# Mine268/CS-ViT

Measured on NVIDIA B200. Metric: images/sec Swin-B spatial fwd @224^2 bs256, higher is better.
Workload: dtype fp16

## Files before the change

cs-vit_b200/cs_vit/_lib.py:

```python
from __future__ import annotations

import ctypes
import os
from ctypes import c_char_p, c_float, c_int, c_longlong, c_void_p

_HERE = os.path.dirname(os.path.abspath(__file__))
LIB_PATH = os.environ.get("CSVIT_LIB", os.path.join(_HERE, "..", "lib", "libcsvit_sm100.so"))

SIGNATURES = {
    "csvit_abi_version": [],
    "csvit_window_index_map": [c_int, c_int, c_int, c_int, c_void_p, c_void_p],
    "csvit_shift_mask": [c_int, c_int, c_int, c_int, c_void_p, c_void_p],
    "csvit_rel_pos_index": [c_int, c_void_p, c_void_p],
    "csvit_merge_index_map": [c_int, c_int, c_void_p, c_void_p],
    "csvit_host_window_index_map": [c_int, c_int, c_int, c_int, c_void_p],
    "csvit_host_shift_mask": [c_int, c_int, c_int, c_int, c_void_p],
    "csvit_host_rel_pos_index": [c_int, c_void_p],
    "csvit_host_merge_index_map": [c_int, c_int, c_void_p],
    "csvit_expand_rel_bias": [c_void_p, c_void_p, c_int, c_int, c_void_p],
    "csvit_layernorm": [c_void_p, c_void_p, c_void_p, c_float, c_void_p, c_int, c_longlong, c_int, c_int, c_int,
                        c_int, c_int, c_int, c_int, c_void_p],
    "csvit_affine_rows": [c_void_p, c_void_p, c_void_p, c_void_p, c_int, c_longlong, c_int, c_void_p],
    "csvit_patch_im2col": [c_void_p, c_void_p, c_int, c_int, c_int, ctypes.POINTER(c_float), ctypes.POINTER(c_float),
                           c_void_p],
    "csvit_linear": [c_void_p, c_longlong, c_void_p, c_longlong, c_int, c_int, c_int, c_int, c_void_p, c_int, c_void_p,
                     c_longlong, c_void_p, c_longlong, c_int, c_int, c_int, c_int, c_int, c_int, c_void_p],
    "csvit_mlp_fused": [c_void_p, c_longlong, c_void_p, c_longlong, c_void_p, c_void_p, c_longlong, c_void_p, c_void_p,
                        c_longlong, c_int, c_int, c_int, c_void_p],
    "csvit_swin_attn_fused": [c_void_p, c_float, c_void_p, c_void_p, c_void_p, c_void_p, c_int, c_int, c_int, c_int,
                              c_int, c_int, c_int, c_int, c_void_p],
    "csvit_swin_attn_core": [c_void_p, c_longlong, c_void_p, c_void_p, c_int, c_int, c_int, c_int, c_int, c_int, c_int, c_int,
                             c_int, c_int, c_void_p],
    "csvit_crop_resize": [c_void_p, c_int, c_int, c_int, c_int, c_void_p, c_float, c_void_p, c_void_p, c_int, c_void_p],
    "csvit_rot6d_to_axis_angle": [c_void_p, c_void_p, c_longlong, c_void_p],
    "csvit_mano_fk": [c_void_p] * 10 + [c_void_p, c_void_p, c_int, c_void_p, c_void_p, c_void_p, c_int, c_void_p],
    "csvit_allreduce_f32": [c_void_p, c_void_p, c_void_p, c_longlong, c_int, c_int, c_float, c_int, c_void_p],
    "csvit_last_gemm_kernel": [],
    "csvit_set_gemm_tuning": [c_int, c_int, c_int, c_int],
    "csvit_window_attention": [c_void_p, c_void_p, c_void_p, c_int, c_int, c_int, c_int, c_int, c_int, c_int, c_int, c_void_p],
    "csvit_attention": [c_void_p, c_void_p, c_void_p, c_void_p, c_int, c_longlong, c_longlong, c_longlong, c_longlong,
                        c_int, c_int, c_int, c_int, c_float, c_void_p],
    "csvit_swinv2_window_attention": [c_void_p, c_void_p, c_void_p, c_void_p, c_int, c_int, c_int, c_int, c_int, c_int, c_int, c_int,
                                      c_int, c_int, c_void_p],
    "csvit_swinv2_qkv": [c_void_p, c_longlong, c_void_p, c_longlong, c_int, c_int, c_int, c_int, c_void_p, c_void_p, c_void_p, c_longlong,
                         c_void_p],
    "csvit_swinv2_attn_tc": [c_void_p, c_longlong, c_void_p, c_void_p, c_int, c_int, c_int, c_int, c_int, c_int, c_int, c_int, c_int,
                             c_void_p],
    "csvit_layernorm_post": [c_void_p, c_longlong, c_void_p, c_void_p, c_void_p, c_float, c_void_p, c_void_p, c_int, c_longlong,
                             c_int, c_int, c_int, c_int, c_int, c_int, c_int, c_void_p],
    "csvit_gemm_ex": [c_void_p, c_longlong, c_int, c_void_p, c_longlong, c_int, c_int, c_int, c_int, c_int, c_void_p, c_longlong,
                      c_int, c_int, c_int, c_int, c_void_p],
    "csvit_col_reduce": [c_void_p, c_int, c_longlong, c_void_p, c_longlong, c_void_p, c_int, c_int, c_int, c_int, c_int, c_int,
                         c_int, c_int, c_void_p, c_int, c_longlong, c_void_p, c_void_p, c_void_p],
    "csvit_transpose_f32": [c_void_p, c_longlong, c_void_p, c_longlong, c_int, c_int, c_void_p],
    "csvit_row_scale_add": [c_void_p, c_void_p, c_void_p, c_void_p, c_longlong, c_int, c_int, c_void_p],
    "csvit_eltwise": [c_int, c_void_p, c_void_p, c_void_p, c_int, c_longlong, c_void_p],
    "csvit_affine2_rows": [c_void_p, c_void_p, c_void_p, c_void_p, c_void_p, c_void_p, c_void_p, c_longlong, c_int, c_void_p],
    "csvit_layernorm_bwd": [c_void_p, c_void_p, c_int, c_longlong, c_void_p, c_float, c_int, c_int, c_int, c_int, c_int, c_int,
                            c_int, c_void_p, c_void_p, c_void_p, c_void_p, c_void_p],
    "csvit_attention_bwd": [c_void_p, c_void_p, c_void_p, c_void_p, c_void_p, c_void_p, c_void_p, c_int, c_longlong, c_longlong,
                            c_longlong, c_longlong, c_longlong, c_longlong, c_longlong, c_int, c_int, c_int, c_int, c_float,
                            c_void_p, c_void_p, c_int, c_int, c_int, c_int, c_void_p],
}

_lib = None


class CsvitError(RuntimeError):
    pass


def load() -> ctypes.CDLL:
    global _lib
    if _lib is not None:
        return _lib
    path = os.path.abspath(LIB_PATH)
    if not os.path.exists(path):
        raise ImportError(
            f"{path} not found. cs_vit has no CPU/PyTorch fallback: build the sm_100a kernels first with "
            f"`python -c 'import __graft_entry__ as g; g.build()'` or `make -C cs-vit_b200/csrc`.")
    lib = ctypes.CDLL(path)
    for name, argtypes in SIGNATURES.items():
        fn = getattr(lib, name)
        fn.argtypes = argtypes
        fn.restype = c_int
    lib.csvit_last_error.argtypes = []
    lib.csvit_last_error.restype = c_char_p
    _lib = lib
    return lib


def check(code: int) -> None:
    if code != 0:
        raise CsvitError(load().csvit_last_error().decode("utf-8", "replace"))
```

cs-vit_b200/cs_vit/net/swin_b200.py:

```python
from __future__ import annotations

import json
import os
from types import SimpleNamespace
from typing import Dict, List, Optional

import torch
import torch.nn as nn

from .. import ops
from ._pack import PackCache


PRECISIONS = {"bf16": torch.bfloat16, "fp16": torch.float16, "fp32": torch.float32}


class SwinConfigLite(SimpleNamespace):

    @classmethod
    def from_dict(cls, d: Dict) -> "SwinConfigLite":
        model_type = d.get("model_type", "swin")
        if model_type != "swin":
            raise NotImplementedError(
                f"backbone model_type '{model_type}' is not built: only Swin v1 (window 7) has sm_100a kernels "
                f"(SwinV2 is the next row of SURVEY.md §8f); there is no fallback path")
        embed_dim = d.get("embed_dim", 96)
        depths = list(d.get("depths", [2, 2, 6, 2]))
        cfg = cls(
            model_type=model_type,
            image_size=d.get("image_size", 224),
            patch_size=d.get("patch_size", 4),
            num_channels=d.get("num_channels", 3),
            embed_dim=embed_dim,
            depths=depths,
            num_heads=list(d.get("num_heads", [3, 6, 12, 24])),
            window_size=d.get("window_size", 7),
            mlp_ratio=d.get("mlp_ratio", 4.0),
            qkv_bias=d.get("qkv_bias", True),
            layer_norm_eps=d.get("layer_norm_eps", 1e-5),
            use_absolute_embeddings=d.get("use_absolute_embeddings", False),
            hidden_act=d.get("hidden_act", "gelu"),
            drop_path_rate=d.get("drop_path_rate", 0.1),
            hidden_size=int(embed_dim * 2 ** (len(depths) - 1)),
        )
        if cfg.patch_size != 4 or cfg.num_channels != 3 or cfg.mlp_ratio != 4.0 or not cfg.qkv_bias:
            raise NotImplementedError("only patch 4 / RGB / mlp_ratio 4 / qkv_bias Swin configurations are built")
        if cfg.use_absolute_embeddings or cfg.hidden_act != "gelu":
            raise NotImplementedError("absolute position embeddings / non-GELU activations are not built")
        if any(cfg.embed_dim * 2 ** s != 32 * h for s, h in enumerate(cfg.num_heads)):
            raise NotImplementedError("the attention kernels require head_dim == 32 at every stage")
        return cfg


def _holder(**children) -> nn.Module:
    m = nn.Module()
    for k, v in children.items():
        setattr(m, k, v)
    return m


class _SelfAttnParams(nn.Module):
    def __init__(self, dim: int, heads: int, ws: int):
        super().__init__()
        self.query = nn.Linear(dim, dim)
        self.key = nn.Linear(dim, dim)
        self.value = nn.Linear(dim, dim)
        self.relative_position_bias_table = nn.Parameter(torch.zeros((2 * ws - 1) ** 2, heads))
        ys, xs = torch.meshgrid(torch.arange(ws), torch.arange(ws), indexing="ij")
        dy = ys.reshape(-1, 1) - ys.reshape(1, -1) + ws - 1
        dx = xs.reshape(-1, 1) - xs.reshape(1, -1) + ws - 1
        self.register_buffer("relative_position_index", (dy * (2 * ws - 1) + dx).to(torch.int64))


class _BlockParams(nn.Module):

    def __init__(self, dim: int, heads: int, ws: int, eps: float):
        super().__init__()
        self.layernorm_before = nn.LayerNorm(dim, eps=eps)
        self.attention = _holder(self=_SelfAttnParams(dim, heads, ws), output=_holder(dense=nn.Linear(dim, dim)))
        self.layernorm_after = nn.LayerNorm(dim, eps=eps)
        self.intermediate = _holder(dense=nn.Linear(dim, 4 * dim))
        self.output = _holder(dense=nn.Linear(4 * dim, dim))


class SwinBackboneB200(nn.Module):
    def __init__(self, config: SwinConfigLite, precision: str = "bf16"):
        super().__init__()
        self.config = config
        self.precision = precision
        self.fuse_attn = True
        self.fuse_attn_widths = ops.ATTN_FUSED_WIDTHS
        self._drop_path_rand: List[torch.Tensor] = []
        self.fuse_mlp = True
        self.micro_batch = 0
        c0, eps, ws = config.embed_dim, config.layer_norm_eps, config.window_size
        self.embeddings = _holder(
            patch_embeddings=_holder(projection=nn.Conv2d(3, c0, kernel_size=4, stride=4)),
            norm=nn.LayerNorm(c0, eps=eps))
        stages: List[nn.Module] = []
        for s, (depth, heads) in enumerate(zip(config.depths, config.num_heads)):
            dim = c0 * 2 ** s
            stage = nn.Module()
            stage.blocks = nn.ModuleList([_BlockParams(dim, heads, ws, eps) for _ in range(depth)])
            if s < len(config.depths) - 1:
                stage.downsample = _holder(reduction=nn.Linear(4 * dim, 2 * dim, bias=False), norm=nn.LayerNorm(4 * dim, eps=eps))
            stages.append(stage)
        self.encoder = _holder(layers=nn.ModuleList(stages))
        self.layernorm = nn.LayerNorm(config.hidden_size, eps=eps)
        self._pack = PackCache()

    @classmethod
    def from_pretrained(cls, path: str, precision: str = "bf16") -> "SwinBackboneB200":
        with open(os.path.join(path, "config.json")) as f:
            cfg = SwinConfigLite.from_dict(json.load(f))
        model = cls(cfg, precision)
        st = os.path.join(path, "model.safetensors")
        if os.path.exists(st):
            from safetensors.torch import load_file
            sd = load_file(st)
        else:
            sd = torch.load(os.path.join(path, "pytorch_model.bin"), map_location="cpu")
        sd = {(k[len("swin."):] if k.startswith("swin.") else k): v for k, v in sd.items()}
        missing, unexpected = model.load_state_dict(sd, strict=False)
        missing = [k for k in missing if not k.endswith("relative_position_index")]
        unexpected = [k for k in unexpected if not k.startswith("pooler")]
        if missing or unexpected:
            raise RuntimeError(f"backbone checkpoint mismatch: missing {missing[:5]} unexpected {unexpected[:5]}")
        model.eval()
        return model

    @property
    def _fp32(self) -> bool:
        if self.precision not in PRECISIONS:
            raise ValueError(f"precision must be one of {sorted(PRECISIONS)}, got {self.precision!r}")
        return self.precision == "fp32"

    @property
    def _act_dtype(self) -> torch.dtype:
        _ = self._fp32
        return PRECISIONS[self.precision]

    def _w(self, key: str, tensors, build):
        return self._pack.get(f"{self.precision}/{key}", tensors, build)

    def _weight(self, key: str, lin_weight: torch.Tensor) -> torch.Tensor:
        dt = self._act_dtype
        return self._w(key, [lin_weight], lambda: lin_weight.detach().reshape(lin_weight.shape[0], -1).to(dt).contiguous())

    def _f32(self, key: str, t: torch.Tensor) -> torch.Tensor:
        return self._w(key, [t], lambda: t.detach().float().contiguous())

    def _block(self, x: torch.Tensor, blk: _BlockParams, key: str, B: int, H: int, W: int, heads: int, shift: int) -> None:
        cfg = self.config
        ws = cfg.window_size
        if min(H, W) <= ws:
            ws, shift = min(H, W), 0
        C = x.shape[1]
        act = self._act_dtype
        impl = ops.GEMM_SIMT if self._fp32 else ops.GEMM_TC
        sa = blk.attention.self
        qkv_src = [sa.query.weight, sa.key.weight, sa.value.weight]
        bqkv_src = [sa.query.bias, sa.key.bias, sa.value.bias]
        eps = cfg.layer_norm_eps
        ln1 = blk.layernorm_before
        proj = blk.attention.output.dense
        wproj, bproj = self._weight(key + "wproj", proj.weight), self._f32(key + "bproj", proj.bias)
        if self._fp32:
            wqkv = self._w(key + "wqkv", qkv_src, lambda: torch.cat([w.detach() for w in qkv_src], 0).to(act).contiguous())
            bqkv = self._w(key + "bqkv", bqkv_src, lambda: torch.cat([b.detach() for b in bqkv_src], 0).float().contiguous())
            bias = self._w(key + "relbias", [sa.relative_position_bias_table],
                           lambda: ops.expand_rel_bias(sa.relative_position_bias_table.detach(), ws))
            xn = ops.layernorm(x, self._f32(key + "ln1w", ln1.weight), self._f32(key + "ln1b", ln1.bias), eps, out_dtype=act,
                               mode=ops.LN_WINDOW, grid=(H, W), ws=ws, shift=shift)
            qkv = ops.linear(xn, wqkv, bqkv, out_dtype=act, impl=impl)
            ctx = ops.window_attention(qkv, bias, B, H, W, heads, ws, shift)
            ops.linear(ctx, wproj, bproj, resid=x, out=x, scatter=(H, W, ws, shift), impl=impl)
        else:
            if ws != 7 or C != 32 * heads:
                raise NotImplementedError(f"the tcgen05 window-attention kernels are built for 7x7 windows and head_dim 32 "
                                          f"(got window {ws}, C={C}, heads={heads}); use precision='fp32'")
            if self.fuse_attn and C in self.fuse_attn_widths:
                src = qkv_src + bqkv_src + [sa.relative_position_bias_table, ln1.weight, ln1.bias]
                wqkv_h, bqkv_h, bias_op = self._w(key + "attn_fused", src, lambda: ops.pack_attn_fused(
                    sa.query.weight, sa.key.weight, sa.value.weight, sa.query.bias, sa.key.bias, sa.value.bias,
                    sa.relative_position_bias_table, sa.relative_position_index, act, ln1.weight, ln1.bias))
                ctx = ops.swin_attn_fused(x, eps, wqkv_h, bqkv_h, bias_op, B, H, W, heads, ws, shift)
                ops.linear(ctx, wproj, bproj, resid=x, out=x, impl=impl)
            else:
                wqs, bqs = self._w(key + "wqkv_qs", qkv_src + bqkv_src, lambda: ops.pack_qkv_prescaled(
                    sa.query.weight, sa.key.weight, sa.value.weight, sa.query.bias, sa.key.bias, sa.value.bias, act))
                bias_l2 = self._w(key + "relbias_l2", [sa.relative_position_bias_table],
                                  lambda: ops.pack_rel_bias_log2(sa.relative_position_bias_table, sa.relative_position_index))
                xn = ops.layernorm(x, self._f32(key + "ln1w", ln1.weight), self._f32(key + "ln1b", ln1.bias), eps, out_dtype=act,
                                   mode=ops.LN_WINDOW, grid=(H, W), ws=ws, shift=shift)
                qkv = ops.linear(xn, wqs, bqs, out_dtype=act, impl=impl)
                tok = C >= 256
                ctx = ops.swin_attn_core(qkv, bias_l2, B, H, W, heads, ws, shift, token_order=tok, q_prescaled=True)
                ops.linear(ctx, wproj, bproj, resid=x, out=x, impl=impl, **({} if tok else {"scatter": (H, W, ws, shift)}))
        ln2 = blk.layernorm_after
        fc1, fc2 = blk.intermediate.dense, blk.output.dense
        xn = ops.layernorm(x, self._f32(key + "ln2w", ln2.weight), self._f32(key + "ln2b", ln2.bias), eps, out_dtype=act)
        if self.fuse_mlp and not self._fp32 and C in ops.MLP_FUSED_WIDTHS:
            ops.mlp_fused(xn, self._weight(key + "w1", fc1.weight), self._f32(key + "b1", fc1.bias),
                          self._weight(key + "w2", fc2.weight), self._f32(key + "b2", fc2.bias), x)
            return
        hid = ops.linear(xn, self._weight(key + "w1", fc1.weight), self._f32(key + "b1", fc1.bias), act=ops.ACT_GELU,
                         out_dtype=act, impl=impl)
        ops.linear(hid, self._weight(key + "w2", fc2.weight), self._f32(key + "b2", fc2.bias), resid=x, out=x, impl=impl)

    def forward_features(self, images: torch.Tensor, normalize: bool, return_stages: bool = False):
        cfg = self.config
        if not images.is_cuda:
            raise RuntimeError("SwinBackboneB200 runs on CUDA tensors only (there is no CPU fallback)")
        n, _, S, S2 = images.shape
        if S != S2 or S % (32 * cfg.window_size) != 0:
            raise ValueError(f"image side {S} must be a multiple of {32 * cfg.window_size} (no padding path, SURVEY.md §8b)")
        wants_grad = torch.is_grad_enabled() and any(p.requires_grad for p in self.parameters())
        if not return_stages and (wants_grad or (self.training and cfg.drop_path_rate > 0)):
            return self._forward_train(images, normalize)
        with torch.no_grad():
            return self._forward_infer(images, normalize, return_stages)

    def _block_pack(self, blk: _BlockParams, key: str, ws: int) -> Dict:
        act = self._act_dtype
        sa = blk.attention.self
        qkv_src = [sa.query.weight, sa.key.weight, sa.value.weight]
        bqkv_src = [sa.query.bias, sa.key.bias, sa.value.bias]
        tab = sa.relative_position_bias_table
        return {
            "wqkv": self._w(key + "wqkv", qkv_src, lambda: torch.cat([w.detach() for w in qkv_src], 0).to(act).contiguous()),
            "bqkv": self._w(key + "bqkv", bqkv_src, lambda: torch.cat([b.detach() for b in bqkv_src], 0).float().contiguous()),
            "bias": self._w(key + "relbias", [tab], lambda: ops.expand_rel_bias(tab.detach(), ws)),
            "bias_log2": None if self._fp32 else self._w(key + "relbias_l2", [tab], lambda: ops.pack_rel_bias_log2(tab, sa.relative_position_index)),
            "wo": self._weight(key + "wproj", blk.attention.output.dense.weight),
            "w1": self._weight(key + "w1", blk.intermediate.dense.weight),
            "w2": self._weight(key + "w2", blk.output.dense.weight),
            "rel_index": self._w(key + "relidx", [sa.relative_position_index], lambda: sa.relative_position_index.reshape(-1).long()),
            "table_rows": tab.shape[0],
        }

    def _forward_train(self, images: torch.Tensor, normalize: bool) -> torch.Tensor:
        from .. import autograd as ag
        cfg = self.config
        n, _, S, _ = images.shape
        act = self._act_dtype
        impl = ops.GEMM_SIMT if self._fp32 else ops.GEMM_TC
        eps = cfg.layer_norm_eps
        H = W = S // 4
        pe = self.embeddings.patch_embeddings.projection
        x = ag.PatchEmbedFn.apply(images.float().contiguous(), pe.weight, pe.bias, self.embeddings.norm.weight, self.embeddings.norm.bias,
                                  self._weight("pe_w", pe.weight), (normalize, eps, act, impl))
        total_blocks = sum(cfg.depths)
        rates = torch.linspace(0, cfg.drop_path_rate, total_blocks).tolist() if self.training and cfg.drop_path_rate > 0 else [0.0] * total_blocks
        k = -1
        for s, stage in enumerate(self.encoder.layers):
            heads = cfg.num_heads[s]
            for i, blk in enumerate(stage.blocks):
                k += 1
                ws, shift = cfg.window_size, (0 if i % 2 == 0 else cfg.window_size // 2)
                if min(H, W) <= ws:
                    ws, shift = min(H, W), 0
                sa = blk.attention.self
                pk = dict(self._block_pack(blk, f"s{s}b{i}/", ws))
                if rates[k] > 0.0:
                    keep = 1.0 - rates[k]
                    u = self._drop_path_rand.pop(0).to(x.device, torch.float32) if self._drop_path_rand else torch.rand(n, device=x.device)
                    pk["keep_scale"] = (torch.floor(keep + u) / keep).contiguous()
                x = ag.SwinBlockFn.apply(
                    x, blk.layernorm_before.weight, blk.layernorm_before.bias, sa.query.weight, sa.query.bias, sa.key.weight,
                    sa.key.bias, sa.value.weight, sa.value.bias, sa.relative_position_bias_table, blk.attention.output.dense.weight,
                    blk.attention.output.dense.bias, blk.layernorm_after.weight, blk.layernorm_after.bias, blk.intermediate.dense.weight,
                    blk.intermediate.dense.bias, blk.output.dense.weight, blk.output.dense.bias, pk,
                    (n, H, W, heads, ws, shift, eps, act, impl))
            if hasattr(stage, "downsample"):
                ds = stage.downsample
                x = ag.PatchMergeFn.apply(x, ds.norm.weight, ds.norm.bias, ds.reduction.weight,
                                          self._weight(f"s{s}/dsr", ds.reduction.weight), (H, W, eps, act, impl))
                H, W = H // 2, W // 2
        out = ag.LayerNormFn.apply(x, self.layernorm.weight, self.layernorm.bias, eps)
        return out.view(n, H * W, cfg.hidden_size)

    def _forward_infer(self, images: torch.Tensor, normalize: bool, return_stages: bool = False, out: Optional[torch.Tensor] = None):
        cfg = self.config
        n, _, S, _ = images.shape
        mb = self.micro_batch
        if mb and n > mb and not return_stages:
            images = images.float().contiguous()
            full = torch.empty(n, (S // 32) ** 2, cfg.hidden_size, dtype=torch.float32, device=images.device)
            for lo in range(0, n, mb):
                self._forward_infer(images[lo:lo + mb], normalize, out=full[lo:lo + mb])
            return full
        act = self._act_dtype
        impl = ops.GEMM_SIMT if self._fp32 else ops.GEMM_TC
        eps = cfg.layer_norm_eps
        H = W = S // 4
        cols = ops.patch_im2col(images.float().contiguous(), out_dtype=act, normalize=normalize)
        pe = self.embeddings.patch_embeddings.projection
        y = ops.linear(cols, self._weight("pe_w", pe.weight), self._f32("pe_b", pe.bias), out_dtype=torch.float32, impl=impl)
        x = ops.layernorm(y, self._f32("pe_lnw", self.embeddings.norm.weight), self._f32("pe_lnb", self.embeddings.norm.bias), eps)
        stages = []
        for s, stage in enumerate(self.encoder.layers):
            heads = cfg.num_heads[s]
            for i, blk in enumerate(stage.blocks):
                self._block(x, blk, f"s{s}b{i}/", n, H, W, heads, 0 if i % 2 == 0 else cfg.window_size // 2)
            if return_stages:
                stages.append(x.view(n, H * W, -1).clone())
            if hasattr(stage, "downsample"):
                ds = stage.downsample
                xm = ops.layernorm(x, self._f32(f"s{s}/dsw", ds.norm.weight), self._f32(f"s{s}/dsb", ds.norm.bias), eps,
                                   out_dtype=act, mode=ops.LN_MERGE2X2, grid=(H, W))
                x = ops.linear(xm, self._weight(f"s{s}/dsr", ds.reduction.weight), None, out_dtype=torch.float32, impl=impl)
                H, W = H // 2, W // 2
        out = ops.layernorm(x, self._f32("final_w", self.layernorm.weight), self._f32("final_b", self.layernorm.bias), eps,
                            out=None if out is None else out.view(n * H * W, cfg.hidden_size))
        out = out.view(n, H * W, cfg.hidden_size)
        return (out, stages) if return_stages else out

    def forward(self, pixel_values: torch.Tensor, **_unused) -> SimpleNamespace:
        return SimpleNamespace(last_hidden_state=self.forward_features(pixel_values, normalize=False), pooler_output=None)
```

cs-vit_b200/cs_vit/ops.py:

```python
from __future__ import annotations

import ctypes
from typing import Optional, Tuple

import torch

from . import _lib

F32, BF16, F16 = 0, 1, 2
ACT_NONE, ACT_GELU, ACT_RELU = 0, 1, 2
LN_IDENTITY, LN_WINDOW, LN_MERGE2X2 = 0, 1, 2
GEMM_TC, GEMM_SIMT = 0, 1

_DT = {torch.float32: F32, torch.bfloat16: BF16, torch.float16: F16}

launch_count = 0


def _code(dtype: torch.dtype) -> int:
    try:
        return _DT[dtype]
    except KeyError:
        raise TypeError(f"cs_vit kernels take float32, bfloat16 or float16 tensors, got {dtype}") from None

# ... 30 lines not shown
    for kind in sorted({e[4] for e in ev if e[4]}):
        sel = [e for e in ev if e[4] == kind]
        out[f"kind{kind}"] = {"launches": len(sel), "ms": sum(e[0].elapsed_time(e[1]) for e in sel), "flops": float(sum(e[2] for e in sel))}
    return out


def _call(name: str, *args, flops: float = 0.0, nbytes: float = 0.0) -> None:
    global launch_count
    launch_count += 1
    if _profile is not None and _profile["name"] == name:
        e0, e1 = torch.cuda.Event(enable_timing=True), torch.cuda.Event(enable_timing=True)
        e0.record()
        _lib.check(getattr(_lib.load(), name)(*args))
        e1.record()
        kind = _lib.load().csvit_last_gemm_kernel() if name == "csvit_linear" else 0
        _profile["events"].append((e0, e1, flops, nbytes, kind))
        return
    _lib.check(getattr(_lib.load(), name)(*args))


def _rows2d(t: torch.Tensor) -> Tuple[int, int, int]:
    if t.dim() != 2 or t.stride(1) != 1:
        raise ValueError(f"expected a 2-D tensor with contiguous rows, got shape {tuple(t.shape)} strides {t.stride()}")
    return t.shape[0], t.shape[1], t.stride(0)


def window_index_map(H: int, W: int, ws: int, shift: int, device="cuda") -> torch.Tensor:
    out = torch.empty(H * W, dtype=torch.int32, device=device)
    _call("csvit_window_index_map", H, W, ws, shift, out.data_ptr(), _stream())
    return out


def shift_mask(H: int, W: int, ws: int, shift: int, device="cuda") -> torch.Tensor:
    nW, L = (H // ws) * (W // ws), ws * ws
    out = torch.empty(nW, L, L, dtype=torch.float32, device=device)
    _call("csvit_shift_mask", H, W, ws, shift, out.data_ptr(), _stream())
    return out


def rel_pos_index(ws: int, device="cuda") -> torch.Tensor:
    out = torch.empty(ws * ws, ws * ws, dtype=torch.int32, device=device)
    _call("csvit_rel_pos_index", ws, out.data_ptr(), _stream())
    return out


def merge_index_map(H: int, W: int, device="cuda") -> torch.Tensor:
    out = torch.empty((H // 2) * (W // 2), 4, dtype=torch.int32, device=device)
    _call("csvit_merge_index_map", H, W, out.data_ptr(), _stream())
    return out


def expand_rel_bias(table: torch.Tensor, ws: int) -> torch.Tensor:
    _dev(table)
    table = table.contiguous().float()
    heads = table.shape[1]
    out = torch.empty(heads, ws * ws, ws * ws, dtype=torch.float32, device=table.device)
    _call("csvit_expand_rel_bias", table.data_ptr(), out.data_ptr(), heads, ws, _stream())
    return out


def layernorm(x: torch.Tensor, gamma: torch.Tensor, beta: torch.Tensor, eps: float, *, out_dtype=torch.float32,
              mode: int = LN_IDENTITY, grid: Tuple[int, int] = (0, 0), ws: int = 0, shift: int = 0,
              out: Optional[torch.Tensor] = None) -> torch.Tensor:
    _dev(x, gamma, beta, out)
    if x.dtype != torch.float32 or not x.is_contiguous():
        raise ValueError("layernorm input must be contiguous float32")
    rows_in, C = x.shape
    H, W = grid
    if mode == LN_MERGE2X2:
        rows, width = rows_in // 4, 4 * C
    else:
        rows, width = rows_in, C
    if gamma.numel() != width or beta.numel() != width:
        raise ValueError(f"layernorm affine width {gamma.numel()} != {width}")
    if out is None:
        out = torch.empty(rows, width, dtype=out_dtype, device=x.device)
    _call("csvit_layernorm", x.data_ptr(), gamma.data_ptr(), beta.data_ptr(), float(eps), out.data_ptr(), _code(out.dtype),
          out.stride(0), rows, C, mode, H, W, ws, shift, _stream(),
          nbytes=float(rows * width * (4 + out.element_size())))
    return out


def affine_rows(x: torch.Tensor, scale: torch.Tensor, shift: torch.Tensor, *, out_dtype=torch.float32) -> torch.Tensor:
    _dev(x, scale, shift)
    if x.dtype != torch.float32 or not x.is_contiguous():
        raise ValueError("affine_rows input must be contiguous float32")
    C = x.shape[-1]
    out = torch.empty(x.shape, dtype=out_dtype, device=x.device)
    _call("csvit_affine_rows", x.data_ptr(), scale.data_ptr(), shift.data_ptr(), out.data_ptr(), _code(out_dtype),
          x.numel() // C, C, _stream())
    return out


_MEAN = (ctypes.c_float * 3)(0.485, 0.456, 0.406)
_STD = (ctypes.c_float * 3)(0.229, 0.224, 0.225)


def patch_im2col(img: torch.Tensor, *, out_dtype=torch.bfloat16, normalize: bool = True) -> torch.Tensor:
    _dev(img)
    if img.dtype != torch.float32 or not img.is_contiguous() or img.dim() != 4 or img.shape[1] != 3:
        raise ValueError("patch_im2col takes contiguous float32 [B,3,S,S]")
    B, _, S, S2 = img.shape
    if S != S2:
        raise ValueError("square images only")
    out = torch.empty(B * (S // 4) ** 2, 48, dtype=out_dtype, device=img.device)
    mean = _MEAN if normalize else (ctypes.c_float * 3)(0, 0, 0)
    std = _STD if normalize else (ctypes.c_float * 3)(1, 1, 1)
    _call("csvit_patch_im2col", img.data_ptr(), out.data_ptr(), _code(out_dtype), B, S, mean, std, _stream())
    return out


def linear(a: torch.Tensor, w: torch.Tensor, bias: Optional[torch.Tensor] = None, *, act: int = ACT_NONE,
           resid: Optional[torch.Tensor] = None, out: Optional[torch.Tensor] = None, out_dtype: Optional[torch.dtype] = None,
           scatter: Optional[Tuple[int, int, int, int]] = None, impl: int = GEMM_TC) -> torch.Tensor:
    _dev(a, w, bias, resid, out)
    M, K, lda = _rows2d(a)
    N, K2, ldw = _rows2d(w)
    if K != K2 or a.dtype != w.dtype:
        raise ValueError(f"linear: A {tuple(a.shape)}/{a.dtype} vs W {tuple(w.shape)}/{w.dtype}")
    if out is None:
        out = torch.empty(M, N, dtype=out_dtype or a.dtype, device=a.device)
    _, No, ldo = _rows2d(out)
    if No != N:
        raise ValueError("linear: output width mismatch")
    ldr = 0
    if resid is not None:
        if resid.dtype != torch.float32:
            raise ValueError("linear: residual must be float32")
        ldr = _rows2d(resid)[2]
    if bias is not None and (bias.dtype != torch.float32 or bias.numel() != N):
        raise ValueError("linear: bias must be float32 [N]")
    sH, sW, sws, ssh = scatter if scatter is not None else (0, 0, 0, 0)
    _call("csvit_linear", a.data_ptr(), lda, w.data_ptr(), ldw, _code(a.dtype), M, N, K, _p(bias), act, _p(resid), ldr,
          out.data_ptr(), ldo, _code(out.dtype), sH, sW, sws, ssh, impl, _stream(), flops=2.0 * M * N * K)
    return out


MLP_FUSED_WIDTHS = (128, 256)


def mlp_fused(xn: torch.Tensor, w1: torch.Tensor, b1: torch.Tensor, w2: torch.Tensor, b2: torch.Tensor, x: torch.Tensor) -> torch.Tensor:
    _dev(xn, w1, b1, w2, b2, x)
    M, C, ldxn = _rows2d(xn)
    if w1.shape != (4 * C, C) or w2.shape != (C, 4 * C) or x.shape != (M, C) or x.dtype != torch.float32:
        raise ValueError("mlp_fused: shape mismatch")
    if not (xn.dtype == w1.dtype == w2.dtype) or xn.dtype not in (torch.bfloat16, torch.float16):
        raise ValueError("mlp_fused: xn / w1 / w2 must share a 16-bit dtype")
    _call("csvit_mlp_fused", xn.data_ptr(), ldxn, w1.data_ptr(), w1.stride(0), b1.data_ptr(), w2.data_ptr(), w2.stride(0),
          b2.data_ptr(), x.data_ptr(), x.stride(0), _code(xn.dtype), M, C, _stream(), flops=16.0 * M * C * C)
    return x


ATTN_FUSED_WIDTHS = (128, 256)
_LOG2E = 1.4426950408889634


def pack_attn_fused(wq: torch.Tensor, wk: torch.Tensor, wv: torch.Tensor, bq: torch.Tensor, bk: torch.Tensor, bv: torch.Tensor,
                    table: torch.Tensor, rel_index: torch.Tensor, dtype: torch.dtype, gamma: torch.Tensor, beta: torch.Tensor):
    C = wq.shape[0]
    heads = C // 32
    g64, be64 = gamma.detach().double(), beta.detach().double()
    fold_w = lambda w_: (w_.detach().double() * g64[None, :]).float()
    fold_b = lambda w_, b_: (b_.detach().double() + w_.detach().double() @ be64).float()
    w = torch.stack([fold_w(wq).view(heads, 32, C), fold_w(wk).view(heads, 32, C), fold_w(wv).view(heads, 32, C)], 1)
    qs = _LOG2E / 32.0 ** 0.5
    b = torch.stack([fold_b(wq, bq).view(heads, 32) * qs, fold_b(wk, bk).view(heads, 32), fold_b(wv, bv).view(heads, 32)], 1)
    return w.reshape(3 * C, C).to(dtype).contiguous(), b.reshape(3 * C).contiguous(), pack_rel_bias_log2(table, rel_index)


def pack_rel_bias_log2(table: torch.Tensor, rel_index: torch.Tensor) -> torch.Tensor:
    heads = table.shape[1]
    L = rel_index.shape[0]
    if L != 49:
        raise ValueError("pack_rel_bias_log2: 7x7 windows only")
    bias = table.detach().float()[rel_index.reshape(-1).long()].view(L, L, heads).permute(2, 0, 1)
    op = torch.zeros(heads, L, 56, dtype=torch.float32, device=table.device)
    op[:, :, :L] = bias * _LOG2E
    return op.to(torch.float16).reshape(heads * L, 56).contiguous()


def pack_qkv_prescaled(wq, wk, wv, bq, bk, bv, dtype: torch.dtype):
    qs = _LOG2E / 32.0 ** 0.5
    w = torch.cat([wq.detach().float() * qs, wk.detach().float(), wv.detach().float()], 0)
    b = torch.cat([bq.detach().float() * qs, bk.detach().float(), bv.detach().float()], 0)
    return w.to(dtype).contiguous(), b.contiguous()


def swin_attn_core(qkv: torch.Tensor, bias_log2: torch.Tensor, B: int, H: int, W: int, heads: int, ws: int, shift: int,
                   token_order: bool = False, q_prescaled: bool = False, out: Optional[torch.Tensor] = None) -> torch.Tensor:
    _dev(qkv, bias_log2, out)
    rows, C3, ld = _rows2d(qkv)
    C = C3 // 3
    if qkv.dtype not in (torch.bfloat16, torch.float16) or rows != B * H * W or C != heads * 32 or ws != 7:
        raise ValueError(f"swin_attn_core: needs 16-bit qkv [B*H*W, 3C] with head_dim 32 and 7x7 windows (rows={rows} C={C} heads={heads} ws={ws})")
    if bias_log2.dtype != torch.float16 or tuple(bias_log2.shape) != (heads * 49, 56) or not bias_log2.is_contiguous():
        raise ValueError("swin_attn_core: bias_log2 must be contiguous float16 [heads*49, 56] (pack_rel_bias_log2)")
    if out is None:
        out = torch.empty(rows, C, dtype=qkv.dtype, device=qkv.device)
    L = ws * ws
    _call("csvit_swin_attn_core", qkv.data_ptr(), ld, bias_log2.data_ptr(), out.data_ptr(), _code(qkv.dtype), B, H, W, C, heads, ws,
          shift, 1 if token_order else 0, 1 if q_prescaled else 0, _stream(),
          flops=float(rows) * 4.0 * L * C, nbytes=float(rows) * C * 8.0)
    return out


def swin_attn_fused(x: torch.Tensor, eps: float, wqkv_h: torch.Tensor, bqkv_h: torch.Tensor,
                    bias_op: torch.Tensor, B: int, H: int, W: int, heads: int, ws: int, shift: int,
                    out: Optional[torch.Tensor] = None) -> torch.Tensor:
    _dev(x, wqkv_h, bqkv_h, bias_op, out)
    if x.dtype != torch.float32 or not x.is_contiguous() or x.dim() != 2:
        raise ValueError("swin_attn_fused input must be contiguous float32 [B*H*W, C]")
    rows, C = x.shape
    if rows != B * H * W or C != heads * 32 or C not in ATTN_FUSED_WIDTHS:
        raise ValueError(f"swin_attn_fused: rows={rows} C={C} heads={heads} not supported (C in {ATTN_FUSED_WIDTHS}, head_dim 32)")
    if wqkv_h.dtype not in (torch.bfloat16, torch.float16) or tuple(wqkv_h.shape) != (3 * C, C) or not wqkv_h.is_contiguous():
        raise ValueError("swin_attn_fused: wqkv_h must be contiguous 16-bit [3C, C]")
    if bqkv_h.dtype != torch.float32 or bqkv_h.numel() != 3 * C or bias_op.dtype != torch.float16 or tuple(bias_op.shape) != (heads * 49, 56) or not bias_op.is_contiguous():
        raise ValueError("swin_attn_fused: bqkv_h must be float32 [3C] and bias_op contiguous float16 [heads*49, 56]")
    if out is None:
        out = torch.empty(rows, C, dtype=wqkv_h.dtype, device=x.device)
    L = ws * ws
    _call("csvit_swin_attn_fused", x.data_ptr(), float(eps), wqkv_h.data_ptr(), bqkv_h.data_ptr(),
          bias_op.data_ptr(), out.data_ptr(), _code(wqkv_h.dtype), B, H, W, C, heads, ws, shift, _stream(),
          flops=float(rows) * (6.0 * C * C + 4.0 * L * C), nbytes=float(rows) * C * 6.0)
    return out


def window_attention(qkv: torch.Tensor, bias_exp: Optional[torch.Tensor], B: int, H: int, W: int, heads: int, ws: int,
                     shift: int, bias_log2: Optional[torch.Tensor] = None, token_order: bool = False) -> torch.Tensor:
    if qkv.dtype != torch.float32:
        if bias_log2 is None:
            raise ValueError("window_attention: 16-bit qkv needs bias_log2 (ops.pack_rel_bias_log2)")
        return swin_attn_core(qkv, bias_log2, B, H, W, heads, ws, shift, token_order=token_order)
    if token_order:
        raise ValueError("window_attention: token-ordered output is built for the 16-bit kernels only")
    _dev(qkv, bias_exp)
    rows, C3, ld = _rows2d(qkv)
    C = C3 // 3
    if ld != C3 or rows != B * H * W:
        raise ValueError("window_attention: qkv must be dense [B*H*W, 3C]")
    out = torch.empty(rows, C, dtype=qkv.dtype, device=qkv.device)
    _call("csvit_window_attention", qkv.data_ptr(), _p(bias_exp), out.data_ptr(), _code(qkv.dtype), B, H, W, C,
          heads, ws, shift, _stream(), nbytes=float(qkv.numel() + out.numel()) * qkv.element_size())
    return out


def attention(q: torch.Tensor, k: torch.Tensor, v: torch.Tensor, n_seq: int, Lq: int, S: int, heads: int,
              scale: float) -> torch.Tensor:
    _dev(q, k, v)
    rq, D, ldq = _rows2d(q)
    rk, _, ldk = _rows2d(k)
    _, _, ldv = _rows2d(v)
    if rq != n_seq * Lq or rk != n_seq * S or D != heads * 32:
        raise ValueError("attention: shape mismatch (head_dim must be 32)")
    out = torch.empty(rq, D, dtype=q.dtype, device=q.device)
    _call("csvit_attention", q.data_ptr(), k.data_ptr(), v.data_ptr(), out.data_ptr(), _code(q.dtype), ldq, ldk, ldv, D,
          n_seq, Lq, S, heads, float(scale), _stream())
    return out


COPY_NONE, COPY_IDENTITY, COPY_WINDOW, COPY_MERGE2X2 = 0, 1, 2, 3


def swinv2_window_attention(qkv: torch.Tensor, bias_tab: torch.Tensor, logit_scale: torch.Tensor, B: int, H: int, W: int, heads: int,
                            ws: int, shift: int, mask_repeat: int = 2, token_order: bool = False) -> torch.Tensor:
    _dev(qkv, bias_tab, logit_scale)
    rows, C3, ld = _rows2d(qkv)
    C = C3 // 3
    if ld != C3 or rows != B * H * W:
        raise ValueError("swinv2_window_attention: qkv must be dense [B*H*W, 3C]")
    if bias_tab.dtype != torch.float32 or tuple(bias_tab.shape) != (heads, (2 * ws - 1) ** 2) or not bias_tab.is_contiguous():
        raise ValueError(f"swinv2_window_attention: bias table must be contiguous float32 [{heads}, {(2 * ws - 1) ** 2}]")
    if logit_scale.dtype != torch.float32 or logit_scale.numel() != heads or not logit_scale.is_contiguous():
        raise ValueError("swinv2_window_attention: logit_scale must be contiguous float32 [heads]")
    out = torch.empty(rows, C, dtype=qkv.dtype, device=qkv.device)
    L = ws * ws
    _call("csvit_swinv2_window_attention", qkv.data_ptr(), bias_tab.data_ptr(), logit_scale.data_ptr(), out.data_ptr(),
          _code(qkv.dtype), B, H, W, C, heads, ws, shift, mask_repeat, 1 if token_order else 0, _stream(),
          flops=4.0 * rows * L * C, nbytes=float(qkv.numel() + out.numel()) * qkv.element_size())
    return out


def swinv2_qkv(a: torch.Tensor, w: torch.Tensor, bias: Optional[torch.Tensor], qscale_log2: torch.Tensor) -> torch.Tensor:
    _dev(a, w, qscale_log2)
    M, K, lda = _rows2d(a)
    N, K2, ldw = _rows2d(w)
    C = N // 3
    if K2 != K or N != 3 * C or a.dtype != w.dtype or a.dtype not in (torch.float16, torch.bfloat16):
        raise ValueError("swinv2_qkv: a [M, K] and w [3C, K] must share one 16-bit dtype")
    if qscale_log2.dtype != torch.float32 or qscale_log2.numel() != C // 32 or not qscale_log2.is_contiguous():
        raise ValueError("swinv2_qkv: qscale_log2 must be contiguous float32 [C / 32]")
    if bias is not None and (bias.dtype != torch.float32 or bias.numel() != N or not bias.is_contiguous()):
        raise ValueError("swinv2_qkv: bias must be contiguous float32 [3C]")
    out = torch.empty(M, N, dtype=a.dtype, device=a.device)
    _call("csvit_swinv2_qkv", a.data_ptr(), lda, w.data_ptr(), ldw, _code(a.dtype), M, C, K, bias.data_ptr() if bias is not None else None,
          qscale_log2.data_ptr(), out.data_ptr(), N, _stream(), flops=2.0 * M * N * K,
          nbytes=float(a.numel() + w.numel() + out.numel()) * a.element_size())
    return out


def swinv2_bias_log2(bias_tab: torch.Tensor) -> torch.Tensor:
    heads = bias_tab.shape[0]
    out = torch.zeros(heads, 31, 48, dtype=torch.float32, device=bias_tab.device)
    out[:, :, :31] = bias_tab.float().view(heads, 31, 31) * 1.4426950408889634
    return out.contiguous()


def swinv2_attn_tc(qkv: torch.Tensor, bias_log2: torch.Tensor, B: int, H: int, W: int, heads: int, shift: int, mask_repeat: int = 2,
                   token_order: bool = False) -> torch.Tensor:
    _dev(qkv, bias_log2)
    rows, C3, ld = _rows2d(qkv)
    C = C3 // 3
    if rows != B * H * W or qkv.dtype not in (torch.float16, torch.bfloat16):
        raise ValueError("swinv2_attn_tc: qkv must be 16-bit [B*H*W, 3C]")
    if bias_log2.dtype != torch.float32 or tuple(bias_log2.shape) != (heads, 31, 48) or not bias_log2.is_contiguous():
        raise ValueError(f"swinv2_attn_tc: bias table must be contiguous float32 [{heads}, 31, 48]")
    out = torch.empty(rows, C, dtype=qkv.dtype, device=qkv.device)
    _call("csvit_swinv2_attn_tc", qkv.data_ptr(), ld, bias_log2.data_ptr(), out.data_ptr(), _code(qkv.dtype), B, H, W, C, heads, shift,
          mask_repeat, 1 if token_order else 0, _stream(), flops=4.0 * rows * 256 * C,
          nbytes=float(qkv.numel() + out.numel()) * qkv.element_size())
    return out


def layernorm_post(y: torch.Tensor, resid: Optional[torch.Tensor], gamma: torch.Tensor, beta: torch.Tensor, eps: float, *,
                   out: Optional[torch.Tensor] = None, copy_mode: int = COPY_NONE, copy_dtype: torch.dtype = torch.bfloat16,
                   geom: Tuple[int, int, int, int] = (0, 0, 0, 0)) -> Tuple[torch.Tensor, Optional[torch.Tensor]]:
    _dev(y, resid, gamma, beta, out)
    rows, C, ldy = _rows2d(y)
    if y.dtype != torch.float32:
        raise ValueError("layernorm_post input must be float32")
    if resid is not None and (resid.dtype != torch.float32 or tuple(resid.shape) != (rows, C) or not resid.is_contiguous()):
        raise ValueError("layernorm_post: residual must be contiguous float32 [rows, C]")
    if gamma.numel() != C or beta.numel() != C:
        raise ValueError(f"layernorm_post affine width {gamma.numel()} != {C}")
    if out is None:
        out = torch.empty(rows, C, dtype=torch.float32, device=y.device)
    elif out.dtype != torch.float32 or tuple(out.shape) != (rows, C) or not out.is_contiguous():
        raise ValueError("layernorm_post: out must be contiguous float32 [rows, C]")
    H, W, ws, shift = geom
    copy = None
    if copy_mode == COPY_MERGE2X2:
        copy = torch.empty(rows // 4, 4 * C, dtype=copy_dtype, device=y.device)
    elif copy_mode != COPY_NONE:
        copy = torch.empty(rows, C, dtype=copy_dtype, device=y.device)
    _call("csvit_layernorm_post", y.data_ptr(), ldy, _p(resid), gamma.data_ptr(), beta.data_ptr(), float(eps), out.data_ptr(), _p(copy),
          _code(copy_dtype), 0 if copy is None else copy.stride(0), copy_mode, rows, C, H, W, ws, shift, _stream(),
          nbytes=float(rows * C * (8 + (4 if resid is not None else 0) + (0 if copy is None else copy.element_size()))))
    return out, copy


CR_SUM, CR_CENTERED, CR_DOT = 0, 1, 2
EW_GELU_FWD, EW_GELU_BWD, EW_RELU_BWD = 0, 1, 2


def gemm_ex(a: torch.Tensor, a_mn: bool, b: torch.Tensor, b_mn: bool, *, out: Optional[torch.Tensor] = None,
            out_dtype: Optional[torch.dtype] = None, accumulate: bool = False, impl: int = GEMM_TC, split_k: int = 0) -> torch.Tensor:
    _dev(a, b, out)
    if a.dtype == torch.float32 and impl == GEMM_TC:
        if a_mn:
            a, a_mn = transpose(a), False
        if b_mn:
            b, b_mn = transpose(b), False
    r0, c0, lda = _rows2d(a)
    r1, c1, ldb = _rows2d(b)
    M, K = (c0, r0) if a_mn else (r0, c0)
    N, K2 = (c1, r1) if b_mn else (r1, c1)
    if K != K2 or a.dtype != b.dtype:
        raise ValueError(f"gemm_ex: A {tuple(a.shape)}/{a.dtype} (mn={a_mn}) vs B {tuple(b.shape)}/{b.dtype} (mn={b_mn})")
    if out is None:
        if accumulate:
            raise ValueError("gemm_ex: accumulate needs an output tensor")
        out = torch.empty(M, N, dtype=out_dtype or a.dtype, device=a.device)
    Mo, No, ldo = _rows2d(out)
    if (Mo, No) != (M, N):
        raise ValueError("gemm_ex: output shape mismatch")
    _call("csvit_gemm_ex", a.data_ptr(), lda, int(a_mn), b.data_ptr(), ldb, int(b_mn), _code(a.dtype), M, N, K, out.data_ptr(), ldo,
# ... 208 lines not shown
```

cs-vit_b200/csrc/api.cu:

```cuda
#include <cstdarg>
#include <cstdio>
#include <cstdlib>

#include "../../include/csvit.h"
#include "errors.h"
#include "gemm.cuh"
#include "rowops.cuh"

namespace csvit {

static thread_local char g_err[1024] = "";

int set_error(const char* fmt, ...) {
  va_list ap;
  va_start(ap, fmt);
  vsnprintf(g_err, sizeof(g_err), fmt, ap);
  va_end(ap);
  return 1;
}
const char* last_error() { return g_err; }

bool pdl_enabled() {
  static const bool on = [] { const char* e = getenv("CSVIT_PDL"); return e && e[0] == '1'; }();
  return on;
}

}

using namespace csvit;

static_assert(int(CSVIT_F32) == int(DT_F32) && int(CSVIT_BF16) == int(DT_BF16) && int(CSVIT_F16) == int(DT_F16), "dtype codes");
static inline bool ok_dtype(int d) { return d == DT_F32 || d == DT_BF16 || d == DT_F16; }
static_assert(int(CSVIT_ACT_GELU) == int(ACT_GELU) && int(CSVIT_ACT_RELU) == int(ACT_RELU), "activation codes");
static_assert(int(CSVIT_LN_WINDOW) == int(LN_WINDOW) && int(CSVIT_LN_MERGE2X2) == int(LN_MERGE2X2), "layernorm modes");
static_assert(int(CSVIT_GEMM_SIMT_FP32) == int(GEMM_SIMT), "gemm impl codes");

static inline cudaStream_t S(void* s) { return static_cast<cudaStream_t>(s); }
static GemmTuning g_tune = {0, 0, -1, -1};

extern "C" {

int csvit_abi_version(void) { return CSVIT_ABI_VERSION; }
const char* csvit_last_error(void) { return last_error(); }

int csvit_window_index_map(int H, int W, int ws, int shift, int32_t* out, void* stream) {
  CSVIT_REQUIRE(ws > 0 && H % ws == 0 && W % ws == 0, "window_index_map: %dx%d not divisible by window %d", H, W, ws);
  CSVIT_REQUIRE(shift >= 0 && shift < ws, "window_index_map: shift %d outside [0,%d)", shift, ws);
  return launch_window_index_map(H, W, ws, shift, out, S(stream));
}
int csvit_shift_mask(int H, int W, int ws, int shift, float* out, void* stream) {
  CSVIT_REQUIRE(ws > 0 && H % ws == 0 && W % ws == 0, "shift_mask: %dx%d not divisible by window %d", H, W, ws);
  CSVIT_REQUIRE(shift >= 0 && shift < ws, "shift_mask: shift %d outside [0,%d)", shift, ws);
  return launch_shift_mask(H, W, ws, shift, out, S(stream));
}
int csvit_rel_pos_index(int ws, int32_t* out, void* stream) {
  CSVIT_REQUIRE(ws > 0, "rel_pos_index: window %d", ws);
  return launch_rel_index(ws, out, S(stream));
}
int csvit_merge_index_map(int H, int W, int32_t* out, void* stream) {
  CSVIT_REQUIRE(H % 2 == 0 && W % 2 == 0, "merge_index_map: %dx%d must be even", H, W);
  return launch_merge_index_map(H, W, out, S(stream));
}
int csvit_host_window_index_map(int H, int W, int ws, int shift, int32_t* out) {
  CSVIT_REQUIRE(ws > 0 && H % ws == 0 && W % ws == 0, "window_index_map: %dx%d not divisible by window %d", H, W, ws);
  CSVIT_REQUIRE(shift >= 0 && shift < ws, "window_index_map: shift %d outside [0,%d)", shift, ws);
  WinGeom g = make_geom(H, W, ws, shift);
  for (int r = 0; r < g.N; ++r) out[r] = win_row_to_token(g, r);
  return 0;
}
int csvit_host_shift_mask(int H, int W, int ws, int shift, float* out) {
  CSVIT_REQUIRE(ws > 0 && H % ws == 0 && W % ws == 0, "shift_mask: %dx%d not divisible by window %d", H, W, ws);
  CSVIT_REQUIRE(shift >= 0 && shift < ws, "shift_mask: shift %d outside [0,%d)", shift, ws);
  WinGeom g = make_geom(H, W, ws, shift);
  const int nW = (H / ws) * (W / ws);
  for (int w = 0; w < nW; ++w)
    for (int i = 0; i < g.L; ++i)
      for (int j = 0; j < g.L; ++j)
        out[(w * g.L + i) * g.L + j] = (shift > 0 && win_region(g, w, i) != win_region(g, w, j)) ? -100.0f : 0.0f;
  return 0;
}
int csvit_host_rel_pos_index(int ws, int32_t* out) {
  CSVIT_REQUIRE(ws > 0, "rel_pos_index: window %d", ws);
  const int L = ws * ws;
  for (int i = 0; i < L; ++i)
    for (int j = 0; j < L; ++j) out[i * L + j] = rel_pos_index(ws, i, j);
  return 0;
}
int csvit_host_merge_index_map(int H, int W, int32_t* out) {
  CSVIT_REQUIRE(H % 2 == 0 && W % 2 == 0, "merge_index_map: %dx%d must be even", H, W);
  for (int t = 0; t < (H / 2) * (W / 2); ++t)
    for (int q = 0; q < 4; ++q) out[t * 4 + q] = merge_src_token(W, t / (W / 2), t % (W / 2), q);
  return 0;
}

int csvit_expand_rel_bias(const float* table, float* out, int heads, int ws, void* stream) {
  CSVIT_REQUIRE(heads > 0 && ws > 0, "expand_rel_bias: heads=%d ws=%d", heads, ws);
  return launch_expand_rel_bias(table, out, heads, ws, S(stream));
}

int csvit_layernorm(const float* x, const float* gamma, const float* beta, float eps, void* out, int out_dtype,
                    long long ldo, int rows, int C, int mode, int H, int W, int ws, int shift, void* stream) {
  CSVIT_REQUIRE(ok_dtype(out_dtype), "layernorm: bad out_dtype %d", out_dtype);
  WinGeom g = make_geom(H > 0 ? H : 1, W > 0 ? W : 1, ws > 0 ? ws : 1, shift);
  if (mode == LN_WINDOW) {
    CSVIT_REQUIRE(ws > 0 && H % ws == 0 && W % ws == 0, "layernorm(window): %dx%d not divisible by window %d", H, W, ws);
    CSVIT_REQUIRE(shift >= 0 && shift < ws, "layernorm(window): shift %d outside [0,%d)", shift, ws);
    CSVIT_REQUIRE(rows % (H * W) == 0, "layernorm(window): rows %d not a multiple of %d tokens", rows, H * W);
  } else if (mode == LN_MERGE2X2) {
    CSVIT_REQUIRE(H % 2 == 0 && W % 2 == 0, "layernorm(merge): %dx%d must be even", H, W);
    CSVIT_REQUIRE(rows % ((H / 2) * (W / 2)) == 0, "layernorm(merge): rows %d not a multiple of %d", rows, (H / 2) * (W / 2));
  } else {
    CSVIT_REQUIRE(mode == LN_IDENTITY, "layernorm: unknown mode %d", mode);
  }
  return launch_layernorm(x, gamma, beta, eps, out, out_dtype, ldo, rows, C, mode, g, S(stream));
}

int csvit_affine_rows(const float* x, const float* scale, const float* shift, void* out, int out_dtype, long long rows,
                      int C, void* stream) {
  CSVIT_REQUIRE(ok_dtype(out_dtype), "affine_rows: bad out_dtype %d", out_dtype);
  return launch_affine_rows(x, scale, shift, out, out_dtype, rows, C, S(stream));
}

int csvit_patch_im2col(const float* img, void* out, int out_dtype, int B, int S_, const float* mean3, const float* std3,
                       void* stream) {
  CSVIT_REQUIRE(ok_dtype(out_dtype), "patch_im2col: bad out_dtype %d", out_dtype);
  return launch_patch_im2col(img, out, out_dtype, B, S_, mean3, std3, S(stream));
}

int csvit_linear(const void* A, long long lda, const void* W, long long ldw, int in_dtype, int M, int N, int K,
                 const float* bias, int act, const float* resid, long long ldr, void* out, long long ldo, int out_dtype,
                 int scatter_H, int scatter_W, int scatter_ws, int scatter_shift, int impl, void* stream) {
  CSVIT_REQUIRE(ok_dtype(in_dtype), "linear: bad in_dtype %d", in_dtype);
  CSVIT_REQUIRE(ok_dtype(out_dtype), "linear: bad out_dtype %d", out_dtype);
  CSVIT_REQUIRE(act >= ACT_NONE && act <= ACT_RELU, "linear: bad activation %d", act);
  CSVIT_REQUIRE(lda >= K && ldw >= K && ldo >= N, "linear: pitches smaller than the logical widths");
  EpiParams ep{};
  ep.bias = bias; ep.resid = resid; ep.out = out; ep.ldo = ldo; ep.ldr = ldr;
  ep.out_dtype = out_dtype; ep.act = act;
  ep.map_mode = ROWMAP_IDENTITY;
  ep.geom = make_geom(1, 1, 1, 0);
  if (scatter_ws > 0) {
    CSVIT_REQUIRE(scatter_H % scatter_ws == 0 && scatter_W % scatter_ws == 0, "linear: scatter grid %dx%d vs window %d",
                  scatter_H, scatter_W, scatter_ws);
    CSVIT_REQUIRE(M % (scatter_H * scatter_W) == 0, "linear: M=%d not a multiple of %d tokens", M, scatter_H * scatter_W);
    ep.map_mode = ROWMAP_WINDOW;
    ep.geom = make_geom(scatter_H, scatter_W, scatter_ws, scatter_shift);
  }
  return launch_gemm(A, lda, W, ldw, in_dtype, M, N, K, ep, impl, g_tune, S(stream));
}

int csvit_mlp_fused(const void* xn, long long ldxn, const void* W1, long long ldw1, const float* b1, const void* W2,
                    long long ldw2, const float* b2, float* x, long long ldx, int dtype, int M, int C, void* stream) {
  CSVIT_REQUIRE(ldxn >= C && ldw1 >= C && ldw2 >= 4 * C && ldx >= C, "mlp_fused: pitches smaller than the logical widths");
  return launch_mlp_fused(xn, ldxn, W1, ldw1, b1, W2, ldw2, b2, x, ldx, dtype, M, C, S(stream));
}

int csvit_last_gemm_kernel(void) { return last_gemm_kernel(); }

int csvit_set_gemm_tuning(int cluster, int tma_store, int max_ctas, int pair) {
  g_tune.pair = pair;
  CSVIT_REQUIRE(cluster == 0 || cluster == 1 || cluster == 2 || cluster == 4, "gemm tuning: cluster %d not in {0,1,2,4}", cluster);
  g_tune.cluster = cluster; g_tune.tma_store = tma_store; g_tune.max_ctas = max_ctas;
  return 0;
}

int csvit_swin_attn_fused(const float* x, float eps, const void* wqkv_h, const float* bqkv_h,
                          const void* bias_op, void* ctx, int dtype, int B, int H, int W, int C, int heads, int ws, int shift,
                          void* stream) {
  CSVIT_REQUIRE(x && wqkv_h && bqkv_h && bias_op && ctx, "swin_attn_fused: null operand");
  return launch_swin_attn_fused(x, eps, wqkv_h, bqkv_h, bias_op, ctx, dtype, B, H, W, C, heads, ws, shift, S(stream));
}

int csvit_swin_attn_core(const void* qkv, long long ldq, const void* bias_log2, void* ctx, int dtype, int B, int H, int W, int C,
                         int heads, int ws, int shift, int token_order, int q_prescaled, void* stream) {
  CSVIT_REQUIRE(qkv && bias_log2 && ctx, "swin_attn_core: null operand");
  return launch_swin_attn_core(qkv, ldq, bias_log2, ctx, dtype, B, H, W, C, heads, ws, shift, token_order, q_prescaled, S(stream));
}

int csvit_window_attention(const void* qkv, const float* bias, void* out, int dtype, int B, int H, int W, int C, int heads, int ws,
                           int shift, void* stream) {
  CSVIT_REQUIRE(dtype == DT_F32, "window_attention: the exact fp32 kernel only (16-bit operands: csvit_swin_attn_core), dtype %d", dtype);
  CSVIT_REQUIRE(bias != nullptr, "window_attention: needs the csvit_expand_rel_bias table");
  CSVIT_REQUIRE(C == heads * 32, "window_attention: head_dim must be 32 (C=%d heads=%d)", C, heads);
  CSVIT_REQUIRE(H % ws == 0 && W % ws == 0, "window_attention: %dx%d not divisible by window %d", H, W, ws);
  const int L = ws * ws, nW = (H / ws) * (W / ws);
  const float* q = static_cast<const float*>(qkv);
  return launch_attention_simt(q, q + C, q + 2 * C, out, DT_F32, 3ll * C, 3ll * C, 3ll * C, C, B * nW, L, L, heads,
                               0.17677669529663687f, bias, H, W, ws, shift, S(stream));
}

int csvit_crop_resize(const void* frames, int frames_u8, int N, int H, int W, const float* boxes, float expansion_ratio,
                      float* square_boxes_out, float* out, int size, void* stream) {
  CSVIT_REQUIRE(frames && boxes && out, "crop_resize: null operand");
  return launch_crop_resize(frames, frames_u8, N, H, W, boxes, expansion_ratio, square_boxes_out, out, size, S(stream));
}

int csvit_rot6d_to_axis_angle(const float* d6, float* axis_angle, long long n, void* stream) {
  CSVIT_REQUIRE(d6 && axis_angle, "rot6d_to_axis_angle: null operand");
  return launch_rot6d_to_axis_angle(d6, axis_angle, n, S(stream));
}

int csvit_mano_fk(const float* pose, const float* betas, const float* root_norm, const float* v_template, const float* shapedirs,
                  const float* posedirs, const float* pose_mean, const float* j_regressor, const float* lbs_weights,
                  const float* j_regressor_out, const int* parents16, const int* edges40, int rodrigues_mode, float* joint_cam,
                  float* verts_cam, float* root_transl, int n, void* stream) {
  CSVIT_REQUIRE(pose && betas && root_norm && v_template && shapedirs && j_regressor && lbs_weights && j_regressor_out && parents16 &&
                    edges40 && joint_cam && verts_cam && root_transl, "mano_fk: null operand");
  CSVIT_REQUIRE(rodrigues_mode == 0 || rodrigues_mode == 1, "mano_fk: rodrigues_mode %d", rodrigues_mode);
  return launch_mano_fk(pose, betas, root_norm, v_template, shapedirs, posedirs, pose_mean, j_regressor, lbs_weights, j_regressor_out,
                        parents16, edges40, rodrigues_mode, joint_cam, verts_cam, root_transl, n, S(stream));
}

int csvit_allreduce_f32(const void* const* bufs, const void* const* flags, void* multicast, long long n, int rank, int world, float scale,
                        int ctas, void* stream) {
  CSVIT_REQUIRE(bufs && flags, "allreduce_f32: null pointer tables");
  return launch_allreduce_f32(const_cast<void* const*>(bufs), const_cast<void* const*>(flags), multicast, n, rank, world, scale, ctas,
                              S(stream));
}

int csvit_attention(const void* q, const void* k, const void* v, void* out, int dtype, long long ldq, long long ldk,
                    long long ldv, long long ldo, int n_seq, int Lq, int S_, int heads, float scale, void* stream) {
  CSVIT_REQUIRE(ok_dtype(dtype), "attention: bad dtype %d", dtype);
  return launch_attention_simt(q, k, v, out, dtype, ldq, ldk, ldv, ldo, n_seq, Lq, S_, heads, scale, nullptr, 0, 0, 0, 0,
                               S(stream));
}

int csvit_swinv2_window_attention(const void* qkv, const float* bias_tab, const float* logit_scale, void* out, int dtype, int B, int H,
                                  int W, int C, int heads, int ws, int shift, int mask_repeat, int out_token_order, void* stream) {
  CSVIT_REQUIRE(ok_dtype(dtype), "swinv2_window_attention: bad dtype %d", dtype);
  CSVIT_REQUIRE(bias_tab != nullptr && logit_scale != nullptr, "swinv2_window_attention: bias table and logit scale are required");
  CSVIT_REQUIRE(mask_repeat >= 0 && mask_repeat <= 2, "swinv2_window_attention: mask_repeat %d outside [0,2]", mask_repeat);
  return launch_swinv2_window_attention(qkv, bias_tab, logit_scale, out, dtype, B, H, W, C, heads, ws, shift, mask_repeat,
                                        out_token_order ? 1 : 0, S(stream));
}

int csvit_swinv2_qkv(const void* A, long long lda, const void* W, long long ldw, int dtype, int M, int C, int K, const float* bias,
                     const float* qscale_log2, void* out, long long ldo, void* stream) {
  CSVIT_REQUIRE(dtype == DT_BF16 || dtype == DT_F16, "swinv2_qkv: 16-bit operands only (the fp32 mode normalises inside its attention kernel)");
  CSVIT_REQUIRE(A && W && out && qscale_log2, "swinv2_qkv: null operand");
  CSVIT_REQUIRE(C > 0 && C % 32 == 0 && lda >= K && ldw >= K && ldo >= 3ll * C, "swinv2_qkv: C=%d must be a multiple of 32, pitches >= widths", C);
  CSVIT_REQUIRE(ldo % 8 == 0 && (reinterpret_cast<uintptr_t>(out) & 15) == 0 && (!bias || (reinterpret_cast<uintptr_t>(bias) & 15) == 0),
                "swinv2_qkv: output rows and bias must be 16-byte aligned");
  EpiParams ep{};
  ep.bias = bias; ep.out = out; ep.ldo = ldo; ep.out_dtype = dtype; ep.act = ACT_NONE;
  ep.map_mode = ROWMAP_IDENTITY;
  ep.geom = make_geom(1, 1, 1, 0);
  ep.cos_scale = qscale_log2; ep.cos_C = C;
  return launch_gemm(A, lda, W, ldw, dtype, M, 3 * C, K, ep, GEMM_TC, g_tune, S(stream));
}

int csvit_swinv2_attn_tc(const void* qkv, long long ldq, const float* bias_log2, void* ctx, int dtype, int B, int H, int W, int C,
                         int heads, int shift, int mask_repeat, int token_order, void* stream) {
  CSVIT_REQUIRE(qkv && bias_log2 && ctx, "swinv2_attn_tc: null operand");
  CSVIT_REQUIRE(mask_repeat >= 0 && mask_repeat <= 2, "swinv2_attn_tc: mask_repeat %d outside [0,2]", mask_repeat);
  return launch_swinv2_attn_tc(qkv, ldq, bias_log2, ctx, dtype, B, H, W, C, heads, shift, mask_repeat, token_order, S(stream));
}

int csvit_layernorm_post(const float* y, long long ldy, const float* resid, const float* gamma, const float* beta, float eps, float* out,
                         void* copy, int copy_dtype, long long ldc, int copy_mode, int rows, int C, int H, int W, int ws, int shift,
                         void* stream) {
  CSVIT_REQUIRE(ok_dtype(copy_dtype), "layernorm_post: bad copy dtype %d", copy_dtype);
  CSVIT_REQUIRE(ldy >= C, "layernorm_post: pitch smaller than the row width");
  WinGeom g = make_geom(H > 0 ? H : 1, W > 0 ? W : 1, ws > 0 ? ws : 1, shift);
  if (copy_mode == CSVIT_COPY_WINDOW) {
    CSVIT_REQUIRE(ws > 0 && H % ws == 0 && W % ws == 0, "layernorm_post(window): %dx%d not divisible by window %d", H, W, ws);
    CSVIT_REQUIRE(shift >= 0 && shift < ws, "layernorm_post(window): shift %d outside [0,%d)", shift, ws);
    CSVIT_REQUIRE(rows % (H * W) == 0, "layernorm_post(window): rows %d not a multiple of %d tokens", rows, H * W);
    CSVIT_REQUIRE(ldc >= C, "layernorm_post(window): copy pitch smaller than the row width");
  } else if (copy_mode == CSVIT_COPY_MERGE2X2) {
    CSVIT_REQUIRE(H > 0 && W > 0 && H % 2 == 0 && W % 2 == 0, "layernorm_post(merge): %dx%d must be even", H, W);
    CSVIT_REQUIRE(rows % (H * W) == 0, "layernorm_post(merge): rows %d not a multiple of %d tokens", rows, H * W);
    CSVIT_REQUIRE(ldc >= 4 * C, "layernorm_post(merge): copy pitch smaller than 4C");
  }
  return launch_layernorm_post(y, ldy, resid, gamma, beta, eps, out, copy, copy_dtype, ldc, copy_mode, rows, C, g, S(stream));
}

int csvit_gemm_ex(const void* A, long long lda, int a_mn, const void* B, long long ldb, int b_mn, int in_dtype, int M, int N, int K,
                  void* out, long long ldo, int out_dtype, int accumulate, int impl, int split_k, void* stream) {
  CSVIT_REQUIRE(ok_dtype(in_dtype) && ok_dtype(out_dtype), "gemm_ex: bad dtype (%d, %d)", in_dtype, out_dtype);
  CSVIT_REQUIRE(lda >= (a_mn ? M : K) && ldb >= (b_mn ? N : K) && ldo >= N, "gemm_ex: pitches smaller than the logical widths");
  return launch_gemm_ex(A, lda, a_mn ? 1 : 0, B, ldb, b_mn ? 1 : 0, in_dtype, M, N, K, out, ldo, out_dtype, accumulate ? 1 : 0, impl,
                        split_k, S(stream));
}

int csvit_col_reduce(const void* a, int a_dtype, long long lda, const float* b, long long ldb, const float* center, int mode,
                     int rows, int C, int row_mode, int H, int W, int ws, int shift, void* copy, int copy_dtype, long long ldc,
                     float* s1, float* s2, void* stream) {
  CSVIT_REQUIRE(ok_dtype(a_dtype) && ok_dtype(copy_dtype), "col_reduce: bad dtype (%d, %d)", a_dtype, copy_dtype);
  WinGeom g = make_geom(H > 0 ? H : 1, W > 0 ? W : 1, ws > 0 ? ws : 1, shift);
  if (row_mode == LN_WINDOW) {
    CSVIT_REQUIRE(ws > 0 && H % ws == 0 && W % ws == 0, "col_reduce(window): %dx%d not divisible by window %d", H, W, ws);
    CSVIT_REQUIRE(shift >= 0 && shift < ws, "col_reduce(window): shift %d outside [0,%d)", shift, ws);
    CSVIT_REQUIRE(rows % (H * W) == 0, "col_reduce(window): rows %d not a multiple of %d tokens", rows, H * W);
  }
  return launch_col_reduce(a, a_dtype, lda, b, ldb, center, mode, rows, C, row_mode, g, copy, copy_dtype, ldc, s1, s2, S(stream));
}

int csvit_transpose_f32(const float* src, long long lds, float* dst, long long ldd, int rows, int cols, void* stream) {
  CSVIT_REQUIRE(lds >= cols && ldd >= rows, "transpose: pitches smaller than the logical widths");
  return launch_transpose_f32(src, lds, dst, ldd, rows, cols, S(stream));
}

int csvit_row_scale_add(const float* x, const float* y, const float* s, float* out, long long rows, int C, int group_rows, void* stream) {
  CSVIT_REQUIRE(y && s && out, "row_scale_add: null operand");
  return launch_row_scale_add(x, y, s, out, rows, C, group_rows, S(stream));
}

int csvit_eltwise(int op, const void* a, const void* b, void* out, int dtype, long long n, void* stream) {
  CSVIT_REQUIRE(ok_dtype(dtype), "eltwise: bad dtype %d", dtype);
  return launch_eltwise(op, a, b, out, dtype, n, S(stream));
}

int csvit_affine2_rows(const float* dy, const float* x, const float* a, const float* b, const float* c0, const float* resid,
                       float* out, long long rows, int C, void* stream) {
  return launch_affine2_rows(dy, x, a, b, c0, resid, out, rows, C, S(stream));
}

int csvit_layernorm_bwd(const float* x, const void* dy, int dy_dtype, long long ldy, const float* gamma, float eps, int rows, int C,
                        int mode, int H, int W, int ws, int shift, const float* dres, float* dx, float* dgamma, float* dbeta,
                        void* stream) {
  CSVIT_REQUIRE(ok_dtype(dy_dtype), "layernorm_bwd: bad dy dtype %d", dy_dtype);
  WinGeom g = make_geom(H > 0 ? H : 1, W > 0 ? W : 1, ws > 0 ? ws : 1, shift);
  if (mode == LN_WINDOW) {
// ... 37 lines not shown
```

cs-vit_b200/csrc/attn_common.cuh:

```cuda
#pragma once
#include "common.cuh"

namespace csvit {

constexpr int FA_L = 49;
constexpr uint32_t FA_BIAS_BYTES = 49 * 56 * 2;
constexpr uint32_t FA_BIAS_STAGE = 5632;
constexpr float FA_MASK_LOG2 = -100.0f * 1.4426950408889634f;

__device__ __forceinline__ void tmem_ld_32x16(uint32_t taddr, uint32_t (&r)[16]) {
  asm volatile(
      "tcgen05.ld.sync.aligned.32x32b.x16.b32 "
      "{%0, %1, %2, %3, %4, %5, %6, %7, %8, %9, %10, %11, %12, %13, %14, %15}, [%16];"
      : "=r"(r[0]), "=r"(r[1]), "=r"(r[2]), "=r"(r[3]), "=r"(r[4]), "=r"(r[5]), "=r"(r[6]), "=r"(r[7]),
        "=r"(r[8]), "=r"(r[9]), "=r"(r[10]), "=r"(r[11]), "=r"(r[12]), "=r"(r[13]), "=r"(r[14]), "=r"(r[15])
      : "r"(taddr)
      : "memory");
}
__device__ __forceinline__ void tmem_ld_32x8(uint32_t taddr, uint32_t (&r)[8]) {
  asm volatile("tcgen05.ld.sync.aligned.32x32b.x8.b32 {%0, %1, %2, %3, %4, %5, %6, %7}, [%8];"
               : "=r"(r[0]), "=r"(r[1]), "=r"(r[2]), "=r"(r[3]), "=r"(r[4]), "=r"(r[5]), "=r"(r[6]), "=r"(r[7])
               : "r"(taddr)
               : "memory");
}
__device__ __forceinline__ uint64_t fa_mnmajor_desc(uint32_t smem_addr) {
  uint64_t d = 0;
  d |= static_cast<uint64_t>((smem_addr & 0x3FFFFu) >> 4);
  d |= static_cast<uint64_t>(8192 >> 4) << 16;
  d |= static_cast<uint64_t>(1024 >> 4) << 32;
  d |= static_cast<uint64_t>(1) << 46;
  d |= static_cast<uint64_t>(2) << 61;
  return d;
}
__device__ __forceinline__ float fa_exp2(float x) {
  float y;
  asm("ex2.approx.ftz.f32 %0, %1;" : "=f"(y) : "f"(x));
  return y;
}

__device__ __forceinline__ void tmem_ld_32x1(uint32_t taddr, uint32_t& r) {
  asm volatile("tcgen05.ld.sync.aligned.32x32b.x1.b32 {%0}, [%1];" : "=r"(r) : "r"(taddr) : "memory");
}
__device__ __forceinline__ void fa_add_h2(float& a, float& b, uint32_t h2) {
  asm("{\n\t.reg .f16 lo, hi;\n\tmov.b32 {lo, hi}, %2;\n\tadd.rn.f32.f16 %0, lo, %0;\n\tadd.rn.f32.f16 %1, hi, %1;\n\t}" : "+f"(a), "+f"(b) : "r"(h2));
}
__device__ __forceinline__ void fa_bulk_load(void* smem_dst, const void* gsrc, uint32_t bytes, uint64_t* bar) {
  asm volatile("cp.async.bulk.shared::cluster.global.mbarrier::complete_tx::bytes [%0], [%1], %2, [%3];"
               ::"r"(smem_u32(smem_dst)), "l"(gsrc), "r"(bytes), "r"(smem_u32(bar)) : "memory");
}
__device__ __forceinline__ float fa_max3(float a, float b, float c) {
  float d;
  asm("max.f32 %0, %1, %2, %3;" : "=f"(d) : "f"(a), "f"(b), "f"(c));
  return d;
}


__device__ __forceinline__ unsigned long long fa_row_mask(const WinGeom& g, int w, int j) {
  if (g.shift <= 0) return 0ull;
  const int nWy = g.H / g.ws;
  const int wy = w / g.nWx, wx = w - wy * g.nWx;
  const int iy = j / 7, ix = j - iy * 7, th = g.ws - g.shift;
  unsigned long long dm = 0;
  if (wy == nWy - 1) {
    const unsigned long long rows_lo = (1ull << (7 * th)) - 1ull;
    dm |= (iy < th) ? ~rows_lo : rows_lo;
  }
  if (wx == g.nWx - 1) {
    const unsigned long long cols_lo = ((1ull << th) - 1ull) * 0x40810204081ull;
    dm |= (ix < th) ? ~cols_lo : cols_lo;
  }
  return dm & ((1ull << FA_L) - 1ull);
}

__device__ __forceinline__ void fa_add_mask(float (&sv)[50], uint32_t dm_lo, uint32_t dm_hi, bool th4) {
  if ((dm_lo | dm_hi) == 0u) return;
  if (th4) {
    const float m[2][2] = {{(dm_lo & 1u) ? FA_MASK_LOG2 : 0.0f, (dm_lo & (1u << 4)) ? FA_MASK_LOG2 : 0.0f},
                           {(dm_lo & (1u << 28)) ? FA_MASK_LOG2 : 0.0f, (dm_hi & 1u) ? FA_MASK_LOG2 : 0.0f}};
#pragma unroll
    for (int c = 0; c < FA_L; ++c) sv[c] += m[(c / 7) >= 4][(c % 7) >= 4];
  } else {
#pragma unroll
    for (int c = 0; c < FA_L; ++c) {
      const uint32_t bit = c < 32 ? (dm_lo >> c) & 1u : (dm_hi >> (c - 32)) & 1u;
      sv[c] += bit ? FA_MASK_LOG2 : 0.0f;
    }
  }
}

}
```

cs-vit_b200/csrc/attn_fused.cu:

```cuda
#include <type_traits>

#include "errors.h"
#include "gemm.cuh"
#include "rowops.cuh"
#include "attn_common.cuh"

namespace csvit {

constexpr int FA_THREADS = 768;
constexpr int FA_SM_WARP0 = 4, FA_LN_WARP0 = 16, FA_LN_WARPS = 8;
constexpr int FA_NSLOT = 3;
constexpr int FA_ROWS = 2 * FA_L;
constexpr uint32_t FA_SLAB = 128 * 128;
constexpr uint32_t FA_STAGE = 96 * 128;
constexpr int FA_NBS = 2;
constexpr int FA_NST = 4;
constexpr uint32_t FA_QP = 0, FA_K = 16384, FA_V = 24576, FA_HB = 32768;
constexpr uint32_t FA_TM_SLOT = 160, FA_TM_S = 96;
constexpr uint32_t FA_TAB = FA_K + 49 * 128;

template <int C>
struct FaCfg {
  static constexpr int KB = C / 64;
  static constexpr int HEADS = C / 32;
  static constexpr int XNB = C <= 128 ? 2 : 1;
  static constexpr uint32_t XN_TILE = KB * FA_SLAB;
  static constexpr uint32_t XN_OFF = 0;
  static constexpr uint32_t RING_OFF = XNB * XN_TILE;
  static constexpr uint32_t HB_OFF = RING_OFF + FA_NST * FA_STAGE;
  static constexpr uint32_t BIAS_OFF = HB_OFF + FA_NSLOT * FA_HB;
  static constexpr uint32_t BAR_OFF = BIAS_OFF + FA_NBS * FA_BIAS_STAGE;
  static constexpr size_t SMEM = 1024 + size_t(BAR_OFF) + 512;
};

struct FaParams {
  const float* x;
  float eps;
  const float* bqkv;
  const void* bias;
  void* ctx;
  int num_windows;
  int nW;
  float qscale;
  WinGeom g;
};

#ifdef CSVIT_FA_TRACE
__device__ long long fa_trace_buf[16][256];
#define FA_TR(kind, idx) do { if (blockIdx.x == 0 && (idx) < 256) fa_trace_buf[kind][idx] = clock64(); } while (0)
#else
#define FA_TR(kind, idx) do { } while (0)
#endif

template <int FMT, int C>
__global__ void __launch_bounds__(FA_THREADS, 1)
swin_attn_fused_kernel(const __grid_constant__ CUtensorMap tmW, FaParams p) {
  using Cfg = FaCfg<C>;
  using T16 = typename std::conditional<FMT == 1, __nv_bfloat16, __half>::type;
  constexpr int KB = Cfg::KB, HEADS = Cfg::HEADS, XNB = Cfg::XNB;
  extern __shared__ uint8_t smem_raw[];
  const uint32_t base = (smem_u32(smem_raw) + 1023u) & ~1023u;
  uint8_t* smem = smem_raw + (base - smem_u32(smem_raw));
  uint64_t* bars = reinterpret_cast<uint64_t*>(smem + Cfg::BAR_OFF);
  uint64_t* w_full = bars;
  uint64_t* w_empty = bars + FA_NST;
  uint64_t* xn_full = bars + 2 * FA_NST;
  uint64_t* xn_empty = xn_full + 2;
  uint64_t* acc_full = xn_full + 4;
  uint64_t* acc_empty = acc_full + FA_NSLOT;
  uint64_t* qkv_full = acc_empty + FA_NSLOT;
  uint64_t* s_full = qkv_full + FA_NSLOT;
  uint64_t* p_full = s_full + FA_NSLOT;
  uint64_t* o_full = p_full + FA_NSLOT;
  uint64_t* b_full = o_full + FA_NSLOT;
  uint64_t* b_empty = b_full + FA_NBS;
  uint32_t* tmem_slot = reinterpret_cast<uint32_t*>(b_empty + FA_NBS);
  volatile int* ln_done = reinterpret_cast<volatile int*>(tmem_slot + 1);
  float* bq_tab = reinterpret_cast<float*>(smem + Cfg::HB_OFF + FA_TAB);
  float* bv_tab = reinterpret_cast<float*>(smem + Cfg::HB_OFF + FA_HB + FA_TAB);
  static_assert(C * 4 <= 15 * 128, "bias table does not fit the padding key rows");

  const int warp = threadIdx.x >> 5, lane = threadIdx.x & 31;
  const int num_tiles = (p.num_windows + 1) >> 1;
  const int my_tiles = (num_tiles - int(blockIdx.x) + int(gridDim.x) - 1) / int(gridDim.x);
  const int total = my_tiles * HEADS;

  for (uint32_t i = threadIdx.x; i < Cfg::RING_OFF / 16; i += FA_THREADS) reinterpret_cast<uint4*>(smem)[i] = make_uint4(0u, 0u, 0u, 0u);
  for (uint32_t i = threadIdx.x; i < (FA_NSLOT * FA_HB) / 16; i += FA_THREADS)
    reinterpret_cast<uint4*>(smem + Cfg::HB_OFF)[i] = make_uint4(0u, 0u, 0u, 0u);
  if (threadIdx.x == 0) {
    prefetch_tmap(&tmW);
    for (int s = 0; s < FA_NST; ++s) { mbar_init(&w_full[s], 1); mbar_init(&w_empty[s], 1); }
    for (int b = 0; b < 2; ++b) { mbar_init(&xn_full[b], FA_LN_WARPS); mbar_init(&xn_empty[b], 1); }
    for (int b = 0; b < FA_NBS; ++b) { mbar_init(&b_full[b], 1); mbar_init(&b_empty[b], 4); }
    for (int b = 0; b < FA_NSLOT; ++b) {
      mbar_init(&acc_full[b], 1); mbar_init(&acc_empty[b], 4);
      mbar_init(&qkv_full[b], 4); mbar_init(&s_full[b], 1);
      mbar_init(&p_full[b], 4); mbar_init(&o_full[b], 1);
    }
    *ln_done = 0;
    fence_mbar_init();
  }
  if (warp == 1) tmem_alloc(tmem_slot, 512);
  __syncthreads();
  for (int c = threadIdx.x; c < C; c += FA_THREADS) {
    bq_tab[c] = p.bqkv[(c >> 5) * 96 + (c & 31)];
    bv_tab[c] = p.bqkv[(c >> 5) * 96 + 64 + (c & 31)];
  }
  fence_proxy_async_smem();
  tc_fence_before();
  __syncthreads();
  tc_fence_after();
  const uint32_t tmem_base = *tmem_slot;
  griddep_launch();
  griddep_wait();

  if (warp < FA_SM_WARP0) {
  asm volatile("setmaxnreg.dec.sync.aligned.u32 40;");
  if (warp == 0) {
    if (lane == 0) {
      int s = 0; uint32_t ph = 0;
      int wq = 0, bq = 0;
      while (wq < total * KB || bq < total) {
        bool moved = false;
        if (wq < total * KB && mbar_test_wait(&w_empty[s], ph ^ 1u)) {
          const int h = (wq / KB) % HEADS, kb = wq % KB;
          mbar_arrive_expect_tx(&w_full[s], 96 * 128);
          tma_load_2d(smem + Cfg::RING_OFF + size_t(s) * FA_STAGE, &tmW, &w_full[s], kb * 64, h * 96);
          if (wq < 128) FA_TR(15, 128 + wq);
          if (++s == FA_NST) { s = 0; ph ^= 1u; }
          ++wq; moved = true;
        }
        if (bq < total) {
          const int bs = bq % FA_NBS;
          if (mbar_test_wait(&b_empty[bs], ((uint32_t(bq) / FA_NBS) & 1u) ^ 1u)) {
            mbar_arrive_expect_tx(&b_full[bs], FA_BIAS_BYTES);
            fa_bulk_load(smem + Cfg::BIAS_OFF + uint32_t(bs) * FA_BIAS_STAGE, static_cast<const char*>(p.bias) + size_t(bq % HEADS) * FA_BIAS_BYTES,
                         FA_BIAS_BYTES, &b_full[bs]);
            ++bq; moved = true;
          }
        }
        if (!moved) __nanosleep(256);
      }
    }
  } else if (warp == 1) {
    {
      constexpr uint32_t idesc_g = make_idesc(uint32_t(FMT), 128, 96);
      int s = 0; uint32_t ph = 0;
      uint32_t xn_addr = 0;
      auto issue_g = [&](int gh) {
        const int h = gh % HEADS, ti = gh / HEADS, sl = gh % FA_NSLOT;
        const uint32_t n = uint32_t(gh / FA_NSLOT);
        const int xb = XNB == 2 ? (ti & 1) : 0;
        if (h == 0) {
          mbar_wait(&xn_full[xb], XNB == 2 ? ((ti >> 1) & 1) : (ti & 1));
          xn_addr = base + Cfg::XN_OFF + uint32_t(xb) * Cfg::XN_TILE;
        }
        mbar_wait(&acc_empty[sl], (n & 1u) ^ 1u);
        tc_fence_after();
        if (lane == 0) FA_TR(0, gh);
        const uint32_t d_tmem = tmem_base + uint32_t(sl) * FA_TM_SLOT;
#pragma unroll 1
        for (int kb = 0; kb < KB; ++kb) {
          mbar_wait(&w_full[s], ph);
          tc_fence_after();
          if (lane == 0 && kb < 2 && gh < 64) FA_TR(15, 2 * gh + kb);
          if (fa_elect_one()) {
            const uint64_t adesc = make_sw128_kmajor_desc(xn_addr + uint32_t(kb) * FA_SLAB);
            const uint64_t bdesc = make_sw128_kmajor_desc(base + Cfg::RING_OFF + uint32_t(s) * FA_STAGE);
#pragma unroll
            for (int k = 0; k < 4; ++k) umma_ss<false>(d_tmem, adesc + uint64_t(2 * k), bdesc + uint64_t(2 * k), idesc_g, (kb | k) ? 1u : 0u);
            umma_commit(&w_empty[s]);
            if (kb == KB - 1) {
              umma_commit(&acc_full[sl]);
              if (h == HEADS - 1) umma_commit(&xn_empty[xb]);
            }
          }
          __syncwarp();
          if (++s == FA_NST) { s = 0; ph ^= 1u; }
        }
        if (lane == 0) FA_TR(1, gh);
      };
      for (int gh = 0; gh < total; ++gh) issue_g(gh);
    }
  } else if (warp == 2) {
    {
      constexpr uint32_t idesc_s = make_idesc(uint32_t(FMT), 128, 64);
      constexpr uint32_t idesc_o = make_idesc(uint32_t(FMT), 128, 64) | (1u << 16);
      for (int gs = 0; gs < total + 2; ++gs) {
        if (gs >= 2) {
          const int gh = gs - 2, sl = gh % FA_NSLOT;
          mbar_wait(&p_full[sl], uint32_t(gh / FA_NSLOT) & 1u);
          tc_fence_after();
          if (lane == 0) FA_TR(2, gh);
          if (fa_elect_one()) {
            const uint32_t hb = base + Cfg::HB_OFF + uint32_t(sl) * FA_HB;
            const uint32_t d_tmem = tmem_base + uint32_t(sl) * FA_TM_SLOT + FA_TM_S;
            const uint64_t pdesc = make_sw128_kmajor_desc(hb + FA_QP);
            const uint64_t vdesc = fa_mnmajor_desc(hb + FA_V);
#pragma unroll
            for (int k = 0; k < 4; ++k) umma_ss<false>(d_tmem, pdesc + uint64_t(2 * k), vdesc + uint64_t(128 * k), idesc_o, k ? 1u : 0u);
            umma_commit(&o_full[sl]);
          }
          __syncwarp();
        }
        if (gs < total) {
          const int sl = gs % FA_NSLOT;
          mbar_wait(&qkv_full[sl], uint32_t(gs / FA_NSLOT) & 1u);
          tc_fence_after();
          if (lane == 0) FA_TR(3, gs);
          if (fa_elect_one()) {
            const uint32_t hb = base + Cfg::HB_OFF + uint32_t(sl) * FA_HB;
            const uint32_t d_tmem = tmem_base + uint32_t(sl) * FA_TM_SLOT + FA_TM_S;
            const uint64_t qdesc = make_sw128_kmajor_desc(hb + FA_QP), kdesc = make_sw128_kmajor_desc(hb + FA_K);
#pragma unroll
            for (int k = 0; k < 4; ++k) umma_ss<false>(d_tmem, qdesc + uint64_t(2 * k), kdesc + uint64_t(2 * k), idesc_s, k ? 1u : 0u);
            umma_commit(&s_full[sl]);
          }
          __syncwarp();
          if (lane == 0) FA_TR(4, gs);
        }
      }
    }
  } else {
    const int pl = lane;
    for (int ti = 1; ti < my_tiles; ++ti) {
      while (*ln_done + 3 < ti) __nanosleep(2000);
      const int t = int(blockIdx.x) + ti * int(gridDim.x);
      for (int q = pl; q < FA_ROWS; q += 32) {
        const int wg = 2 * t + q / FA_L, i = q % FA_L;
        if (wg >= p.num_windows) continue;
        const int b = wg / p.nW, w = wg - b * p.nW;
        const char* src = reinterpret_cast<const char*>(p.x + (static_cast<long long>(b) * p.g.N + win_row_to_token(p.g, w * FA_L + i)) * C);
#pragma unroll
        for (int o = 0; o < C * 4; o += 128) asm volatile("prefetch.global.L2 [%0];" ::"l"(src + o));
      }
    }
  }
  } else if (warp < FA_LN_WARP0) {
    asm volatile("setmaxnreg.inc.sync.aligned.u32 104;");
    const int g = (warp - FA_SM_WARP0) >> 2;
    const int quad = warp & 3;
    const int r = quad * 32 + lane;
    const int wdx = r >> 6, j = r & 63;
    const bool bf = FMT == 1;
    uint8_t* hb = smem + Cfg::HB_OFF + uint32_t(g) * FA_HB;
    const uint32_t lane_bits = uint32_t(quad * 32) << 16;
    const uint32_t ta = tmem_base + lane_bits + uint32_t(g) * FA_TM_SLOT;
    const uint32_t ts = ta + FA_TM_S;
    T16* ctx = static_cast<T16*>(p.ctx);
    long long tok_off = -1;
    uint32_t dm_lo = 0, dm_hi = 0;
    int cur_ti = -1;
    uint32_t n = 0;
    const int slot_iy = (j < FA_L ? j : 0) / 7, slot_ix = (j < FA_L ? j : 0) % 7;
    const int th = p.g.ws - p.g.shift, nWy = p.g.H / p.g.ws;
    const unsigned long long rows_lo = (1ull << (7 * th)) - 1ull;
    const unsigned long long cols_lo = ((1ull << th) - 1ull) * 0x40810204081ull;
    for (int gh = g; gh < total; gh += FA_NSLOT, ++n) {
      const int ti = gh / HEADS, h = gh - ti * HEADS;
      const uint32_t ph = n & 1u;
      if (ti != cur_ti) {
        cur_ti = ti;
        const int t = int(blockIdx.x) + ti * int(gridDim.x);
        const int wg = 2 * t + wdx;
        tok_off = -1; dm_lo = dm_hi = 0;
        if (j < FA_L && wg < p.num_windows) {
          const int b = wg / p.nW, w = wg - b * p.nW;
          const int wy = w / p.g.nWx, wx = w - wy * p.g.nWx;
          int y = wy * 7 + slot_iy + p.g.shift; if (y >= p.g.H) y -= p.g.H;
          int x = wx * 7 + slot_ix + p.g.shift; if (x >= p.g.W) x -= p.g.W;
          tok_off = (static_cast<long long>(b) * p.g.N + y * p.g.W + x) * C;
          if (p.g.shift > 0) {
            unsigned long long dm = 0;
            if (wy == nWy - 1) dm |= (slot_iy < th) ? ~rows_lo : rows_lo;
            if (wx == p.g.nWx - 1) dm |= (slot_ix < th) ? ~cols_lo : cols_lo;
            dm &= (1ull << FA_L) - 1ull;
            dm_lo = uint32_t(dm); dm_hi = uint32_t(dm >> 32);
          }
        }
      }
      {
        if (quad == 0 && lane == 0) FA_TR(5, gh);
        mbar_wait(&acc_full[g], ph);
        tc_fence_after();
        if (quad == 0 && lane == 0) FA_TR(6, gh);
        uint8_t* qrow = hb + FA_QP + r * 128;
        uint8_t* krow = hb + FA_K + j * 128;
        uint8_t* vrow = hb + FA_V + j * 128;
        uint32_t rq[32], rk[32];
        tmem_ld_32x32(ta, rq);
        tmem_ld_wait();
        tmem_ld_32x32(ta + 32u, rk);
        {
          const float4* bq4 = reinterpret_cast<const float4*>(bq_tab + h * 32);
          const float2 qs2 = make_float2(p.qscale, p.qscale);
#pragma unroll
          for (int c = 0; c < 4; ++c) {
            const float4 b0 = bq4[2 * c], b1 = bq4[2 * c + 1];
            const float2 q0 = __ffma2_rn(make_float2(__uint_as_float(rq[8 * c]), __uint_as_float(rq[8 * c + 1])), qs2, make_float2(b0.x, b0.y));
            const float2 q1 = __ffma2_rn(make_float2(__uint_as_float(rq[8 * c + 2]), __uint_as_float(rq[8 * c + 3])), qs2, make_float2(b0.z, b0.w));
            const float2 q2 = __ffma2_rn(make_float2(__uint_as_float(rq[8 * c + 4]), __uint_as_float(rq[8 * c + 5])), qs2, make_float2(b1.x, b1.y));
            const float2 q3 = __ffma2_rn(make_float2(__uint_as_float(rq[8 * c + 6]), __uint_as_float(rq[8 * c + 7])), qs2, make_float2(b1.z, b1.w));
            const uint32_t own = uint32_t(((wdx * 4 + c) ^ (r & 7)) << 4), other = uint32_t((((1 - wdx) * 4 + c) ^ (r & 7)) << 4);
            *reinterpret_cast<uint4*>(qrow + own) = make_uint4(pack16(bf, q0.x, q0.y), pack16(bf, q1.x, q1.y), pack16(bf, q2.x, q2.y), pack16(bf, q3.x, q3.y));
            *reinterpret_cast<uint4*>(qrow + other) = make_uint4(0u, 0u, 0u, 0u);
          }
        }
        auto store_kv = [&](uint8_t* row, const uint32_t (&rr)[32]) {
          if (j < FA_L) {
#pragma unroll
            for (int c = 0; c < 4; ++c)
              *reinterpret_cast<uint4*>(row + (((wdx * 4 + c) ^ (r & 7)) << 4)) =
                  make_uint4(pack16(bf, __uint_as_float(rr[8 * c]), __uint_as_float(rr[8 * c + 1])), pack16(bf, __uint_as_float(rr[8 * c + 2]), __uint_as_float(rr[8 * c + 3])),
                             pack16(bf, __uint_as_float(rr[8 * c + 4]), __uint_as_float(rr[8 * c + 5])), pack16(bf, __uint_as_float(rr[8 * c + 6]), __uint_as_float(rr[8 * c + 7])));
          }
        };
        tmem_ld_wait();
        tmem_ld_32x32(ta + 64u, rq);
        store_kv(krow, rk);
        tmem_ld_wait();
        tc_fence_before();
        __syncwarp();
        if (lane == 0) mbar_arrive(&acc_empty[g]);
        store_kv(vrow, rq);
        fence_proxy_async_smem();
        __syncwarp();
        if (lane == 0) mbar_arrive(&qkv_full[g]);
        if (quad == 0 && lane == 0) FA_TR(7, gh);
      }
      float rsum;
      {
        mbar_wait(&s_full[g], ph);
        tc_fence_after();
        if (quad == 0 && lane == 0) FA_TR(8, gh);
        uint32_t s0[32], s1[16], s2;
        tmem_ld_32x32(ts, s0);
        tmem_ld_32x16(ts + 32u, s1);
        tmem_ld_32x1(ts + 48u, s2);
        tmem_ld_wait();
        tc_fence_before();
        float sv[50];
#pragma unroll
        for (int c = 0; c < 32; ++c) sv[c] = __uint_as_float(s0[c]);
#pragma unroll
        for (int c = 0; c < 16; ++c) sv[32 + c] = __uint_as_float(s1[c]);
        sv[48] = __uint_as_float(s2);
        sv[49] = 0.0f;
        {
          const int bs = gh % FA_NBS;
          mbar_wait(&b_full[bs], (uint32_t(gh) / FA_NBS) & 1u);
          const uint4* brow = reinterpret_cast<const uint4*>(smem + Cfg::BIAS_OFF + uint32_t(bs) * FA_BIAS_STAGE + (j < FA_L ? j : 0) * 112);
#pragma unroll
          for (int c = 0; c < 7; ++c) {
            const uint4 b4 = brow[c];
            fa_add_h2(sv[8 * c], sv[8 * c + 1], b4.x);
            if (c < 6) {
              fa_add_h2(sv[8 * c + 2], sv[8 * c + 3], b4.y);
              fa_add_h2(sv[8 * c + 4], sv[8 * c + 5], b4.z);
              fa_add_h2(sv[8 * c + 6], sv[8 * c + 7], b4.w);
            }
          }
          __syncwarp();
          if (lane == 0) mbar_arrive(&b_empty[bs]);
        }
        sv[49] = -INFINITY;
        fa_add_mask(sv, dm_lo, dm_hi, p.g.ws - p.g.shift == 4);
        float mx0 = fa_max3(sv[0], sv[1], sv[2]), mx1 = fa_max3(sv[3], sv[4], sv[5]);
#pragma unroll
        for (int c = 6; c < 48; c += 4) { mx0 = fa_max3(mx0, sv[c], sv[c + 1]); mx1 = fa_max3(mx1, sv[c + 2], sv[c + 3]); }
        const float mxx = fmaxf(mx0, mx1);
        const float2 nm = make_float2(-mxx, -mxx);
        float2 acc2 = make_float2(0.f, 0.f);
        uint32_t pp[25];
#pragma unroll
        for (int c = 0; c < 25; ++c) {
          const float2 d = __fadd2_rn(make_float2(sv[2 * c], sv[2 * c + 1]), nm);
          const float2 e = make_float2(fa_exp2(d.x), c == 24 ? 0.0f : fa_exp2(d.y));
          acc2 = __fadd2_rn(acc2, e);
          pp[c] = pack16(bf, e.x, e.y);
        }
        rsum = acc2.x + acc2.y;
        uint8_t* prow = hb + FA_QP + r * 128;
#pragma unroll
        for (int c = 0; c < 6; ++c)
          *reinterpret_cast<uint4*>(prow + ((c ^ (r & 7)) << 4)) = make_uint4(pp[4 * c], pp[4 * c + 1], pp[4 * c + 2], pp[4 * c + 3]);
        *reinterpret_cast<uint4*>(prow + ((6 ^ (r & 7)) << 4)) = make_uint4(pp[24], 0u, 0u, 0u);
        *reinterpret_cast<uint4*>(prow + ((7 ^ (r & 7)) << 4)) = make_uint4(0u, 0u, 0u, 0u);
        fence_proxy_async_smem();
        __syncwarp();
        if (lane == 0) mbar_arrive(&p_full[g]);
        if (quad == 0 && lane == 0) FA_TR(9, gh);
      }
      {
        mbar_wait(&o_full[g], ph);
        tc_fence_after();
        if (quad == 0 && lane == 0) FA_TR(10, gh);
        uint32_t o[32];
        tmem_ld_32x32(ts + uint32_t(wdx * 32), o);
        tmem_ld_wait();
        tc_fence_before();
        if (tok_off >= 0) {
          const float inv = 1.0f / rsum;
          const float2 inv2 = make_float2(inv, inv);
          const float4* bv4 = reinterpret_cast<const float4*>(bv_tab + h * 32);
          uint4* dst = reinterpret_cast<uint4*>(ctx + tok_off + h * 32);
#pragma unroll
          for (int q = 0; q < 4; ++q) {
            const float4 b0 = bv4[2 * q], b1 = bv4[2 * q + 1];
            const float2 c0 = __ffma2_rn(make_float2(__uint_as_float(o[8 * q]), __uint_as_float(o[8 * q + 1])), inv2, make_float2(b0.x, b0.y));
            const float2 c1 = __ffma2_rn(make_float2(__uint_as_float(o[8 * q + 2]), __uint_as_float(o[8 * q + 3])), inv2, make_float2(b0.z, b0.w));
            const float2 c2 = __ffma2_rn(make_float2(__uint_as_float(o[8 * q + 4]), __uint_as_float(o[8 * q + 5])), inv2, make_float2(b1.x, b1.y));
            const float2 c3 = __ffma2_rn(make_float2(__uint_as_float(o[8 * q + 6]), __uint_as_float(o[8 * q + 7])), inv2, make_float2(b1.z, b1.w));
            dst[q] = make_uint4(pack16(bf, c0.x, c0.y), pack16(bf, c1.x, c1.y), pack16(bf, c2.x, c2.y), pack16(bf, c3.x, c3.y));
          }
        }
      }
    }
  } else {
    asm volatile("setmaxnreg.dec.sync.aligned.u32 64;");
    constexpr int LPR = C / 16;
    constexpr int RPP = 32 / LPR;
    constexpr int CPL = 2;
    constexpr int NPASS = (FA_ROWS + FA_LN_WARPS * RPP - 1) / (FA_LN_WARPS * RPP);
    constexpr int GP = 2, GH = 2;
    constexpr int NB = (NPASS + GP - 1) / GP;
    const int ln = warp - FA_LN_WARP0;
    const int sub = lane / LPR, lr = lane % LPR;
    int* rowtab = reinterpret_cast<int*>(smem + Cfg::HB_OFF + 2 * FA_HB + FA_TAB);
    auto write_table = [&](int ti) {
      if (ln >= 4) return;
      const int q = ln * 32 + lane;
      int tok = -1;
      if (ti < my_tiles && q < FA_ROWS) {
        const int wg = 2 * (int(blockIdx.x) + ti * int(gridDim.x)) + q / FA_L, i = q % FA_L;
        if (wg < p.num_windows) {
          const int b = wg / p.nW, w = wg - b * p.nW;
          tok = b * p.g.N + win_row_to_token(p.g, w * FA_L + i);
        }
      }
      rowtab[(ti % 3) * 128 + q] = tok;
    };
    auto issue = [&](int ti, int pidx, float2 (&vv)[CPL][4], int& rr) {
      const int q = (pidx * FA_LN_WARPS + ln) * RPP + sub;
      int tok = -1;
      if (ti < my_tiles && pidx < NPASS && q < FA_ROWS) tok = rowtab[(ti % 3) * 128 + q];
      rr = tok >= 0 ? (q / FA_L) * 64 + q % FA_L : -1;
      const float* xr = p.x + static_cast<long long>(tok < 0 ? 0 : tok) * C;
#pragma unroll
      for (int tt = 0; tt < CPL; ++tt) {
        const int c = lr + LPR * tt;
        const float4 a0 = *reinterpret_cast<const float4*>(xr + c * 8), a1 = *reinterpret_cast<const float4*>(xr + c * 8 + 4);
        vv[tt][0] = make_float2(a0.x, a0.y); vv[tt][1] = make_float2(a0.z, a0.w);
        vv[tt][2] = make_float2(a1.x, a1.y); vv[tt][3] = make_float2(a1.z, a1.w);
      }
    };
    float2 v[GP][CPL][4];
    int rowq[GP];
    write_table(0);
    write_table(1);
    asm volatile("bar.sync 1, 256;" ::: "memory");
#pragma unroll
    for (int pp = 0; pp < GP; ++pp) issue(0, pp, v[pp], rowq[pp]);
    for (int ti = 0; ti < my_tiles; ++ti) {
      const int xb = XNB == 2 ? (ti & 1) : 0;
      uint8_t* xn = smem + Cfg::XN_OFF + uint32_t(xb) * Cfg::XN_TILE;
      if (ln == 0 && lane == 0) FA_TR(11, ti);
      if (ti > 0) {
        write_table(ti + 1);
        asm volatile("bar.sync 1, 256;" ::: "memory");
      }
      if (ln == 0 && lane == 0) FA_TR(12, ti);
      mbar_wait(&xn_empty[xb], (XNB == 2 ? ((ti >> 1) & 1) : (ti & 1)) ^ 1u);
      if (ln == 0 && lane == 0) FA_TR(13, ti);
#pragma unroll 1
      for (int bt = 0; bt < NB; ++bt) {
        const bool last = bt + 1 == NB;
        const int nti = last ? ti + 1 : ti, np0 = last ? 0 : (bt + 1) * GP;
#pragma unroll
        for (int g0 = 0; g0 < GP; g0 += GH) {
          if (bt * GP + g0 < NPASS) {
            float mean[GH], rstd[GH];
#pragma unroll
            for (int u = 0; u < GH; ++u) {
              float2 (&w)[CPL][4] = v[g0 + u];
              const float2 s2 = __fadd2_rn(__fadd2_rn(__fadd2_rn(w[0][0], w[0][1]), __fadd2_rn(w[0][2], w[0][3])),
                                           __fadd2_rn(__fadd2_rn(w[1][0], w[1][1]), __fadd2_rn(w[1][2], w[1][3])));
              mean[u] = s2.x + s2.y;
            }
#pragma unroll
            for (int o = LPR / 2; o > 0; o >>= 1)
#pragma unroll
              for (int u = 0; u < GH; ++u) mean[u] += __shfl_xor_sync(0xffffffffu, mean[u], o);
#pragma unroll
            for (int u = 0; u < GH; ++u) {
              float2 (&w)[CPL][4] = v[g0 + u];
              mean[u] *= 1.0f / float(C);
              const float2 nm = make_float2(-mean[u], -mean[u]);
              float2 qa = make_float2(0.f, 0.f), qb = make_float2(0.f, 0.f);
#pragma unroll
              for (int e = 0; e < 4; ++e) {
                w[0][e] = __fadd2_rn(w[0][e], nm); qa = __ffma2_rn(w[0][e], w[0][e], qa);
                w[1][e] = __fadd2_rn(w[1][e], nm); qb = __ffma2_rn(w[1][e], w[1][e], qb);
              }
              rstd[u] = (qa.x + qa.y) + (qb.x + qb.y);
            }
#pragma unroll
            for (int o = LPR / 2; o > 0; o >>= 1)
#pragma unroll
              for (int u = 0; u < GH; ++u) rstd[u] += __shfl_xor_sync(0xffffffffu, rstd[u], o);
#pragma unroll
            for (int u = 0; u < GH; ++u) {
              float2 (&w)[CPL][4] = v[g0 + u];
              const float rs = rsqrtf(rstd[u] * (1.0f / float(C)) + p.eps);
              const float2 rs2 = make_float2(rs, rs);
              const int rr = rowq[g0 + u];
              const int ra = rr < 0 ? 0 : rr;
#pragma unroll
              for (int tt = 0; tt < CPL; ++tt) {
                const int c = lr + LPR * tt;
                float2 y[4];
#pragma unroll
                for (int e = 0; e < 4; ++e) y[e] = __fmul2_rn(w[tt][e], rs2);
                uint4 pk;
                pk.x = Half16<T16>::pack(y[0].x, y[0].y); pk.y = Half16<T16>::pack(y[1].x, y[1].y);
                pk.z = Half16<T16>::pack(y[2].x, y[2].y); pk.w = Half16<T16>::pack(y[3].x, y[3].y);
                if (rr >= 0) *reinterpret_cast<uint4*>(xn + (c >> 3) * FA_SLAB + ra * 128 + (((c & 7) ^ (ra & 7)) << 4)) = pk;
              }
            }
          }
#pragma unroll
          for (int u = 0; u < GH; ++u) issue(nti, np0 + g0 + u, v[g0 + u], rowq[g0 + u]);
        }
      }
      fence_proxy_async_smem();
      __syncwarp();
      if (ln == 0 && lane == 0) FA_TR(14, ti);
      if (lane == 0) {
        mbar_arrive(&xn_full[xb]);
        if (ln == 0) *ln_done = ti + 1;
      }
    }
  }

  tc_fence_before();
  __syncthreads();
  if (warp == 1) tmem_dealloc(tmem_base, 512);
}

template <int FMT, int C>
static int launch_fa(const CUtensorMap& tmW, const FaParams& p, cudaStream_t stream) {
  using Cfg = FaCfg<C>;
  auto kern = swin_attn_fused_kernel<FMT, C>;
  CSVIT_CUDA(cudaFuncSetAttribute(kern, cudaFuncAttributeMaxDynamicSharedMemorySize, int(Cfg::SMEM)));
  const int tiles = (p.num_windows + 1) / 2;
  const int ctas = tiles < num_sms() ? tiles : num_sms();
  CSVIT_CUDA(launch_pdl(kern, dim3(ctas), dim3(FA_THREADS), Cfg::SMEM, stream, tmW, p));
  return 0;
}

int launch_swin_attn_fused(const float* x, float eps, const void* wqkv_h, const float* bqkv_h,
                           const void* bias_op, void* ctx, int dtype, int B, int H, int W, int C, int heads, int ws, int shift,
                           cudaStream_t stream) {
  CSVIT_REQUIRE(dtype == DT_BF16 || dtype == DT_F16, "swin_attn_fused: 16-bit operand formats only");
  CSVIT_REQUIRE(C == 128 || C == 256, "swin_attn_fused: C=%d not in {128, 256}", C);
  CSVIT_REQUIRE(ws == 7 && C == heads * 32, "swin_attn_fused: window 7 / head_dim 32 only (ws=%d C=%d heads=%d)", ws, C, heads);
  CSVIT_REQUIRE(H % ws == 0 && W % ws == 0 && shift >= 0 && shift < ws, "swin_attn_fused: bad geometry %dx%d shift %d", H, W, shift);
  CSVIT_REQUIRE((reinterpret_cast<uintptr_t>(x) & 15) == 0 && (reinterpret_cast<uintptr_t>(ctx) & 15) == 0 &&
                    (reinterpret_cast<uintptr_t>(bqkv_h) & 15) == 0,
                "swin_attn_fused: operands must be 16-byte aligned");
  const int nW = (H / ws) * (W / ws);
  const long long windows = static_cast<long long>(B) * nW;
  if (windows <= 0) return 0;
  CSVIT_REQUIRE(windows < (1ll << 30), "swin_attn_fused: too many windows");
  FaParams p{};
  p.x = x; p.eps = eps; p.bqkv = bqkv_h; p.bias = bias_op; p.ctx = ctx;
  p.num_windows = static_cast<int>(windows); p.nW = nW;
  p.qscale = 1.4426950408889634f * 0.17677669529663687f;
  p.g = make_geom(H, W, ws, shift);
  CUtensorMap tmW;
  if (int e = make_tmap(&tmW, wqkv_h, C, 3ll * C, C, dtype, 96, true)) return e;
  const bool bf = dtype == DT_BF16;
  if (C == 128) return bf ? launch_fa<1, 128>(tmW, p, stream) : launch_fa<0, 128>(tmW, p, stream);
  return bf ? launch_fa<1, 256>(tmW, p, stream) : launch_fa<0, 256>(tmW, p, stream);
}

}

#ifdef CSVIT_FA_TRACE
extern "C" __attribute__((visibility("default"))) int csvit_debug_fa_trace(long long* host_out) {
  return int(cudaMemcpyFromSymbol(host_out, csvit::fa_trace_buf, sizeof(long long) * 16 * 256));
}
#endif
```

cs-vit_b200/csrc/common.cuh:

```cuda
#pragma once
#include <cuda.h>
#include <cuda_bf16.h>
#include <cuda_fp16.h>
#include <cuda_runtime.h>
#include <stdint.h>
#include <stdio.h>

namespace csvit {

struct WinGeom {
  int H, W;
  int ws;
  int shift;
  int nWx;
  int L;
  int N;
};

__host__ __device__ inline WinGeom make_geom(int H, int W, int ws, int shift) {
  WinGeom g;
  g.H = H; g.W = W; g.ws = ws; g.shift = shift;
  g.nWx = W / ws; g.L = ws * ws; g.N = H * W;
  return g;
}

__host__ __device__ inline int win_row_to_token(const WinGeom& g, int r) {
  int w = r / g.L, i = r - w * g.L;
  int wy = w / g.nWx, wx = w - wy * g.nWx;
  int iy = i / g.ws, ix = i - iy * g.ws;
  int y = wy * g.ws + iy + g.shift; if (y >= g.H) y -= g.H;
  int x = wx * g.ws + ix + g.shift; if (x >= g.W) x -= g.W;
  return y * g.W + x;
}

__host__ __device__ inline int win_token_to_row(const WinGeom& g, int t) {
  int y = t / g.W, x = t - y * g.W;
  int ys = y - g.shift; if (ys < 0) ys += g.H;
  int xs = x - g.shift; if (xs < 0) xs += g.W;
  int wy = ys / g.ws, wx = xs / g.ws;
  return (wy * g.nWx + wx) * g.L + (ys - wy * g.ws) * g.ws + (xs - wx * g.ws);
}

__host__ __device__ inline int win_region(const WinGeom& g, int w, int i) {
  int wy = w / g.nWx, wx = w - wy * g.nWx;
  int iy = i / g.ws, ix = i - iy * g.ws;
  int p = wy * g.ws + iy, q = wx * g.ws + ix;
  int rp = p < g.H - g.ws ? 0 : (p < g.H - g.shift ? 1 : 2);
  int rq = q < g.W - g.ws ? 0 : (q < g.W - g.shift ? 1 : 2);
  return 3 * rp + rq;
}

__host__ __device__ inline int rel_pos_index(int ws, int i, int j) {
  int iy = i / ws, ix = i - iy * ws, jy = j / ws, jx = j - jy * ws;
  return (iy - jy + ws - 1) * (2 * ws - 1) + (ix - jx + ws - 1);
}

__host__ __device__ inline int merge_src_token(int W, int Y, int X, int q) {
  int dy = q & 1, dx = q >> 1;
  return (2 * Y + dy) * W + (2 * X + dx);
}

__device__ __forceinline__ float gelu_erf(float x) {
  return 0.5f * x * (1.0f + erff(x * 0.70710678118654752440f));
}

__device__ __forceinline__ uint32_t pack_bf16x2(float lo, float hi) {
  __nv_bfloat162 v = __floats2bfloat162_rn(lo, hi);
  return *reinterpret_cast<uint32_t*>(&v);
}

__device__ __forceinline__ uint32_t pack_f16x2(float lo, float hi) {
  __half2 v = __floats2half2_rn(lo, hi);
  return *reinterpret_cast<uint32_t*>(&v);
}
template <typename T> struct Half16;
template <> struct Half16<__nv_bfloat16> {
  static __device__ __forceinline__ uint32_t pack(float lo, float hi) { return pack_bf16x2(lo, hi); }
  static __device__ __forceinline__ __nv_bfloat16 from(float v) { return __float2bfloat16_rn(v); }
  static __device__ __forceinline__ float to(__nv_bfloat16 v) { return __bfloat162float(v); }
};
template <> struct Half16<__half> {
  static __device__ __forceinline__ uint32_t pack(float lo, float hi) { return pack_f16x2(lo, hi); }
  static __device__ __forceinline__ __half from(float v) { return __float2half_rn(v); }
  static __device__ __forceinline__ float to(__half v) { return __half2float(v); }
};

__device__ __forceinline__ float warp_sum(float v) {
#pragma unroll
  for (int o = 16; o > 0; o >>= 1) v += __shfl_xor_sync(0xffffffffu, v, o);
  return v;
}
__device__ __forceinline__ float warp_max(float v) {
#pragma unroll
  for (int o = 16; o > 0; o >>= 1) v = fmaxf(v, __shfl_xor_sync(0xffffffffu, v, o));
  return v;
}

__device__ __forceinline__ uint32_t smem_u32(const void* p) {
  return static_cast<uint32_t>(__cvta_generic_to_shared(p));
}

__device__ __forceinline__ void mbar_init(uint64_t* bar, uint32_t count) {
  asm volatile("mbarrier.init.shared::cta.b64 [%0], %1;" ::"r"(smem_u32(bar)), "r"(count) : "memory");
}
__device__ __forceinline__ void fence_mbar_init() {
  asm volatile("fence.mbarrier_init.release.cluster;" ::: "memory");
}
__device__ __forceinline__ void fence_proxy_async_smem() {
  asm volatile("fence.proxy.async.shared::cta;" ::: "memory");
}
__device__ __forceinline__ void mbar_arrive_expect_tx(uint64_t* bar, uint32_t bytes) {
  asm volatile("mbarrier.arrive.expect_tx.shared::cta.b64 _, [%0], %1;" ::"r"(smem_u32(bar)), "r"(bytes) : "memory");
}
__device__ __forceinline__ void mbar_arrive(uint64_t* bar) {
  asm volatile("mbarrier.arrive.shared::cta.b64 _, [%0];" ::"r"(smem_u32(bar)) : "memory");
}
__device__ __forceinline__ bool mbar_try_wait(uint64_t* bar, uint32_t parity) {
  uint32_t ok;
  asm volatile(
      "{\n\t.reg .pred p;\n\t"
      "mbarrier.try_wait.parity.shared::cta.b64 p, [%1], %2;\n\t"
      "selp.u32 %0, 1, 0, p;\n\t}"
      : "=r"(ok)
      : "r"(smem_u32(bar)), "r"(parity)
      : "memory");
  return ok != 0;
}
__device__ __forceinline__ uint64_t globaltimer_ns() {
  uint64_t t;
  asm volatile("mov.u64 %0, %%globaltimer;" : "=l"(t));
  return t;
}
__device__ __forceinline__ bool mbar_test_wait(uint64_t* bar, uint32_t parity) {
  uint32_t ok;
  asm volatile(
      "{\n\t.reg .pred p;\n\t"
      "mbarrier.test_wait.parity.shared::cta.b64 p, [%1], %2;\n\t"
      "selp.u32 %0, 1, 0, p;\n\t}"
      : "=r"(ok)
      : "r"(smem_u32(bar)), "r"(parity)
      : "memory");
  return ok != 0;
}
__device__ __forceinline__ void mbar_wait(uint64_t* bar, uint32_t parity) {
  if (mbar_try_wait(bar, parity)) return;
  uint32_t spins = 0;
  while (!mbar_try_wait(bar, parity)) {
    if (++spins > (1u << 26)) __trap();
  }
}

__device__ __forceinline__ void prefetch_tmap(const CUtensorMap* t) {
  asm volatile("prefetch.tensormap [%0];" ::"l"(reinterpret_cast<uint64_t>(t)) : "memory");
}
__device__ __forceinline__ void tma_load_2d(void* smem_dst, const CUtensorMap* tmap, uint64_t* bar, int x, int y) {
  asm volatile(
      "cp.async.bulk.tensor.2d.shared::cluster.global.mbarrier::complete_tx::bytes [%0], [%1, {%3, %4}], [%2];"
      ::"r"(smem_u32(smem_dst)), "l"(reinterpret_cast<uint64_t>(tmap)), "r"(smem_u32(bar)), "r"(x), "r"(y)
      : "memory");
}

__device__ __forceinline__ void tma_load_2d_mc(void* smem_dst, const CUtensorMap* tmap, uint64_t* bar, int x, int y, uint16_t cta_mask) {
  asm volatile(
      "cp.async.bulk.tensor.2d.shared::cluster.global.mbarrier::complete_tx::bytes.multicast::cluster [%0], [%1, {%3, %4}], [%2], %5;"
      ::"r"(smem_u32(smem_dst)), "l"(reinterpret_cast<uint64_t>(tmap)), "r"(smem_u32(bar)), "r"(x), "r"(y), "h"(cta_mask)
      : "memory");
}
__device__ __forceinline__ void tma_store_2d(const CUtensorMap* tmap, const void* smem_src, int x, int y) {
  asm volatile("cp.async.bulk.tensor.2d.global.shared::cta.bulk_group [%0, {%2, %3}], [%1];"
               ::"l"(reinterpret_cast<uint64_t>(tmap)), "r"(smem_u32(smem_src)), "r"(x), "r"(y) : "memory");
}
__device__ __forceinline__ void tma_reduce_add_2d(const CUtensorMap* tmap, const void* smem_src, int x, int y) {
  asm volatile("cp.reduce.async.bulk.tensor.2d.global.shared::cta.add.tile.bulk_group [%0, {%2, %3}], [%1];"
               ::"l"(reinterpret_cast<uint64_t>(tmap)), "r"(smem_u32(smem_src)), "r"(x), "r"(y) : "memory");
}
__device__ __forceinline__ void red_add_f32x4(float* p, float4 v) {
  asm volatile("red.global.add.v4.f32 [%0], {%1, %2, %3, %4};" ::"l"(p), "f"(v.x), "f"(v.y), "f"(v.z), "f"(v.w) : "memory");
}
__device__ __forceinline__ void tma_store_commit() { asm volatile("cp.async.bulk.commit_group;" ::: "memory"); }
__device__ __forceinline__ void tma_store_wait_read0() { asm volatile("cp.async.bulk.wait_group.read 0;" ::: "memory"); }
__device__ __forceinline__ void tma_store_wait_all() { asm volatile("cp.async.bulk.wait_group 0;" ::: "memory"); }

__device__ __forceinline__ uint32_t cluster_ctarank() {
  uint32_t r;
  asm volatile("mov.u32 %0, %%cluster_ctarank;" : "=r"(r));
  return r;
}
__device__ __forceinline__ void cluster_sync_all() {
  asm volatile("barrier.cluster.arrive.release.aligned;\n\tbarrier.cluster.wait.acquire.aligned;" ::: "memory");
}

#ifdef CSVIT_PDL_NO_TRIGGER
__device__ __forceinline__ void griddep_launch() {}
#else
__device__ __forceinline__ void griddep_launch() { asm volatile("griddepcontrol.launch_dependents;" ::: "memory"); }
#endif
__device__ __forceinline__ void griddep_wait() { asm volatile("griddepcontrol.wait;" ::: "memory"); }

__device__ __forceinline__ bool fa_elect_one() {
  uint32_t pred;
  asm volatile("{\n\t.reg .pred p;\n\telect.sync _|p, 0xffffffff;\n\tselp.u32 %0, 1, 0, p;\n\t}" : "=r"(pred));
  return pred != 0;
}

__device__ __forceinline__ void tc_fence_before() { asm volatile("tcgen05.fence::before_thread_sync;" ::: "memory"); }
__device__ __forceinline__ void tc_fence_after() { asm volatile("tcgen05.fence::after_thread_sync;" ::: "memory"); }

__device__ __forceinline__ void tmem_alloc(uint32_t* smem_dst, uint32_t ncols) {
  asm volatile("tcgen05.alloc.cta_group::1.sync.aligned.shared::cta.b32 [%0], %1;" ::"r"(smem_u32(smem_dst)), "r"(ncols) : "memory");
  asm volatile("tcgen05.relinquish_alloc_permit.cta_group::1.sync.aligned;" ::: "memory");
}
__device__ __forceinline__ void tmem_dealloc(uint32_t taddr, uint32_t ncols) {
  asm volatile("tcgen05.dealloc.cta_group::1.sync.aligned.b32 %0, %1;" ::"r"(taddr), "r"(ncols) : "memory");
}

template <bool kTF32>
__device__ __forceinline__ void umma_ss(uint32_t tmem_d, uint64_t adesc, uint64_t bdesc, uint32_t idesc, uint32_t accumulate) {
  if constexpr (kTF32) {
    asm volatile(
        "{\n\t.reg .pred p;\n\tsetp.ne.b32 p, %4, 0;\n\t"
        "tcgen05.mma.cta_group::1.kind::tf32 [%0], %1, %2, %3, p;\n\t}"
        ::"r"(tmem_d), "l"(adesc), "l"(bdesc), "r"(idesc), "r"(accumulate)
        : "memory");
  } else {
    asm volatile(
        "{\n\t.reg .pred p;\n\tsetp.ne.b32 p, %4, 0;\n\t"
        "tcgen05.mma.cta_group::1.kind::f16 [%0], %1, %2, %3, p;\n\t}"
        ::"r"(tmem_d), "l"(adesc), "l"(bdesc), "r"(idesc), "r"(accumulate)
        : "memory");
  }
}
__device__ __forceinline__ void umma_commit(uint64_t* bar) {
  asm volatile("tcgen05.commit.cta_group::1.mbarrier::arrive::one.shared::cluster.b64 [%0];" ::"r"(smem_u32(bar)) : "memory");
}

__device__ __forceinline__ void umma_commit_mc(uint64_t* bar, uint16_t cta_mask) {
  asm volatile("tcgen05.commit.cta_group::1.mbarrier::arrive::one.shared::cluster.multicast::cluster.b64 [%0], %1;"
               ::"r"(smem_u32(bar)), "h"(cta_mask) : "memory");
}

__device__ __forceinline__ uint32_t mapa_u32(uint32_t smem_addr, uint32_t rank) {
  uint32_t r;
  asm volatile("mapa.shared::cluster.u32 %0, %1, %2;" : "=r"(r) : "r"(smem_addr), "r"(rank));
  return r;
}
__device__ __forceinline__ void mbar_arrive_expect_tx_cluster(uint32_t cluster_bar_addr, uint32_t bytes) {
  asm volatile("mbarrier.arrive.expect_tx.shared::cluster.b64 _, [%0], %1;" ::"r"(cluster_bar_addr), "r"(bytes) : "memory");
}
__device__ __forceinline__ void mbar_arrive_cluster(uint32_t cluster_bar_addr) {
  asm volatile("mbarrier.arrive.shared::cluster.b64 _, [%0];" ::"r"(cluster_bar_addr) : "memory");
}
__device__ __forceinline__ void tma_load_2d_pair(void* smem_dst, const CUtensorMap* tmap, uint32_t cluster_bar_addr, int x, int y) {
  asm volatile(
      "cp.async.bulk.tensor.2d.cta_group::2.shared::cluster.global.mbarrier::complete_tx::bytes [%0], [%1, {%3, %4}], [%2];"
      ::"r"(smem_u32(smem_dst)), "l"(reinterpret_cast<uint64_t>(tmap)), "r"(cluster_bar_addr), "r"(x), "r"(y)
      : "memory");
}
__device__ __forceinline__ void tmem_alloc_pair(uint32_t* smem_dst, uint32_t ncols) {
  asm volatile("tcgen05.alloc.cta_group::2.sync.aligned.shared::cta.b32 [%0], %1;" ::"r"(smem_u32(smem_dst)), "r"(ncols) : "memory");
  asm volatile("tcgen05.relinquish_alloc_permit.cta_group::2.sync.aligned;" ::: "memory");
}
__device__ __forceinline__ void tmem_dealloc_pair(uint32_t taddr, uint32_t ncols) {
  asm volatile("tcgen05.dealloc.cta_group::2.sync.aligned.b32 %0, %1;" ::"r"(taddr), "r"(ncols) : "memory");
}
__device__ __forceinline__ void umma_ss_pair(uint32_t tmem_d, uint64_t adesc, uint64_t bdesc, uint32_t idesc, uint32_t accumulate) {
  asm volatile(
      "{\n\t.reg .pred p;\n\tsetp.ne.b32 p, %4, 0;\n\t"
      "tcgen05.mma.cta_group::2.kind::f16 [%0], %1, %2, %3, p;\n\t}"
      ::"r"(tmem_d), "l"(adesc), "l"(bdesc), "r"(idesc), "r"(accumulate)
      : "memory");
}
__device__ __forceinline__ void umma_commit_pair(uint64_t* bar, uint16_t cta_mask) {
  asm volatile("tcgen05.commit.cta_group::2.mbarrier::arrive::one.shared::cluster.multicast::cluster.b64 [%0], %1;"
               ::"r"(smem_u32(bar)), "h"(cta_mask) : "memory");
}

__device__ __forceinline__ void tmem_ld_32x32(uint32_t taddr, uint32_t (&r)[32]) {
  asm volatile(
      "tcgen05.ld.sync.aligned.32x32b.x32.b32 "
      "{%0, %1, %2, %3, %4, %5, %6, %7, %8, %9, %10, %11, %12, %13, %14, %15, "
      "%16, %17, %18, %19, %20, %21, %22, %23, %24, %25, %26, %27, %28, %29, %30, %31}, [%32];"
      : "=r"(r[0]), "=r"(r[1]), "=r"(r[2]), "=r"(r[3]), "=r"(r[4]), "=r"(r[5]), "=r"(r[6]), "=r"(r[7]),
        "=r"(r[8]), "=r"(r[9]), "=r"(r[10]), "=r"(r[11]), "=r"(r[12]), "=r"(r[13]), "=r"(r[14]), "=r"(r[15]),
        "=r"(r[16]), "=r"(r[17]), "=r"(r[18]), "=r"(r[19]), "=r"(r[20]), "=r"(r[21]), "=r"(r[22]), "=r"(r[23]),
        "=r"(r[24]), "=r"(r[25]), "=r"(r[26]), "=r"(r[27]), "=r"(r[28]), "=r"(r[29]), "=r"(r[30]), "=r"(r[31])
      : "r"(taddr)
      : "memory");
}
__device__ __forceinline__ void tmem_ld_wait() { asm volatile("tcgen05.wait::ld.sync.aligned;" ::: "memory"); }

__device__ __forceinline__ uint64_t make_sw128_kmajor_desc(uint32_t smem_addr) {
  uint64_t d = 0;
  d |= static_cast<uint64_t>((smem_addr & 0x3FFFFu) >> 4);
  d |= static_cast<uint64_t>(1) << 16;
  d |= static_cast<uint64_t>(1024 >> 4) << 32;
  d |= static_cast<uint64_t>(1) << 46;
  d |= static_cast<uint64_t>(2) << 61;
  return d;
}

__host__ __device__ constexpr uint32_t make_idesc(uint32_t fmt, int M, int N) {
  return (1u << 4)
         | (fmt << 7)
         | (fmt << 10)
         | (0u << 15) | (0u << 16)
         | (static_cast<uint32_t>(N >> 3) << 17) | (static_cast<uint32_t>(M >> 4) << 24);
}

}
```

cs-vit_b200/csrc/gemm.cu:

```cuda
#include <cudaTypedefs.h>

#include "errors.h"
#include <cstdlib>
#include "gemm.cuh"

namespace csvit {


template <int BN>
struct TcCfg {
  static constexpr int STAGES = BN == 256 ? 3 : 5;
  static constexpr uint32_t A_BYTES = kBM * 128;
  static constexpr uint32_t B_BYTES = BN * 128;
  static constexpr uint32_t STAGE_BYTES = A_BYTES + B_BYTES;
  static constexpr uint32_t TMEM_COLS = 2 * BN <= 256 ? 256 : 512;
  static constexpr uint32_t TILES_BYTES = STAGES * STAGE_BYTES;
  static constexpr uint32_t STG_BYTES = 2 * kEpiWarps * kStageBufBytes;
  static constexpr size_t SMEM = 1024 + size_t(TILES_BYTES) + STG_BYTES + 256;
};

template <int BN, int FMT, int CS>
__global__ void __launch_bounds__(kGemmThreads, 1)
gemm_tc_kernel(const __grid_constant__ CUtensorMap tmA, const __grid_constant__ CUtensorMap tmB,
               const __grid_constant__ CUtensorMap tmC, const __grid_constant__ CUtensorMap tmR, int K, EpiParams ep) {
// ... 46 lines not shown
  const uint32_t tmem_base = *tmem_slot;
  griddep_launch();
  griddep_wait();

  if (warp == 0) {
    if (lane == 0) {
      int s = 0; uint32_t ph = 0;
      for (int ct = cluster_id; ct < num_ctiles; ct += num_clusters) {
        const int mg = ct / num_n, n_blk = ct - mg * num_n;
        const int m_blk = mg * CS + rank;
        for (int kb = 0; kb < num_kb; ++kb) {
          mbar_wait(&empty[s], ph ^ 1u);
          mbar_arrive_expect_tx(&full[s], Cfg::STAGE_BYTES);
          uint8_t* sa = tiles + size_t(s) * Cfg::STAGE_BYTES;
          tma_load_2d(sa, &tmA, &full[s], kb * BK, m_blk * kBM);
          if constexpr (CS == 1) {
            tma_load_2d(sa + Cfg::A_BYTES, &tmB, &full[s], kb * BK, n_blk * BN);
          } else {
            tma_load_2d_mc(sa + Cfg::A_BYTES + rank * B_SLICE_ROWS * 128, &tmB, &full[s], kb * BK,
                           n_blk * BN + rank * B_SLICE_ROWS, kMask);
          }
          if (++s == STAGES) { s = 0; ph ^= 1u; }
        }
      }
    }
  } else if (warp == 1) {
    {
      constexpr uint32_t idesc = make_idesc(uint32_t(FMT), kBM, BN);
      int s = 0; uint32_t ph = 0;
      int as = 0; uint32_t aph = 0;
      for (int ct = cluster_id; ct < num_ctiles; ct += num_clusters) {
        mbar_wait(&tempty[as], aph ^ 1u);
        tc_fence_after();
        const uint32_t d_tmem = tmem_base + uint32_t(as * BN);
        for (int kb = 0; kb < num_kb; ++kb) {
          mbar_wait(&full[s], ph);
          tc_fence_after();
          if (fa_elect_one()) {
            const uint32_t sa = base + uint32_t(s) * Cfg::STAGE_BYTES;
            const uint64_t adesc = make_sw128_kmajor_desc(sa);
            const uint64_t bdesc = make_sw128_kmajor_desc(sa + Cfg::A_BYTES);
#pragma unroll
            for (int k = 0; k < 4; ++k)
              umma_ss<TF32>(d_tmem, adesc + uint64_t(2 * k), bdesc + uint64_t(2 * k), idesc, (kb | k) ? 1u : 0u);
            if constexpr (CS == 1) umma_commit(&empty[s]);
            else umma_commit_mc(&empty[s], kMask);
            if (kb == num_kb - 1) umma_commit(&tfull[as]);
          }
          __syncwarp();
          if (++s == STAGES) { s = 0; ph ^= 1u; }
        }
        if (++as == 2) { as = 0; aph ^= 1u; }
      }
    }
  } else {
    const int e = warp - 2;
    const int quad = warp & 3;
    const int half = e >> 2;
    uint8_t* stg = staging + e * 2 * kStageBufBytes;
    uint32_t stg_sel = 0, rph = 0;
    int as = 0; uint32_t aph = 0;
    for (int ct = cluster_id; ct < num_ctiles; ct += num_clusters) {
      const int mg = ct / num_n, n_blk = ct - mg * num_n;
      const int m_blk = mg * CS + rank;
      {
        const int nct = ct + num_clusters;
        if (ct == cluster_id) prefetch_resid_tile<BN>(ep, m_blk, n_blk, quad, half, lane);
        if (nct < num_ctiles) prefetch_resid_tile<BN>(ep, (nct / num_n) * CS + rank, nct % num_n, quad, half, lane);
      }
      epilogue_tile<BN>(ep, &tmC, stg, tmem_base + uint32_t(as * BN), &tfull[as], aph, m_blk, n_blk, quad, half, lane, 2, &stg_sel,
                        &tmR, rbar + 2 * e, &rph);
      tc_fence_before();
      __syncwarp();
      if (lane == 0) mbar_arrive(&tempty[as]);
      if (++as == 2) { as = 0; aph ^= 1u; }
    }
    if ((ep.tma_store || ep.tma_f32) && lane == 0) tma_store_wait_all();
  }

  tc_fence_before();
  __syncthreads();
  if constexpr (CS > 1) cluster_sync_all();
  if (warp == 1) tmem_dealloc(tmem_base, Cfg::TMEM_COLS);
}

__global__ void __launch_bounds__(256)
gemm_simt_f32_kernel(const float* __restrict__ A, long long lda, const float* __restrict__ W, long long ldw, int K, EpiParams ep) {
  __shared__ float As[16][64 + 4];
  __shared__ float Ws[16][64 + 4];
  const int tx = threadIdx.x & 15, ty = threadIdx.x >> 4;
  const int m0 = blockIdx.y * 64, n0 = blockIdx.x * 64;
  float acc[4][4] = {};
  for (int k0 = 0; k0 < K; k0 += 16) {
    for (int i = threadIdx.x; i < 64 * 16; i += 256) {
      int r = i >> 4, k = i & 15;
      int gm = m0 + r, gn = n0 + r, gk = k0 + k;
      As[k][r] = (gm < ep.M && gk < K) ? A[gm * lda + gk] : 0.0f;
      Ws[k][r] = (gn < ep.N && gk < K) ? W[gn * ldw + gk] : 0.0f;
    }
    __syncthreads();
#pragma unroll
    for (int k = 0; k < 16; ++k) {
      float a[4], b[4];
#pragma unroll
      for (int i = 0; i < 4; ++i) { a[i] = As[k][ty * 4 + i]; b[i] = Ws[k][tx * 4 + i]; }
#pragma unroll
      for (int i = 0; i < 4; ++i)
#pragma unroll
        for (int j = 0; j < 4; ++j) acc[i][j] = fmaf(a[i], b[j], acc[i][j]);
    }
    __syncthreads();
  }
#pragma unroll
  for (int i = 0; i < 4; ++i) {
    int row = m0 + ty * 4 + i;
    if (row >= ep.M) continue;
    long long orow = epi_out_row(ep, row);
#pragma unroll
    for (int j = 0; j < 4; ++j) {
      int col = n0 + tx * 4 + j;
      if (col < ep.N) epi_store_scalar(ep, orow, col, acc[i][j]);
    }
  }
}

static PFN_cuTensorMapEncodeTiled_v12000 get_tmap_encoder() {
  static PFN_cuTensorMapEncodeTiled_v12000 fn = nullptr;
  if (!fn) {
    void* p = nullptr;
    cudaDriverEntryPointQueryResult q;
    if (cudaGetDriverEntryPoint("cuTensorMapEncodeTiled", &p, cudaEnableDefault, &q) == cudaSuccess &&
        q == cudaDriverEntryPointSuccess)
      fn = reinterpret_cast<PFN_cuTensorMapEncodeTiled_v12000>(p);
  }
  return fn;
}

int make_tmap(CUtensorMap* tm, const void* ptr, long long ld, long long rows, long long cols, int dtype, int box_rows,
                     bool as_tf32) {
  auto enc = get_tmap_encoder();
  if (!enc) return set_error("cuTensorMapEncodeTiled entry point not available (driver too old?)");
  const size_t es = dtype_size(dtype);
  if ((reinterpret_cast<uintptr_t>(ptr) & 15) || ((ld * es) & 15))
    return set_error("GEMM operand must be 16-byte aligned with a 16-byte-multiple row pitch (ptr=%p ld=%lld)", ptr, ld);
  cuuint64_t gdim[2] = {cuuint64_t(cols), cuuint64_t(rows)};
  cuuint64_t gstr[1] = {cuuint64_t(ld * es)};
  cuuint32_t box[2] = {cuuint32_t(128 / es), cuuint32_t(box_rows)};
  cuuint32_t estr[2] = {1, 1};
  const CUtensorMapDataType tdt = dtype == DT_BF16 ? CU_TENSOR_MAP_DATA_TYPE_BFLOAT16
                                  : (dtype == DT_F16 ? CU_TENSOR_MAP_DATA_TYPE_FLOAT16
                                                     : (as_tf32 ? CU_TENSOR_MAP_DATA_TYPE_TFLOAT32 : CU_TENSOR_MAP_DATA_TYPE_FLOAT32));
  CUresult r = enc(tm, tdt, 2, const_cast<void*>(ptr), gdim, gstr, box, estr, CU_TENSOR_MAP_INTERLEAVE_NONE,
                   CU_TENSOR_MAP_SWIZZLE_128B, CU_TENSOR_MAP_L2_PROMOTION_L2_256B, CU_TENSOR_MAP_FLOAT_OOB_FILL_NONE);
  if (r != CUDA_SUCCESS)
    return set_error("cuTensorMapEncodeTiled failed with CUresult %d (rows=%lld cols=%lld ld=%lld)", int(r), rows, cols, ld);
  return 0;
}

int red_add_mode() {
  static const int m = [] { const char* e = getenv("CSVIT_RED_ADD"); return (e && e[0] >= '0' && e[0] <= '2') ? e[0] - '0' : 1; }();
  return m;
}
static const bool g_tma_f32 = [] { const char* e = getenv("CSVIT_TMA_F32"); return !(e && e[0] == '0'); }();
static int g_num_sms = 0;
int num_sms() {
  if (!g_num_sms) {
    int dev = 0;
    cudaGetDevice(&dev);
    cudaDeviceGetAttribute(&g_num_sms, cudaDevAttrMultiProcessorCount, dev);
    if (g_num_sms <= 0) g_num_sms = 148;
  }
  return g_num_sms;
}

template <int BN, int FMT, int CS>
static int launch_tc(const CUtensorMap& tmA, const CUtensorMap& tmB, const CUtensorMap& tmC, const CUtensorMap& tmR, int K,
                     const EpiParams& ep, int max_ctas, cudaStream_t stream) {
  using Cfg = TcCfg<BN>;
  static DeviceOnce once;
  auto kern = gemm_tc_kernel<BN, FMT, CS>;
  if (once.first()) {
    CSVIT_CUDA(cudaFuncSetAttribute(kern, cudaFuncAttributeMaxDynamicSharedMemorySize, int(Cfg::SMEM)));
  }
  const int num_m = (ep.M + kBM - 1) / kBM, num_n = (ep.N + BN - 1) / BN;
  const int ctiles = ((num_m + CS - 1) / CS) * num_n;
  int ctas = max_ctas > 0 ? max_ctas : num_sms();
  int clusters = ctas / CS;
  if (clusters > ctiles) clusters = ctiles;
  if (clusters < 1) clusters = 1;
  cudaLaunchConfig_t cfg{};
  cfg.gridDim = dim3(unsigned(clusters * CS));
  cfg.blockDim = dim3(kGemmThreads);
  cfg.dynamicSmemBytes = Cfg::SMEM;
  cfg.stream = stream;
  cudaLaunchAttribute attr[2];
  attr[0].id = cudaLaunchAttributeClusterDimension;
  attr[0].val.clusterDim.x = CS;
  attr[0].val.clusterDim.y = 1;
  attr[0].val.clusterDim.z = 1;
  attr[1].id = cudaLaunchAttributeProgrammaticStreamSerialization;
  attr[1].val.programmaticStreamSerializationAllowed = 1;
  cfg.attrs = attr;
  cfg.numAttrs = pdl_enabled() ? 2 : 1;
  CSVIT_CUDA(cudaLaunchKernelEx(&cfg, kern, tmA, tmB, tmC, tmR, K, ep));
  return 0;
}

template <int BN, int FMT>
static int launch_tc_cs(int cs, const CUtensorMap& a, const CUtensorMap& b, const CUtensorMap& c, const CUtensorMap& r, int K,
                        const EpiParams& ep, int max_ctas, cudaStream_t st) {
  if (cs == 4) return launch_tc<BN, FMT, 4>(a, b, c, r, K, ep, max_ctas, st);
  if (cs == 2) return launch_tc<BN, FMT, 2>(a, b, c, r, K, ep, max_ctas, st);
  return launch_tc<BN, FMT, 1>(a, b, c, r, K, ep, max_ctas, st);
}

static thread_local int g_last_gemm_kernel = 0;
int last_gemm_kernel() { return g_last_gemm_kernel; }

int launch_gemm(const void* A, long long lda, const void* W, long long ldw, int in_dtype, int M, int N, int K,
                const EpiParams& ep_in, int impl, const GemmTuning& tune, cudaStream_t stream) {
  g_last_gemm_kernel = 0;
  if (M <= 0 || N <= 0 || K <= 0) return 0;
  EpiParams ep = ep_in;
  ep.M = M; ep.N = N;
  const size_t oes = dtype_size(ep.out_dtype);
  ep.vec_ok = (N % 8 == 0) && ((ep.ldo * oes) % 16 == 0) && ((reinterpret_cast<uintptr_t>(ep.out) & 15) == 0) &&
              (!ep.resid || ((ep.ldr % 4 == 0) && (reinterpret_cast<uintptr_t>(ep.resid) & 15) == 0)) &&
              (!ep.bias || (reinterpret_cast<uintptr_t>(ep.bias) & 15) == 0);
  ep.tma_store = 0;
  if (impl == GEMM_SIMT) {
    if (in_dtype != DT_F32) return set_error("SIMT GEMM takes fp32 operands only");
    dim3 grid((N + 63) / 64, (M + 63) / 64);
    gemm_simt_f32_kernel<<<grid, 256, 0, stream>>>(static_cast<const float*>(A), lda, static_cast<const float*>(W), ldw, K, ep);
    CSVIT_CUDA(cudaGetLastError());
    g_last_gemm_kernel = 3;
    return 0;
  }
  int BN = 256;
  if (N <= 128 || (N % 256 != 0 && N % 128 == 0)) BN = 128;
  const int num_m = (M + kBM - 1) / kBM;
  if (BN == 256 && num_m * ((N + 255) / 256) < num_sms()) BN = 128;
  int cs = tune.cluster;
  if (cs == 0) cs = 1;
  if (cs != 1 && cs != 2 && cs != 4) return set_error("gemm: cluster size %d not in {1,2,4}", cs);
  const bool can_tma_store = ep.out_dtype != DT_F32 && !ep.resid && ep.map_mode == ROWMAP_IDENTITY && (N % 64 == 0) &&
                             ep.vec_ok;
  ep.tma_store = (tune.tma_store != 0 && can_tma_store) ? 1 : 0;
  ep.tma_f32 = (tune.tma_store != 0 && ep.out_dtype == DT_F32 && ep.map_mode == ROWMAP_IDENTITY && ep.vec_ok && (N % 32 == 0) && N >= 256 &&
                ((ep.ldo * 4) % 16 == 0) && (!ep.resid || (ep.ldr * 4) % 16 == 0) && g_tma_f32) ? 1 : 0;
  ep.coalesced = (!ep.tma_store && !ep.tma_f32 && tune.tma_store != 0 && ep.out_dtype == DT_F32 && ep.vec_ok && (N % 32 == 0)) ? 1 : 0;
  ep.red_add = 0;
  if ((ep.tma_f32 ? red_add_mode() != 0 : (ep.coalesced && red_add_mode() == 1)) && ep.resid && static_cast<const void*>(ep.resid) == ep.out &&
      ep.ldr == ep.ldo) {
    ep.red_add = 1;
    ep.resid = nullptr;
  }
  const bool pair_ok = in_dtype != DT_F32 && N % 256 == 0 && num_m * (N / 256) >= 2 * num_sms();
  if (pair_ok && tune.pair != 0) {
    g_last_gemm_kernel = 1;
    return launch_gemm_pair(A, lda, W, ldw, in_dtype, M, N, K, ep, tune, stream);
  }
  g_last_gemm_kernel = 2;
  CUtensorMap tmA, tmB, tmC, tmR;
  if (int e = make_tmap(&tmA, A, lda, M, K, in_dtype, kBM, true)) return e;
  if (int e = make_tmap(&tmB, W, ldw, N, K, in_dtype, BN / cs, true)) return e;
  if (ep.tma_store || ep.tma_f32) {
    if (int e = make_tmap(&tmC, ep.out, ep.ldo, M, N, ep.out_dtype, 32, false)) return e;
  } else {
    tmC = tmA;
  }
  tmR = tmC;
  if (ep.tma_f32 && ep.resid)
    if (int e = make_tmap(&tmR, ep.resid, ep.ldr, M, N, DT_F32, 32, false)) return e;
  const int mc = tune.max_ctas;
  if (BN == 256) {
    if (in_dtype == DT_F32) return launch_tc_cs<256, 2>(cs, tmA, tmB, tmC, tmR, K, ep, mc, stream);
    if (in_dtype == DT_BF16) return launch_tc_cs<256, 1>(cs, tmA, tmB, tmC, tmR, K, ep, mc, stream);
    return launch_tc_cs<256, 0>(cs, tmA, tmB, tmC, tmR, K, ep, mc, stream);
  }
  if (in_dtype == DT_F32) return launch_tc_cs<128, 2>(cs, tmA, tmB, tmC, tmR, K, ep, mc, stream);
  if (in_dtype == DT_BF16) return launch_tc_cs<128, 1>(cs, tmA, tmB, tmC, tmR, K, ep, mc, stream);
  return launch_tc_cs<128, 0>(cs, tmA, tmB, tmC, tmR, K, ep, mc, stream);
}

}
```

cs-vit_b200/csrc/gemm.cuh:

```cuda
#pragma once
#include "common.cuh"

namespace csvit {

enum : int { ACT_NONE = 0, ACT_GELU = 1, ACT_RELU = 2 };
enum : int { ROWMAP_IDENTITY = 0, ROWMAP_WINDOW = 1 };
enum : int { DT_F32 = 0, DT_BF16 = 1, DT_F16 = 2 };
__host__ __device__ inline int dtype_size(int dt) { return dt == DT_F32 ? 4 : 2; }

struct EpiParams {
  const float* bias;
  const float* resid;
  void* out;
  long long ldo, ldr;
  int out_dtype;
  int act;
  int M, N;
  int vec_ok;
  int tma_store;
  int coalesced;
  int tma_f32;
  long long* trace;
  int red_add;
  int map_mode;
// ... 271 lines not shown
        const uint32_t t_addr = tmem_tile + (uint32_t(quad * 32) << 16);
        if (ep.tma_store) {
  #pragma unroll 1
          for (int c = 0; c < BN / 2; c += 64) {
            const int col_local = half * (BN / 2) + c;
            const int gcol = n_blk * BN + col_local;
            if (gcol >= ep.N) break;
            uint32_t pk[32];
            uint32_t r2[2][32];
            tmem_ld_32x32(t_addr + uint32_t(col_local), r2[0]);
            tmem_ld_32x32(t_addr + uint32_t(col_local + 32), r2[1]);
            tmem_ld_wait();
  #pragma unroll
            for (int hh = 0; hh < 2; ++hh) {
              if (ep.act == ACT_GELU) {
                epi_bias_gelu_pack32(ep.bias, bf, gcol + 32 * hh, r2[hh], pk + 16 * hh);
              } else {
                float v[32];
    #pragma unroll
                for (int j = 0; j < 32; ++j) v[j] = __uint_as_float(r2[hh][j]);
                epi_bias_act32(ep, gcol + 32 * hh, v);
    #pragma unroll
                for (int j = 0; j < 16; ++j) pk[16 * hh + j] = pack16(bf, v[2 * j], v[2 * j + 1]);
              }
            }
            uint8_t* sbuf = stg;
            if (nbuf == 2) {
              sbuf = stg + (*stg_sel & 1u) * kStageBufBytes;
              *stg_sel ^= 1u;
              if (lane == 0) asm volatile("cp.async.bulk.wait_group.read 1;" ::: "memory");
            } else if (lane == 0) {
              tma_store_wait_read0();
            }
            __syncwarp();
  #pragma unroll
            for (int q = 0; q < 8; ++q)
              *reinterpret_cast<uint4*>(sbuf + lane * 128 + ((q ^ (lane & 7)) << 4)) =
                  make_uint4(pk[4 * q], pk[4 * q + 1], pk[4 * q + 2], pk[4 * q + 3]);
            fence_proxy_async_smem();
            __syncwarp();
            if (lane == 0 && m_blk * kBM + quad * 32 < ep.M) {
              tma_store_2d(tmC, sbuf, gcol, m_blk * kBM + quad * 32);
              tma_store_commit();
            }
          }
        } else if (ep.coalesced) {
          float* outp = reinterpret_cast<float*>(ep.out);
  #pragma unroll 1
          for (int c = 0; c < BN / 2; c += 32) {
            const int col_local = half * (BN / 2) + c;
            const int gcol = n_blk * BN + col_local;
            if (gcol >= ep.N) break;
            uint32_t r[32];
            tmem_ld_32x32(t_addr + uint32_t(col_local), r);
            tmem_ld_wait();
            float v[32];
  #pragma unroll
            for (int j = 0; j < 32; ++j) v[j] = __uint_as_float(r[j]);
            epi_bias_act32(ep, gcol, v);
  #pragma unroll
            for (int k = 0; k < 8; ++k)
              *reinterpret_cast<float4*>(stg + lane * 128 + ((k ^ (lane & 7)) << 4)) =
                  make_float4(v[4 * k], v[4 * k + 1], v[4 * k + 2], v[4 * k + 3]);
            __syncwarp();
            float4 val[8];
  #pragma unroll
            for (int j = 0; j < 8; ++j) {
              const int i = 4 * j + (lane >> 3);
              const float4 t = *reinterpret_cast<const float4*>(stg + i * 128 + ((q ^ (i & 7)) << 4));
              val[j] = make_float4(t.x + res[j].x, t.y + res[j].y, t.z + res[j].z, t.w + res[j].w);
            }
            if (c + 32 < BN / 2) load_resid(gcol + 32);
            if (ep.red_add) {
  #pragma unroll
              for (int j = 0; j < 8; ++j)
                if (ok8[j]) red_add_f32x4(outp + orow8[j] * ep.ldo + gcol + 4 * q, val[j]);
            } else {
  #pragma unroll
              for (int j = 0; j < 8; ++j)
                if (ok8[j]) *reinterpret_cast<float4*>(outp + orow8[j] * ep.ldo + gcol + 4 * q) = val[j];
            }
            __syncwarp();
          }
        } else {
          const long long orow = row_ok ? epi_out_row(ep, row) : 0;
  #pragma unroll 1
          for (int c = 0; c < BN / 2; c += 32) {
            const int col_local = half * (BN / 2) + c;
            const int gcol = n_blk * BN + col_local;
            if (gcol >= ep.N) break;
            uint32_t r[32];
            tmem_ld_32x32(t_addr + uint32_t(col_local), r);
            tmem_ld_wait();
            if (row_ok) epi_store_chunk32(ep, orow, gcol, r);
          }
        }
}

template <int BN>
__device__ __forceinline__ void epilogue_tile16(const EpiParams& ep, const CUtensorMap* tmC, uint8_t* sbuf, uint32_t tmem_tile,
                                                uint64_t* tfull_bar, uint32_t aph, int m_blk, int n_blk, int quad, int part, int lane) {
  static_assert(BN == 256, "four 64-column parts");
  const bool bf = ep.out_dtype == DT_BF16;
  const int col_local = part * 64;
  const int gcol = n_blk * BN + col_local;
  mbar_wait(tfull_bar, aph);
  tc_fence_after();
  if (gcol >= ep.N) return;
  const uint32_t t_addr = tmem_tile + (uint32_t(quad * 32) << 16) + uint32_t(col_local);
  uint32_t r0[32], r1[32];
  tmem_ld_32x32(t_addr, r0);
  tmem_ld_32x32(t_addr + 32u, r1);
  if (lane == 0) tma_store_wait_read0();
  __syncwarp();
  tmem_ld_wait();
  auto step32 = [&](const uint32_t (&r)[32], int gc, int hh) {
    uint32_t pk[16];
    if (ep.act == ACT_GELU) {
      epi_bias_gelu_pack32(ep.bias, bf, gc, r, pk);
    } else {
      float v[32];
#pragma unroll
      for (int j = 0; j < 32; ++j) v[j] = __uint_as_float(r[j]);
      epi_bias_act32(ep, gc, v);
#pragma unroll
      for (int j = 0; j < 16; ++j) pk[j] = pack16(bf, v[2 * j], v[2 * j + 1]);
    }
#pragma unroll
    for (int q = 0; q < 4; ++q)
      *reinterpret_cast<uint4*>(sbuf + lane * 128 + (((4 * hh + q) ^ (lane & 7)) << 4)) =
          make_uint4(pk[4 * q], pk[4 * q + 1], pk[4 * q + 2], pk[4 * q + 3]);
  };
  step32(r0, gcol, 0);
  step32(r1, gcol + 32, 1);
  fence_proxy_async_smem();
  __syncwarp();
  if (lane == 0 && m_blk * kBM + quad * 32 < ep.M) {
    tma_store_2d(tmC, sbuf, gcol, m_blk * kBM + quad * 32);
    tma_store_commit();
  }
}

enum : int { GEMM_TC = 0, GEMM_SIMT = 1 };
int last_gemm_kernel();

struct GemmTuning {
  int max_ctas;
  int cluster;
  int tma_store;
  int pair;
};
int make_tmap(CUtensorMap* tm, const void* ptr, long long ld, long long rows, long long cols, int dtype, int box_rows,
              bool as_tf32);
int num_sms();
int red_add_mode();
int launch_gemm_pair(const void* A, long long lda, const void* W, long long ldw, int in_dtype, int M, int N, int K,
                     const EpiParams& ep, const GemmTuning& tune, cudaStream_t stream);
int launch_gemm(const void* A, long long lda, const void* W, long long ldw, int in_dtype, int M, int N, int K,
                const EpiParams& ep, int impl, const GemmTuning& tune, cudaStream_t stream);

}
```

cs-vit_b200/csrc/rowops.cuh:

```cuda
#pragma once
#include "common.cuh"
#include "gemm.cuh"

namespace csvit {

enum : int { LN_IDENTITY = 0, LN_WINDOW = 1, LN_MERGE2X2 = 2 };

int launch_layernorm(const float* x, const float* gamma, const float* beta, float eps, void* out, int out_dtype,
                     long long ldo, int rows, int C, int mode, const WinGeom& g, cudaStream_t stream);
int launch_affine_rows(const float* x, const float* scale, const float* shift, void* out, int out_dtype, long long rows,
                       int C, cudaStream_t stream);
int launch_patch_im2col(const float* img, void* out, int out_dtype, int B, int S, const float* mean3, const float* std3,
                        cudaStream_t stream);
int launch_window_index_map(int H, int W, int ws, int shift, int* out, cudaStream_t stream);
int launch_shift_mask(int H, int W, int ws, int shift, float* out, cudaStream_t stream);
int launch_rel_index(int ws, int* out, cudaStream_t stream);
int launch_merge_index_map(int H, int W, int* out, cudaStream_t stream);
int launch_expand_rel_bias(const float* table, float* out, int heads, int ws, cudaStream_t stream);

int launch_swin_attn_fused(const float* x, float eps, const void* wqkv_h, const float* bqkv_h,
                           const void* bias_op, void* ctx, int dtype, int B, int H, int W, int C, int heads, int ws, int shift,
                           cudaStream_t stream);

int launch_swin_attn_core(const void* qkv, long long ldq, const void* bias_log2, void* ctx, int dtype, int B, int H, int W, int C,
                          int heads, int ws, int shift, int token_order, int q_prescaled, cudaStream_t stream);

int launch_crop_resize(const void* frames, int frames_u8, int N, int H, int W, const float* boxes, float expansion, float* square_out,
                       float* out, int S, cudaStream_t stream);

int launch_rot6d_to_axis_angle(const float* d6, float* aa, long long n, cudaStream_t stream);
int launch_mano_fk(const float* pose, const float* betas, const float* root_norm, const float* v_template, const float* shapedirs,
                   const float* posedirs, const float* pose_mean, const float* j_regressor, const float* lbs_weights, const float* j_out,
                   const int* parents16, const int* edges40, int rodrigues_mode, float* joint_cam, float* verts_cam, float* root_transl,
                   int n, cudaStream_t stream);

int launch_allreduce_f32(void* const* bufs, void* const* flags, void* mc, long long n, int rank, int world, float scale, int ctas,
                         cudaStream_t stream);

int launch_mlp_fused(const void* xn, long long ldxn, const void* W1, long long ldw1, const float* b1, const void* W2,
                     long long ldw2, const float* b2, float* x, long long ldx, int dtype, int M, int C, cudaStream_t stream);

int launch_attention_simt(const void* q, const void* k, const void* v, void* out, int dtype, long long ldq, long long ldk,
                          long long ldv, long long ldo, int n_seq, int Lq, int S, int heads, float scale,
                          const float* bias, int mH, int mW, int mws, int mshift, cudaStream_t stream);

int launch_gemm_ex(const void* A, long long lda, int a_mn, const void* B, long long ldb, int b_mn, int in_dtype, int M, int N,
                   int K, void* out, long long ldo, int out_dtype, int accumulate, int impl, int split_k, cudaStream_t stream);

int launch_col_reduce(const void* a, int a_dtype, long long lda, const float* b, long long ldb, const float* center, int mode,
                      int rows, int C, int row_mode, const WinGeom& g, void* copy, int copy_dtype, long long ldc, float* s1,
                      float* s2, cudaStream_t stream);
int launch_transpose_f32(const float* src, long long lds, float* dst, long long ldd, int R, int C, cudaStream_t stream);
int launch_row_scale_add(const float* x, const float* y, const float* s, float* out, long long rows, int C, int group_rows,
                         cudaStream_t stream);
int launch_eltwise(int op, const void* a, const void* b, void* out, int dtype, long long n, cudaStream_t stream);
int launch_affine2_rows(const float* dy, const float* x, const float* a, const float* b, const float* c0, const float* resid,
                        float* out, long long rows, int C, cudaStream_t stream);
int launch_layernorm_bwd(const float* x, const void* dy, int dy_dtype, long long ldy, const float* gamma, float eps, int rows, int C,
                         int mode, const WinGeom& g, const float* dres, float* dx, float* dgamma, float* dbeta, cudaStream_t stream);
int launch_attention_bwd(const void* q, const void* k, const void* v, const void* dout, void* dq, void* dk, void* dv, int dtype,
                         long long ldq, long long ldk, long long ldv, long long ldo, long long lddq, long long lddk, long long lddv,
                         int n_seq, int Lq, int S, int heads, float scale, const float* bias, float* dbias, int mH, int mW, int mws,
                         int mshift, cudaStream_t stream);

int launch_swinv2_window_attention(const void* qkv, const float* bias_tab, const float* logit_scale, void* out, int dtype, int B, int H,
                                   int W, int C, int heads, int ws, int shift, int mask_repeat, int tok_order, cudaStream_t stream);
int launch_layernorm_post(const float* y, long long ldy, const float* resid, const float* gamma, const float* beta, float eps,
                          float* xo, void* copy, int copy_dtype, long long ldc, int copy_mode, int rows, int C, const WinGeom& g,
                          cudaStream_t stream);

int launch_swinv2_attn_tc(const void* qkv, long long ldq, const float* bias_log2, void* ctx, int dtype, int B, int H, int W, int C,
                          int heads, int shift, int mask_repeat, int token_order, cudaStream_t stream);

int launch_window_attention_bwd_mma(const void* qkv, const void* dout, void* dqkv, int dtype, const float* bias, float* dbias, int B,
                                    int H, int W, int C, int heads, int ws, int shift, cudaStream_t stream);

}
```

include/csvit.h:

```cpp
#ifndef CSVIT_H_
#define CSVIT_H_

#include <stdint.h>

#ifdef __cplusplus
extern "C" {
#endif

#define CSVIT_ABI_VERSION 11

#if defined(__GNUC__)
#define CSVIT_API __attribute__((visibility("default")))
#else
#define CSVIT_API
#endif

enum { CSVIT_F32 = 0, CSVIT_BF16 = 1, CSVIT_F16 = 2 };
enum { CSVIT_ACT_NONE = 0, CSVIT_ACT_GELU = 1, CSVIT_ACT_RELU = 2 };
enum { CSVIT_LN_IDENTITY = 0, CSVIT_LN_WINDOW = 1, CSVIT_LN_MERGE2X2 = 2 };
enum { CSVIT_GEMM_TENSORCORE = 0, CSVIT_GEMM_SIMT_FP32 = 1 };

CSVIT_API int csvit_abi_version(void);
CSVIT_API const char* csvit_last_error(void);

CSVIT_API int csvit_window_index_map(int H, int W, int ws, int shift, int32_t* out, void* stream);
CSVIT_API int csvit_shift_mask(int H, int W, int ws, int shift, float* out, void* stream);
CSVIT_API int csvit_rel_pos_index(int ws, int32_t* out, void* stream);
CSVIT_API int csvit_merge_index_map(int H, int W, int32_t* out, void* stream);

CSVIT_API int csvit_host_window_index_map(int H, int W, int ws, int shift, int32_t* out);
CSVIT_API int csvit_host_shift_mask(int H, int W, int ws, int shift, float* out);
CSVIT_API int csvit_host_rel_pos_index(int ws, int32_t* out);
CSVIT_API int csvit_host_merge_index_map(int H, int W, int32_t* out);

CSVIT_API int csvit_expand_rel_bias(const float* table, float* out, int heads, int ws, void* stream);

CSVIT_API int csvit_layernorm(const float* x, const float* gamma, const float* beta, float eps, void* out, int out_dtype,
                    long long ldo, int rows, int C, int mode, int H, int W, int ws, int shift, void* stream);

CSVIT_API int csvit_affine_rows(const float* x, const float* scale, const float* shift, void* out, int out_dtype,
                      long long rows, int C, void* stream);

CSVIT_API int csvit_patch_im2col(const float* img, void* out, int out_dtype, int B, int S, const float* mean3,
                       const float* std3, void* stream);

CSVIT_API int csvit_crop_resize(const void* frames, int frames_u8, int N, int H, int W, const float* boxes, float expansion_ratio,
                                float* square_boxes_out, float* out, int S, void* stream);

CSVIT_API int csvit_linear(const void* A, long long lda, const void* W, long long ldw, int in_dtype, int M, int N, int K,
                 const float* bias, int act, const float* resid, long long ldr, void* out, long long ldo,
                 int out_dtype, int scatter_H, int scatter_W, int scatter_ws, int scatter_shift, int impl,
                 void* stream);

CSVIT_API int csvit_mlp_fused(const void* xn, long long ldxn, const void* W1, long long ldw1, const float* b1, const void* W2,
                              long long ldw2, const float* b2, float* x, long long ldx, int dtype, int M, int C, void* stream);

CSVIT_API int csvit_last_gemm_kernel(void);

CSVIT_API int csvit_set_gemm_tuning(int cluster, int tma_store, int max_ctas, int pair);

CSVIT_API int csvit_window_attention(const void* qkv, const float* bias, void* out, int dtype, int B, int H, int W, int C,
                                     int heads, int ws, int shift, void* stream);

CSVIT_API int csvit_swin_attn_fused(const float* x, float eps, const void* wqkv_h, const float* bqkv_h,
                                    const void* bias_op, void* ctx, int dtype, int B, int H, int W, int C,
                                    int heads, int ws, int shift, void* stream);

CSVIT_API int csvit_swin_attn_core(const void* qkv, long long ldq, const void* bias_log2, void* ctx, int dtype, int B, int H,
                                   int W, int C, int heads, int ws, int shift, int token_order, int q_prescaled, void* stream);

CSVIT_API int csvit_rot6d_to_axis_angle(const float* d6, float* axis_angle, long long n, void* stream);

CSVIT_API int csvit_mano_fk(const float* pose, const float* betas, const float* root_norm, const float* v_template,
                            const float* shapedirs, const float* posedirs, const float* pose_mean, const float* j_regressor,
                            const float* lbs_weights, const float* j_regressor_out, const int* parents16, const int* edges40,
                            int rodrigues_mode, float* joint_cam, float* verts_cam, float* root_transl, int n, void* stream);

#define CSVIT_ALLREDUCE_FLAG_BYTES 4096
CSVIT_API int csvit_allreduce_f32(const void* const* bufs, const void* const* flags, void* multicast, long long n, int rank, int world,
                                  float scale, int ctas, void* stream);

CSVIT_API int csvit_swinv2_window_attention(const void* qkv, const float* bias_tab, const float* logit_scale, void* out,
                                            int dtype, int B, int H, int W, int C, int heads, int ws, int shift,
                                            int mask_repeat, int out_token_order, void* stream);

CSVIT_API int csvit_swinv2_qkv(const void* A, long long lda, const void* W, long long ldw, int dtype, int M, int C, int K,
                               const float* bias, const float* qscale_log2, void* out, long long ldo, void* stream);

CSVIT_API int csvit_swinv2_attn_tc(const void* qkv, long long ldq, const float* bias_log2, void* ctx, int dtype, int B, int H, int W,
                                   int C, int heads, int shift, int mask_repeat, int token_order, void* stream);

enum { CSVIT_COPY_NONE = 0, CSVIT_COPY_IDENTITY = 1, CSVIT_COPY_WINDOW = 2, CSVIT_COPY_MERGE2X2 = 3 };
CSVIT_API int csvit_layernorm_post(const float* y, long long ldy, const float* resid, const float* gamma, const float* beta,
                                   float eps, float* out, void* copy, int copy_dtype, long long ldc, int copy_mode, int rows,
                                   int C, int H, int W, int ws, int shift, void* stream);

CSVIT_API int csvit_attention(const void* q, const void* k, const void* v, void* out, int dtype, long long ldq, long long ldk,
                    long long ldv, long long ldo, int n_seq, int Lq, int S, int heads, float scale, void* stream);

CSVIT_API int csvit_gemm_ex(const void* A, long long lda, int a_mn, const void* B, long long ldb, int b_mn, int in_dtype, int M,
                            int N, int K, void* out, long long ldo, int out_dtype, int accumulate, int impl, int split_k,
                            void* stream);

CSVIT_API int csvit_transpose_f32(const float* src, long long lds, float* dst, long long ldd, int rows, int cols, void* stream);

enum { CSVIT_CR_SUM = 0, CSVIT_CR_CENTERED = 1, CSVIT_CR_DOT = 2 };
CSVIT_API int csvit_col_reduce(const void* a, int a_dtype, long long lda, const float* b, long long ldb, const float* center,
                               int mode, int rows, int C, int row_mode, int H, int W, int ws, int shift, void* copy,
                               int copy_dtype, long long ldc, float* s1, float* s2, void* stream);

CSVIT_API int csvit_row_scale_add(const float* x, const float* y, const float* s, float* out, long long rows, int C, int group_rows,
                                  void* stream);

enum { CSVIT_EW_GELU_FWD = 0, CSVIT_EW_GELU_BWD = 1, CSVIT_EW_RELU_BWD = 2 };
CSVIT_API int csvit_eltwise(int op, const void* a, const void* b, void* out, int dtype, long long n, void* stream);

CSVIT_API int csvit_affine2_rows(const float* dy, const float* x, const float* a, const float* b, const float* c0,
                                 const float* resid, float* out, long long rows, int C, void* stream);

CSVIT_API int csvit_layernorm_bwd(const float* x, const void* dy, int dy_dtype, long long ldy, const float* gamma, float eps,
                                  int rows, int C, int mode, int H, int W, int ws, int shift, const float* dres, float* dx,
                                  float* dgamma, float* dbeta, void* stream);

CSVIT_API int csvit_attention_bwd(const void* q, const void* k, const void* v, const void* dout, void* dq, void* dk, void* dv,
                                  int dtype, long long ldq, long long ldk, long long ldv, long long ldo, long long lddq,
                                  long long lddk, long long lddv, int n_seq, int Lq, int S, int heads, float scale,
                                  const float* bias, float* dbias, int mask_H, int mask_W, int mask_ws, int mask_shift,
                                  void* stream);

#ifdef __cplusplus
}
#endif
#endif
```

Before: 18360.

## Fuse attention output projection and residual add into the fused Swin attention kernel

For C=128 (stage 1 of Swin-B), the fused LN+QKV+window-attention kernel now also runs the output projection per head on tensor cores. It streams projection weight slices through a new TMA ring with 64B swizzle and accumulates the result into the fp32 residual x using bulk async reduce-add. This removes the separate linear launch and the round trip of the ctx tensor through global memory. In exchange it shrinks the QKV weight ring from 4 to 3 stages, reworks the TMEM column layout and adds more barriers. The reduce-add into x may also create atomic traffic contention.

```diff
diff --git a/cs-vit_b200/cs_vit/_lib.py b/cs-vit_b200/cs_vit/_lib.py
--- a/cs-vit_b200/cs_vit/_lib.py
+++ b/cs-vit_b200/cs_vit/_lib.py
@@ -27,8 +27,8 @@
                      c_longlong, c_void_p, c_longlong, c_int, c_int, c_int, c_int, c_int, c_int, c_void_p],
     "csvit_mlp_fused": [c_void_p, c_longlong, c_void_p, c_longlong, c_void_p, c_void_p, c_longlong, c_void_p, c_void_p,
                         c_longlong, c_int, c_int, c_int, c_void_p],
-    "csvit_swin_attn_fused": [c_void_p, c_float, c_void_p, c_void_p, c_void_p, c_void_p, c_int, c_int, c_int, c_int,
-                              c_int, c_int, c_int, c_int, c_void_p],
+    "csvit_swin_attn_fused": [c_void_p, c_float, c_void_p, c_void_p, c_void_p, c_void_p, c_void_p, c_void_p, c_int, c_int,
+                              c_int, c_int, c_int, c_int, c_int, c_int, c_void_p],
     "csvit_swin_attn_core": [c_void_p, c_longlong, c_void_p, c_void_p, c_int, c_int, c_int, c_int, c_int, c_int, c_int, c_int,
                              c_int, c_int, c_void_p],
     "csvit_crop_resize": [c_void_p, c_int, c_int, c_int, c_int, c_void_p, c_float, c_void_p, c_void_p, c_int, c_void_p],
diff --git a/cs-vit_b200/cs_vit/net/swin_b200.py b/cs-vit_b200/cs_vit/net/swin_b200.py
--- a/cs-vit_b200/cs_vit/net/swin_b200.py
+++ b/cs-vit_b200/cs_vit/net/swin_b200.py
@@ -90,6 +90,7 @@
         self.precision = precision
         self.fuse_attn = True
         self.fuse_attn_widths = ops.ATTN_FUSED_WIDTHS
+        self.fuse_attn_proj = os.environ.get("CSVIT_FA_PROJ", "1") != "0"
         self._drop_path_rand: List[torch.Tensor] = []
         self.fuse_mlp = True
         self.micro_batch = 0
@@ -184,8 +185,11 @@
                 wqkv_h, bqkv_h, bias_op = self._w(key + "attn_fused", src, lambda: ops.pack_attn_fused(
                     sa.query.weight, sa.key.weight, sa.value.weight, sa.query.bias, sa.key.bias, sa.value.bias,
                     sa.relative_position_bias_table, sa.relative_position_index, act, ln1.weight, ln1.bias))
-                ctx = ops.swin_attn_fused(x, eps, wqkv_h, bqkv_h, bias_op, B, H, W, heads, ws, shift)
-                ops.linear(ctx, wproj, bproj, resid=x, out=x, impl=impl)
+                if self.fuse_attn_proj and C in ops.ATTN_FUSED_PROJ_WIDTHS:
+                    ops.swin_attn_fused(x, eps, wqkv_h, bqkv_h, bias_op, B, H, W, heads, ws, shift, w_proj=wproj, b_proj=bproj)
+                else:
+                    ctx = ops.swin_attn_fused(x, eps, wqkv_h, bqkv_h, bias_op, B, H, W, heads, ws, shift)
+                    ops.linear(ctx, wproj, bproj, resid=x, out=x, impl=impl)
             else:
                 wqs, bqs = self._w(key + "wqkv_qs", qkv_src + bqkv_src, lambda: ops.pack_qkv_prescaled(
                     sa.query.weight, sa.key.weight, sa.value.weight, sa.query.bias, sa.key.bias, sa.value.bias, act))
diff --git a/cs-vit_b200/cs_vit/ops.py b/cs-vit_b200/cs_vit/ops.py
--- a/cs-vit_b200/cs_vit/ops.py
+++ b/cs-vit_b200/cs_vit/ops.py
@@ -206,6 +206,7 @@
 
 
 ATTN_FUSED_WIDTHS = (128, 256)
+ATTN_FUSED_PROJ_WIDTHS = (128,)
 _LOG2E = 1.4426950408889634
 
 
@@ -260,8 +261,9 @@
 
 def swin_attn_fused(x: torch.Tensor, eps: float, wqkv_h: torch.Tensor, bqkv_h: torch.Tensor,
                     bias_op: torch.Tensor, B: int, H: int, W: int, heads: int, ws: int, shift: int,
-                    out: Optional[torch.Tensor] = None) -> torch.Tensor:
-    _dev(x, wqkv_h, bqkv_h, bias_op, out)
+                    out: Optional[torch.Tensor] = None, w_proj: Optional[torch.Tensor] = None,
+                    b_proj: Optional[torch.Tensor] = None) -> torch.Tensor:
+    _dev(x, wqkv_h, bqkv_h, bias_op, out, w_proj, b_proj)
     if x.dtype != torch.float32 or not x.is_contiguous() or x.dim() != 2:
         raise ValueError("swin_attn_fused input must be contiguous float32 [B*H*W, C]")
     rows, C = x.shape
@@ -271,11 +273,24 @@
         raise ValueError("swin_attn_fused: wqkv_h must be contiguous 16-bit [3C, C]")
     if bqkv_h.dtype != torch.float32 or bqkv_h.numel() != 3 * C or bias_op.dtype != torch.float16 or tuple(bias_op.shape) != (heads * 49, 56) or not bias_op.is_contiguous():
         raise ValueError("swin_attn_fused: bqkv_h must be float32 [3C] and bias_op contiguous float16 [heads*49, 56]")
+    L = ws * ws
+    if w_proj is not None:
+        if C not in ATTN_FUSED_PROJ_WIDTHS or out is not None:
+            raise ValueError(f"swin_attn_fused: the out-projection form takes C in {ATTN_FUSED_PROJ_WIDTHS} and no `out` (C={C})")
+        if w_proj.dtype != wqkv_h.dtype or tuple(w_proj.shape) != (C, C) or not w_proj.is_contiguous():
+            raise ValueError("swin_attn_fused: w_proj must be contiguous [C, C] in the dtype of wqkv_h")
+        if b_proj is None or b_proj.dtype != torch.float32 or b_proj.numel() != C or not b_proj.is_contiguous():
+            raise ValueError("swin_attn_fused: b_proj must be contiguous float32 [C]")
+        _call("csvit_swin_attn_fused", x.data_ptr(), float(eps), wqkv_h.data_ptr(), bqkv_h.data_ptr(), bias_op.data_ptr(),
+              w_proj.data_ptr(), b_proj.data_ptr(), None, _code(wqkv_h.dtype), B, H, W, C, heads, ws, shift, _stream(),
+              flops=float(rows) * (8.0 * C * C + 4.0 * L * C), nbytes=float(rows) * C * 12.0)
+        return x
+    if b_proj is not None:
+        raise ValueError("swin_attn_fused: b_proj without w_proj")
     if out is None:
         out = torch.empty(rows, C, dtype=wqkv_h.dtype, device=x.device)
-    L = ws * ws
     _call("csvit_swin_attn_fused", x.data_ptr(), float(eps), wqkv_h.data_ptr(), bqkv_h.data_ptr(),
-          bias_op.data_ptr(), out.data_ptr(), _code(wqkv_h.dtype), B, H, W, C, heads, ws, shift, _stream(),
+          bias_op.data_ptr(), None, None, out.data_ptr(), _code(wqkv_h.dtype), B, H, W, C, heads, ws, shift, _stream(),
           flops=float(rows) * (6.0 * C * C + 4.0 * L * C), nbytes=float(rows) * C * 6.0)
     return out
 
diff --git a/cs-vit_b200/csrc/api.cu b/cs-vit_b200/csrc/api.cu
--- a/cs-vit_b200/csrc/api.cu
+++ b/cs-vit_b200/csrc/api.cu
@@ -164,11 +164,11 @@
   return 0;
 }
 
-int csvit_swin_attn_fused(const float* x, float eps, const void* wqkv_h, const float* bqkv_h,
-                          const void* bias_op, void* ctx, int dtype, int B, int H, int W, int C, int heads, int ws, int shift,
-                          void* stream) {
-  CSVIT_REQUIRE(x && wqkv_h && bqkv_h && bias_op && ctx, "swin_attn_fused: null operand");
-  return launch_swin_attn_fused(x, eps, wqkv_h, bqkv_h, bias_op, ctx, dtype, B, H, W, C, heads, ws, shift, S(stream));
+int csvit_swin_attn_fused(float* x, float eps, const void* wqkv_h, const float* bqkv_h, const void* bias_op,
+                          const void* w_proj, const float* b_proj, void* ctx, int dtype, int B, int H, int W, int C, int heads,
+                          int ws, int shift, void* stream) {
+  CSVIT_REQUIRE(x && wqkv_h && bqkv_h && bias_op, "swin_attn_fused: null operand");
+  return launch_swin_attn_fused(x, eps, wqkv_h, bqkv_h, bias_op, w_proj, b_proj, ctx, dtype, B, H, W, C, heads, ws, shift, S(stream));
 }
 
 int csvit_swin_attn_core(const void* qkv, long long ldq, const void* bias_log2, void* ctx, int dtype, int B, int H, int W, int C,
diff --git a/cs-vit_b200/csrc/attn_common.cuh b/cs-vit_b200/csrc/attn_common.cuh
--- a/cs-vit_b200/csrc/attn_common.cuh
+++ b/cs-vit_b200/csrc/attn_common.cuh
@@ -30,6 +30,15 @@
   d |= static_cast<uint64_t>(1024 >> 4) << 32;
   d |= static_cast<uint64_t>(1) << 46;
   d |= static_cast<uint64_t>(2) << 61;
+  return d;
+}
+__device__ __forceinline__ uint64_t fa_sw64_kmajor_desc(uint32_t smem_addr) {
+  uint64_t d = 0;
+  d |= static_cast<uint64_t>((smem_addr & 0x3FFFFu) >> 4);
+  d |= static_cast<uint64_t>(1) << 16;
+  d |= static_cast<uint64_t>(512 >> 4) << 32;
+  d |= static_cast<uint64_t>(1) << 46;
+  d |= static_cast<uint64_t>(4) << 61;
   return d;
 }
 __device__ __forceinline__ float fa_exp2(float x) {
diff --git a/cs-vit_b200/csrc/attn_fused.cu b/cs-vit_b200/csrc/attn_fused.cu
--- a/cs-vit_b200/csrc/attn_fused.cu
+++ b/cs-vit_b200/csrc/attn_fused.cu
@@ -14,27 +14,37 @@
 constexpr uint32_t FA_SLAB = 128 * 128;
 constexpr uint32_t FA_STAGE = 96 * 128;
 constexpr int FA_NBS = 2;
-constexpr int FA_NST = 4;
+constexpr int FA_NWP = 2;
 constexpr uint32_t FA_QP = 0, FA_K = 16384, FA_V = 24576, FA_HB = 32768;
 constexpr uint32_t FA_TM_SLOT = 160, FA_TM_S = 96;
+constexpr uint32_t FA_TM_OUT = 384;
 constexpr uint32_t FA_TAB = FA_K + 49 * 128;
 
-template <int C>
+template <int C, bool PROJ>
 struct FaCfg {
+  static_assert(!PROJ || C == 128, "the out-projection form is built for C = 128 only (TMEM budget, see the header)");
   static constexpr int KB = C / 64;
   static constexpr int HEADS = C / 32;
   static constexpr int XNB = C <= 128 ? 2 : 1;
+  static constexpr int NST = PROJ ? 3 : 4;
+  static constexpr int NACC = PROJ ? 2 : FA_NSLOT;
+  static constexpr uint32_t WP_STAGE = C * 64;
   static constexpr uint32_t XN_TILE = KB * FA_SLAB;
   static constexpr uint32_t XN_OFF = 0;
   static constexpr uint32_t RING_OFF = XNB * XN_TILE;
-  static constexpr uint32_t HB_OFF = RING_OFF + FA_NST * FA_STAGE;
+  static constexpr uint32_t WP_OFF = RING_OFF + NST * FA_STAGE;
+  static constexpr uint32_t HB_OFF = WP_OFF + (PROJ ? FA_NWP * WP_STAGE : 0);
   static constexpr uint32_t BIAS_OFF = HB_OFF + FA_NSLOT * FA_HB;
   static constexpr uint32_t BAR_OFF = BIAS_OFF + FA_NBS * FA_BIAS_STAGE;
   static constexpr size_t SMEM = 1024 + size_t(BAR_OFF) + 512;
+  static_assert(SMEM <= 232448, "shared memory budget");
+  static __device__ __forceinline__ uint32_t acc_col(int a) { return PROJ ? uint32_t(a) * 96u : uint32_t(a) * FA_TM_SLOT; }
+  static __device__ __forceinline__ uint32_t s_col(int g) { return PROJ ? 192u + uint32_t(g) * 64u : uint32_t(g) * FA_TM_SLOT + FA_TM_S; }
 };
 
 struct FaParams {
-  const float* x;
+  float* x;
+  const float* bproj;
   float eps;
   const float* bqkv;
   const void* bias;
@@ -52,19 +62,19 @@
 #define FA_TR(kind, idx) do { } while (0)
 #endif
 
-template <int FMT, int C>
+template <int FMT, int C, bool PROJ>
 __global__ void __launch_bounds__(FA_THREADS, 1)
-swin_attn_fused_kernel(const __grid_constant__ CUtensorMap tmW, FaParams p) {
-  using Cfg = FaCfg<C>;
+swin_attn_fused_kernel(const __grid_constant__ CUtensorMap tmW, const __grid_constant__ CUtensorMap tmP, FaParams p) {
+  using Cfg = FaCfg<C, PROJ>;
   using T16 = typename std::conditional<FMT == 1, __nv_bfloat16, __half>::type;
-  constexpr int KB = Cfg::KB, HEADS = Cfg::HEADS, XNB = Cfg::XNB;
+  constexpr int KB = Cfg::KB, HEADS = Cfg::HEADS, XNB = Cfg::XNB, NST = Cfg::NST, NACC = Cfg::NACC;
   extern __shared__ uint8_t smem_raw[];
   const uint32_t base = (smem_u32(smem_raw) + 1023u) & ~1023u;
   uint8_t* smem = smem_raw + (base - smem_u32(smem_raw));
   uint64_t* bars = reinterpret_cast<uint64_t*>(smem + Cfg::BAR_OFF);
   uint64_t* w_full = bars;
-  uint64_t* w_empty = bars + FA_NST;
-  uint64_t* xn_full = bars + 2 * FA_NST;
+  uint64_t* w_empty = bars + 4;
+  uint64_t* xn_full = bars + 8;
   uint64_t* xn_empty = xn_full + 2;
   uint64_t* acc_full = xn_full + 4;
   uint64_t* acc_empty = acc_full + FA_NSLOT;
@@ -74,11 +84,18 @@
   uint64_t* o_full = p_full + FA_NSLOT;
   uint64_t* b_full = o_full + FA_NSLOT;
   uint64_t* b_empty = b_full + FA_NBS;
-  uint32_t* tmem_slot = reinterpret_cast<uint32_t*>(b_empty + FA_NBS);
+  uint64_t* pw_full = b_empty + FA_NBS;
+  uint64_t* pw_empty = pw_full + FA_NWP;
+  uint64_t* c_full = pw_empty + FA_NWP;
+  uint64_t* c_empty = c_full + FA_NSLOT;
+  uint64_t* out_full = c_empty + FA_NSLOT;
+  uint64_t* out_empty = out_full + 1;
+  uint32_t* tmem_slot = reinterpret_cast<uint32_t*>(out_empty + 1);
   volatile int* ln_done = reinterpret_cast<volatile int*>(tmem_slot + 1);
   float* bq_tab = reinterpret_cast<float*>(smem + Cfg::HB_OFF + FA_TAB);
   float* bv_tab = reinterpret_cast<float*>(smem + Cfg::HB_OFF + FA_HB + FA_TAB);
-  static_assert(C * 4 <= 15 * 128, "bias table does not fit the padding key rows");
+  float* bp_tab = bq_tab + C;
+  static_assert((PROJ ? 2 : 1) * C * 4 <= 15 * 128, "bias table does not fit the padding key rows");
 
   const int warp = threadIdx.x >> 5, lane = threadIdx.x & 31;
   const int num_tiles = (p.num_windows + 1) >> 1;
@@ -90,13 +107,17 @@
     reinterpret_cast<uint4*>(smem + Cfg::HB_OFF)[i] = make_uint4(0u, 0u, 0u, 0u);
   if (threadIdx.x == 0) {
     prefetch_tmap(&tmW);
-    for (int s = 0; s < FA_NST; ++s) { mbar_init(&w_full[s], 1); mbar_init(&w_empty[s], 1); }
+    if (PROJ) prefetch_tmap(&tmP);
+    for (int s = 0; s < NST; ++s) { mbar_init(&w_full[s], 1); mbar_init(&w_empty[s], 1); }
+    for (int s = 0; s < FA_NWP; ++s) { mbar_init(&pw_full[s], 1); mbar_init(&pw_empty[s], 1); }
+    mbar_init(out_full, 1); mbar_init(out_empty, 4);
     for (int b = 0; b < 2; ++b) { mbar_init(&xn_full[b], FA_LN_WARPS); mbar_init(&xn_empty[b], 1); }
     for (int b = 0; b < FA_NBS; ++b) { mbar_init(&b_full[b], 1); mbar_init(&b_empty[b], 4); }
     for (int b = 0; b < FA_NSLOT; ++b) {
       mbar_init(&acc_full[b], 1); mbar_init(&acc_empty[b], 4);
       mbar_init(&qkv_full[b], 4); mbar_init(&s_full[b], 1);
       mbar_init(&p_full[b], 4); mbar_init(&o_full[b], 1);
+      mbar_init(&c_full[b], 4); mbar_init(&c_empty[b], 1);
     }
     *ln_done = 0;
     fence_mbar_init();
@@ -106,6 +127,7 @@
   for (int c = threadIdx.x; c < C; c += FA_THREADS) {
     bq_tab[c] = p.bqkv[(c >> 5) * 96 + (c & 31)];
     bv_tab[c] = p.bqkv[(c >> 5) * 96 + 64 + (c & 31)];
+    if (PROJ) bp_tab[c] = p.bproj[c];
   }
   fence_proxy_async_smem();
   tc_fence_before();
@@ -120,16 +142,24 @@
   if (warp == 0) {
     if (lane == 0) {
       int s = 0; uint32_t ph = 0;
-      int wq = 0, bq = 0;
-      while (wq < total * KB || bq < total) {
+      int wq = 0, bq = 0, pq = PROJ ? 0 : total;
+      while (wq < total * KB || bq < total || pq < total) {
         bool moved = false;
         if (wq < total * KB && mbar_test_wait(&w_empty[s], ph ^ 1u)) {
           const int h = (wq / KB) % HEADS, kb = wq % KB;
           mbar_arrive_expect_tx(&w_full[s], 96 * 128);
           tma_load_2d(smem + Cfg::RING_OFF + size_t(s) * FA_STAGE, &tmW, &w_full[s], kb * 64, h * 96);
           if (wq < 128) FA_TR(15, 128 + wq);
-          if (++s == FA_NST) { s = 0; ph ^= 1u; }
+          if (++s == NST) { s = 0; ph ^= 1u; }
           ++wq; moved = true;
+        }
+        if (pq < total) {
+          const int ps = pq % FA_NWP;
+          if (mbar_test_wait(&pw_empty[ps], ((uint32_t(pq) / FA_NWP) & 1u) ^ 1u)) {
+            mbar_arrive_expect_tx(&pw_full[ps], Cfg::WP_STAGE);
+            tma_load_2d(smem + Cfg::WP_OFF + uint32_t(ps) * Cfg::WP_STAGE, &tmP, &pw_full[ps], (pq % HEADS) * 32, 0);
+            ++pq; moved = true;
+          }
         }
         if (bq < total) {
           const int bs = bq % FA_NBS;
@@ -149,8 +179,8 @@
       int s = 0; uint32_t ph = 0;
       uint32_t xn_addr = 0;
       auto issue_g = [&](int gh) {
-        const int h = gh % HEADS, ti = gh / HEADS, sl = gh % FA_NSLOT;
-        const uint32_t n = uint32_t(gh / FA_NSLOT);
+        const int h = gh % HEADS, ti = gh / HEADS, sl = gh % NACC;
+        const uint32_t n = uint32_t(gh / NACC);
         const int xb = XNB == 2 ? (ti & 1) : 0;
         if (h == 0) {
           mbar_wait(&xn_full[xb], XNB == 2 ? ((ti >> 1) & 1) : (ti & 1));
@@ -159,7 +189,7 @@
         mbar_wait(&acc_empty[sl], (n & 1u) ^ 1u);
         tc_fence_after();
         if (lane == 0) FA_TR(0, gh);
-        const uint32_t d_tmem = tmem_base + uint32_t(sl) * FA_TM_SLOT;
+        const uint32_t d_tmem = tmem_base + Cfg::acc_col(sl);
 #pragma unroll 1
         for (int kb = 0; kb < KB; ++kb) {
           mbar_wait(&w_full[s], ph);
@@ -172,12 +202,12 @@
             for (int k = 0; k < 4; ++k) umma_ss<false>(d_tmem, adesc + uint64_t(2 * k), bdesc + uint64_t(2 * k), idesc_g, (kb | k) ? 1u : 0u);
             umma_commit(&w_empty[s]);
             if (kb == KB - 1) {
-              umma_commit(&acc_full[sl]);
+              umma_commit(&acc_full[gh % FA_NSLOT]);
               if (h == HEADS - 1) umma_commit(&xn_empty[xb]);
             }
           }
           __syncwarp();
-          if (++s == FA_NST) { s = 0; ph ^= 1u; }
+          if (++s == NST) { s = 0; ph ^= 1u; }
         }
         if (lane == 0) FA_TR(1, gh);
       };
@@ -195,7 +225,7 @@
           if (lane == 0) FA_TR(2, gh);
           if (fa_elect_one()) {
             const uint32_t hb = base + Cfg::HB_OFF + uint32_t(sl) * FA_HB;
-            const uint32_t d_tmem = tmem_base + uint32_t(sl) * FA_TM_SLOT + FA_TM_S;
+            const uint32_t d_tmem = tmem_base + Cfg::s_col(sl);
             const uint64_t pdesc = make_sw128_kmajor_desc(hb + FA_QP);
             const uint64_t vdesc = fa_mnmajor_desc(hb + FA_V);
 #pragma unroll
@@ -211,7 +241,7 @@
           if (lane == 0) FA_TR(3, gs);
           if (fa_elect_one()) {
             const uint32_t hb = base + Cfg::HB_OFF + uint32_t(sl) * FA_HB;
-            const uint32_t d_tmem = tmem_base + uint32_t(sl) * FA_TM_SLOT + FA_TM_S;
+            const uint32_t d_tmem = tmem_base + Cfg::s_col(sl);
             const uint64_t qdesc = make_sw128_kmajor_desc(hb + FA_QP), kdesc = make_sw128_kmajor_desc(hb + FA_K);
 #pragma unroll
             for (int k = 0; k < 4; ++k) umma_ss<false>(d_tmem, qdesc + uint64_t(2 * k), kdesc + uint64_t(2 * k), idesc_s, k ? 1u : 0u);
@@ -223,17 +253,44 @@
       }
     }
   } else {
-    const int pl = lane;
-    for (int ti = 1; ti < my_tiles; ++ti) {
-      while (*ln_done + 3 < ti) __nanosleep(2000);
+    auto prefetch_tile = [&](int ti) {
       const int t = int(blockIdx.x) + ti * int(gridDim.x);
-      for (int q = pl; q < FA_ROWS; q += 32) {
+      for (int q = lane; q < FA_ROWS; q += 32) {
         const int wg = 2 * t + q / FA_L, i = q % FA_L;
         if (wg >= p.num_windows) continue;
         const int b = wg / p.nW, w = wg - b * p.nW;
         const char* src = reinterpret_cast<const char*>(p.x + (static_cast<long long>(b) * p.g.N + win_row_to_token(p.g, w * FA_L + i)) * C);
 #pragma unroll
         for (int o = 0; o < C * 4; o += 128) asm volatile("prefetch.global.L2 [%0];" ::"l"(src + o));
+      }
+    };
+    if constexpr (PROJ) {
+      constexpr uint32_t idesc_p = make_idesc(uint32_t(FMT), 128, C);
+      int ps = 0, pf = 1;
+      uint32_t pph = 0;
+      for (int gh = 0; gh < total; ++gh) {
+        const int ti = gh / HEADS, h = gh - ti * HEADS, sl = gh % FA_NSLOT;
+        for (; pf < my_tiles && *ln_done + 3 >= pf; ++pf) prefetch_tile(pf);
+        if (h == 0 && ti > 0) mbar_wait(out_empty, uint32_t(ti - 1) & 1u);
+        mbar_wait(&pw_full[ps], pph);
+        mbar_wait(&c_full[sl], uint32_t(gh / FA_NSLOT) & 1u);
+        tc_fence_after();
+        if (fa_elect_one()) {
+          const uint64_t adesc = make_sw128_kmajor_desc(base + Cfg::HB_OFF + uint32_t(sl) * FA_HB + FA_QP);
+          const uint64_t bdesc = fa_sw64_kmajor_desc(base + Cfg::WP_OFF + uint32_t(ps) * Cfg::WP_STAGE);
+#pragma unroll
+          for (int k = 0; k < 2; ++k) umma_ss<false>(tmem_base + FA_TM_OUT, adesc + uint64_t(2 * k), bdesc + uint64_t(2 * k), idesc_p, (h | k) ? 1u : 0u);
+          umma_commit(&c_empty[sl]);
+          umma_commit(&pw_empty[ps]);
+          if (h == HEADS - 1) umma_commit(out_full);
+        }
+        __syncwarp();
+        if (++ps == FA_NWP) { ps = 0; pph ^= 1u; }
+      }
+    } else {
+      for (int ti = 1; ti < my_tiles; ++ti) {
+        while (*ln_done + 3 < ti) __nanosleep(2000);
+        prefetch_tile(ti);
       }
     }
   }
@@ -246,8 +303,7 @@
     const bool bf = FMT == 1;
     uint8_t* hb = smem + Cfg::HB_OFF + uint32_t(g) * FA_HB;
     const uint32_t lane_bits = uint32_t(quad * 32) << 16;
-    const uint32_t ta = tmem_base + lane_bits + uint32_t(g) * FA_TM_SLOT;
-    const uint32_t ts = ta + FA_TM_S;
+    const uint32_t ts = tmem_base + lane_bits + Cfg::s_col(g);
     T16* ctx = static_cast<T16*>(p.ctx);
     long long tok_off = -1;
     uint32_t dm_lo = 0, dm_hi = 0;
@@ -282,6 +338,8 @@
       }
       {
         if (quad == 0 && lane == 0) FA_TR(5, gh);
+        const int a = gh % NACC;
+        const uint32_t ta = tmem_base + lane_bits + Cfg::acc_col(a);
         mbar_wait(&acc_full[g], ph);
         tc_fence_after();
         if (quad == 0 && lane == 0) FA_TR(6, gh);
@@ -289,10 +347,7 @@
         uint8_t* krow = hb + FA_K + j * 128;
         uint8_t* vrow = hb + FA_V + j * 128;
         uint32_t rq[32], rk[32];
-        tmem_ld_32x32(ta, rq);
-        tmem_ld_wait();
-        tmem_ld_32x32(ta + 32u, rk);
-        {
+        auto store_q = [&]() {
           const float4* bq4 = reinterpret_cast<const float4*>(bq_tab + h * 32);
           const float2 qs2 = make_float2(p.qscale, p.qscale);
 #pragma unroll
@@ -306,7 +361,7 @@
             *reinterpret_cast<uint4*>(qrow + own) = make_uint4(pack16(bf, q0.x, q0.y), pack16(bf, q1.x, q1.y), pack16(bf, q2.x, q2.y), pack16(bf, q3.x, q3.y));
             *reinterpret_cast<uint4*>(qrow + other) = make_uint4(0u, 0u, 0u, 0u);
           }
-        }
+        };
         auto store_kv = [&](uint8_t* row, const uint32_t (&rr)[32]) {
           if (j < FA_L) {
 #pragma unroll
@@ -316,14 +371,33 @@
                              pack16(bf, __uint_as_float(rr[8 * c + 4]), __uint_as_float(rr[8 * c + 5])), pack16(bf, __uint_as_float(rr[8 * c + 6]), __uint_as_float(rr[8 * c + 7])));
           }
         };
-        tmem_ld_wait();
-        tmem_ld_32x32(ta + 64u, rq);
-        store_kv(krow, rk);
-        tmem_ld_wait();
-        tc_fence_before();
-        __syncwarp();
-        if (lane == 0) mbar_arrive(&acc_empty[g]);
-        store_kv(vrow, rq);
+        if constexpr (PROJ) {
+          tmem_ld_32x32(ta + 32u, rk);
+          tmem_ld_32x32(ta + 64u, rq);
+          tmem_ld_wait();
+          store_kv(krow, rk);
+          store_kv(vrow, rq);
+          tmem_ld_32x32(ta, rq);
+          tmem_ld_wait();
+          tc_fence_before();
+          __syncwarp();
+          if (lane == 0) mbar_arrive(&acc_empty[a]);
+          mbar_wait(&c_empty[g], ph ^ 1u);
+          store_q();
+        } else {
+          tmem_ld_32x32(ta, rq);
+          tmem_ld_wait();
+          tmem_ld_32x32(ta + 32u, rk);
+          store_q();
+          tmem_ld_wait();
+          tmem_ld_32x32(ta + 64u, rq);
+          store_kv(krow, rk);
+          tmem_ld_wait();
+          tc_fence_before();
+          __syncwarp();
+          if (lane == 0) mbar_arrive(&acc_empty[a]);
+          store_kv(vrow, rq);
+        }
         fence_proxy_async_smem();
         __syncwarp();
         if (lane == 0) mbar_arrive(&qkv_full[g]);
@@ -400,7 +474,55 @@
         tmem_ld_32x32(ts + uint32_t(wdx * 32), o);
         tmem_ld_wait();
         tc_fence_before();
-        if (tok_off >= 0) {
+        if constexpr (PROJ) {
+          const float inv = 1.0f / rsum;
+          const float2 inv2 = make_float2(inv, inv);
+          const float4* bv4 = reinterpret_cast<const float4*>(bv_tab + h * 32);
+          uint8_t* crow = hb + FA_QP + r * 128;
+#pragma unroll
+          for (int q = 0; q < 4; ++q) {
+            const float4 b0 = bv4[2 * q], b1 = bv4[2 * q + 1];
+            const float2 c0 = __ffma2_rn(make_float2(__uint_as_float(o[8 * q]), __uint_as_float(o[8 * q + 1])), inv2, make_float2(b0.x, b0.y));
+            const float2 c1 = __ffma2_rn(make_float2(__uint_as_float(o[8 * q + 2]), __uint_as_float(o[8 * q + 3])), inv2, make_float2(b0.z, b0.w));
+            const float2 c2 = __ffma2_rn(make_float2(__uint_as_float(o[8 * q + 4]), __uint_as_float(o[8 * q + 5])), inv2, make_float2(b1.x, b1.y));
+            const float2 c3 = __ffma2_rn(make_float2(__uint_as_float(o[8 * q + 6]), __uint_as_float(o[8 * q + 7])), inv2, make_float2(b1.z, b1.w));
+            *reinterpret_cast<uint4*>(crow + ((q ^ (r & 7)) << 4)) =
+                make_uint4(pack16(bf, c0.x, c0.y), pack16(bf, c1.x, c1.y), pack16(bf, c2.x, c2.y), pack16(bf, c3.x, c3.y));
+          }
+          fence_proxy_async_smem();
+          __syncwarp();
+          if (lane == 0) mbar_arrive(&c_full[g]);
+          if (h == HEADS - 1) {
+            mbar_wait(out_full, uint32_t(ti) & 1u);
+            tc_fence_after();
+            float* xrow = p.x + (tok_off < 0 ? 0 : tok_off);
+            uint8_t* srow = hb + FA_QP + r * 128;
+#pragma unroll 1
+            for (int cb = 0; cb < C / 32; ++cb) {
+              tmem_ld_32x32(tmem_base + lane_bits + FA_TM_OUT + uint32_t(cb * 32), o);
+              tmem_ld_wait();
+              if (cb == C / 32 - 1) {
+                tc_fence_before();
+                __syncwarp();
+                if (lane == 0) mbar_arrive(out_empty);
+              }
+              if (tok_off >= 0) {
+                if (cb > 0) tma_store_wait_read0();
+                const float4* bp4 = reinterpret_cast<const float4*>(bp_tab + cb * 32);
+#pragma unroll
+                for (int q = 0; q < 8; ++q) {
+                  const float4 b = bp4[q];
+                  *reinterpret_cast<float4*>(srow + q * 16) = make_float4(__uint_as_float(o[4 * q]) + b.x, __uint_as_float(o[4 * q + 1]) + b.y,
+                                                                          __uint_as_float(o[4 * q + 2]) + b.z, __uint_as_float(o[4 * q + 3]) + b.w);
+                }
+                fence_proxy_async_smem();
+                bulk_reduce_add_f32(xrow + cb * 32, srow, 128);
+                tma_store_commit();
+              }
+            }
+            if (tok_off >= 0) tma_store_wait_read0();
+          }
+                } else if (tok_off >= 0) {
           const float inv = 1.0f / rsum;
           const float2 inv2 = make_float2(inv, inv);
           const float4* bv4 = reinterpret_cast<const float4*>(bv_tab + h * 32);
@@ -548,41 +670,48 @@
   if (warp == 1) tmem_dealloc(tmem_base, 512);
 }
 
-template <int FMT, int C>
-static int launch_fa(const CUtensorMap& tmW, const FaParams& p, cudaStream_t stream) {
-  using Cfg = FaCfg<C>;
-  auto kern = swin_attn_fused_kernel<FMT, C>;
+template <int FMT, int C, bool PROJ>
+static int launch_fa(const CUtensorMap& tmW, const CUtensorMap& tmP, const FaParams& p, cudaStream_t stream) {
+  using Cfg = FaCfg<C, PROJ>;
+  auto kern = swin_attn_fused_kernel<FMT, C, PROJ>;
   CSVIT_CUDA(cudaFuncSetAttribute(kern, cudaFuncAttributeMaxDynamicSharedMemorySize, int(Cfg::SMEM)));
   const int tiles = (p.num_windows + 1) / 2;
   const int ctas = tiles < num_sms() ? tiles : num_sms();
-  CSVIT_CUDA(launch_pdl(kern, dim3(ctas), dim3(FA_THREADS), Cfg::SMEM, stream, tmW, p));
+  CSVIT_CUDA(launch_pdl(kern, dim3(ctas), dim3(FA_THREADS), Cfg::SMEM, stream, tmW, tmP, p));
   return 0;
 }
 
-int launch_swin_attn_fused(const float* x, float eps, const void* wqkv_h, const float* bqkv_h,
-                           const void* bias_op, void* ctx, int dtype, int B, int H, int W, int C, int heads, int ws, int shift,
-                           cudaStream_t stream) {
+int launch_swin_attn_fused(float* x, float eps, const void* wqkv_h, const float* bqkv_h, const void* bias_op,
+                           const void* w_proj, const float* b_proj, void* ctx, int dtype, int B, int H, int W, int C, int heads,
+                           int ws, int shift, cudaStream_t stream) {
+  const bool proj = w_proj != nullptr;
   CSVIT_REQUIRE(dtype == DT_BF16 || dtype == DT_F16, "swin_attn_fused: 16-bit operand formats only");
   CSVIT_REQUIRE(C == 128 || C == 256, "swin_attn_fused: C=%d not in {128, 256}", C);
+  CSVIT_REQUIRE(!proj || C == 128, "swin_attn_fused: the out-projection form is built for C = 128 only (C=%d)", C);
+  CSVIT_REQUIRE(proj ? b_proj != nullptr : ctx != nullptr, "swin_attn_fused: null operand");
   CSVIT_REQUIRE(ws == 7 && C == heads * 32, "swin_attn_fused: window 7 / head_dim 32 only (ws=%d C=%d heads=%d)", ws, C, heads);
   CSVIT_REQUIRE(H % ws == 0 && W % ws == 0 && shift >= 0 && shift < ws, "swin_attn_fused: bad geometry %dx%d shift %d", H, W, shift);
   CSVIT_REQUIRE((reinterpret_cast<uintptr_t>(x) & 15) == 0 && (reinterpret_cast<uintptr_t>(ctx) & 15) == 0 &&
-                    (reinterpret_cast<uintptr_t>(bqkv_h) & 15) == 0,
+                    (reinterpret_cast<uintptr_t>(bqkv_h) & 15) == 0 && (reinterpret_cast<uintptr_t>(b_proj) & 15) == 0,
                 "swin_attn_fused: operands must be 16-byte aligned");
   const int nW = (H / ws) * (W / ws);
   const long long windows = static_cast<long long>(B) * nW;
   if (windows <= 0) return 0;
   CSVIT_REQUIRE(windows < (1ll << 30), "swin_attn_fused: too many windows");
   FaParams p{};
-  p.x = x; p.eps = eps; p.bqkv = bqkv_h; p.bias = bias_op; p.ctx = ctx;
+  p.x = x; p.bproj = b_proj; p.eps = eps; p.bqkv = bqkv_h; p.bias = bias_op; p.ctx = ctx;
   p.num_windows = static_cast<int>(windows); p.nW = nW;
   p.qscale = 1.4426950408889634f * 0.17677669529663687f;
   p.g = make_geom(H, W, ws, shift);
-  CUtensorMap tmW;
+  CUtensorMap tmW, tmP{};
   if (int e = make_tmap(&tmW, wqkv_h, C, 3ll * C, C, dtype, 96, true)) return e;
   const bool bf = dtype == DT_BF16;
-  if (C == 128) return bf ? launch_fa<1, 128>(tmW, p, stream) : launch_fa<0, 128>(tmW, p, stream);
-  return bf ? launch_fa<1, 256>(tmW, p, stream) : launch_fa<0, 256>(tmW, p, stream);
+  if (proj) {
+    if (int e = make_tmap_sw64(&tmP, w_proj, C, C, C, dtype, C)) return e;
+    return bf ? launch_fa<1, 128, true>(tmW, tmP, p, stream) : launch_fa<0, 128, true>(tmW, tmP, p, stream);
+  }
+  if (C == 128) return bf ? launch_fa<1, 128, false>(tmW, tmP, p, stream) : launch_fa<0, 128, false>(tmW, tmP, p, stream);
+  return bf ? launch_fa<1, 256, false>(tmW, tmP, p, stream) : launch_fa<0, 256, false>(tmW, tmP, p, stream);
 }
 
 }
diff --git a/cs-vit_b200/csrc/common.cuh b/cs-vit_b200/csrc/common.cuh
--- a/cs-vit_b200/csrc/common.cuh
+++ b/cs-vit_b200/csrc/common.cuh
@@ -176,6 +176,9 @@
 }
 __device__ __forceinline__ void red_add_f32x4(float* p, float4 v) {
   asm volatile("red.global.add.v4.f32 [%0], {%1, %2, %3, %4};" ::"l"(p), "f"(v.x), "f"(v.y), "f"(v.z), "f"(v.w) : "memory");
+}
+__device__ __forceinline__ void bulk_reduce_add_f32(float* gdst, const void* ssrc, uint32_t bytes) {
+  asm volatile("cp.reduce.async.bulk.global.shared::cta.bulk_group.add.f32 [%0], [%1], %2;" ::"l"(gdst), "r"(smem_u32(ssrc)), "r"(bytes) : "memory");
 }
 __device__ __forceinline__ void tma_store_commit() { asm volatile("cp.async.bulk.commit_group;" ::: "memory"); }
 __device__ __forceinline__ void tma_store_wait_read0() { asm volatile("cp.async.bulk.wait_group.read 0;" ::: "memory"); }
diff --git a/cs-vit_b200/csrc/gemm.cu b/cs-vit_b200/csrc/gemm.cu
--- a/cs-vit_b200/csrc/gemm.cu
+++ b/cs-vit_b200/csrc/gemm.cu
@@ -222,6 +222,24 @@
                                                      : (as_tf32 ? CU_TENSOR_MAP_DATA_TYPE_TFLOAT32 : CU_TENSOR_MAP_DATA_TYPE_FLOAT32));
   CUresult r = enc(tm, tdt, 2, const_cast<void*>(ptr), gdim, gstr, box, estr, CU_TENSOR_MAP_INTERLEAVE_NONE,
                    CU_TENSOR_MAP_SWIZZLE_128B, CU_TENSOR_MAP_L2_PROMOTION_L2_256B, CU_TENSOR_MAP_FLOAT_OOB_FILL_NONE);
+  if (r != CUDA_SUCCESS)
+    return set_error("cuTensorMapEncodeTiled failed with CUresult %d (rows=%lld cols=%lld ld=%lld)", int(r), rows, cols, ld);
+  return 0;
+}
+
+int make_tmap_sw64(CUtensorMap* tm, const void* ptr, long long ld, long long rows, long long cols, int dtype, int box_rows) {
+  auto enc = get_tmap_encoder();
+  if (!enc) return set_error("cuTensorMapEncodeTiled entry point not available (driver too old?)");
+  if (dtype != DT_BF16 && dtype != DT_F16) return set_error("make_tmap_sw64: 16-bit tensors only");
+  if ((reinterpret_cast<uintptr_t>(ptr) & 15) || ((ld * 2) & 15))
+    return set_error("operand must be 16-byte aligned with a 16-byte-multiple row pitch (ptr=%p ld=%lld)", ptr, ld);
+  cuuint64_t gdim[2] = {cuuint64_t(cols), cuuint64_t(rows)};
+  cuuint64_t gstr[1] = {cuuint64_t(ld * 2)};
+  cuuint32_t box[2] = {32u, cuuint32_t(box_rows)};
+  cuuint32_t estr[2] = {1, 1};
+  CUresult r = enc(tm, dtype == DT_BF16 ? CU_TENSOR_MAP_DATA_TYPE_BFLOAT16 : CU_TENSOR_MAP_DATA_TYPE_FLOAT16, 2, const_cast<void*>(ptr),
+                   gdim, gstr, box, estr, CU_TENSOR_MAP_INTERLEAVE_NONE, CU_TENSOR_MAP_SWIZZLE_64B, CU_TENSOR_MAP_L2_PROMOTION_L2_256B,
+                   CU_TENSOR_MAP_FLOAT_OOB_FILL_NONE);
   if (r != CUDA_SUCCESS)
     return set_error("cuTensorMapEncodeTiled failed with CUresult %d (rows=%lld cols=%lld ld=%lld)", int(r), rows, cols, ld);
   return 0;
diff --git a/cs-vit_b200/csrc/gemm.cuh b/cs-vit_b200/csrc/gemm.cuh
--- a/cs-vit_b200/csrc/gemm.cuh
+++ b/cs-vit_b200/csrc/gemm.cuh
@@ -447,6 +447,7 @@
 };
 int make_tmap(CUtensorMap* tm, const void* ptr, long long ld, long long rows, long long cols, int dtype, int box_rows,
               bool as_tf32);
+int make_tmap_sw64(CUtensorMap* tm, const void* ptr, long long ld, long long rows, long long cols, int dtype, int box_rows);
 int num_sms();
 int red_add_mode();
 int launch_gemm_pair(const void* A, long long lda, const void* W, long long ldw, int in_dtype, int M, int N, int K,
diff --git a/cs-vit_b200/csrc/rowops.cuh b/cs-vit_b200/csrc/rowops.cuh
--- a/cs-vit_b200/csrc/rowops.cuh
+++ b/cs-vit_b200/csrc/rowops.cuh
@@ -18,9 +18,9 @@
 int launch_merge_index_map(int H, int W, int* out, cudaStream_t stream);
 int launch_expand_rel_bias(const float* table, float* out, int heads, int ws, cudaStream_t stream);
 
-int launch_swin_attn_fused(const float* x, float eps, const void* wqkv_h, const float* bqkv_h,
-                           const void* bias_op, void* ctx, int dtype, int B, int H, int W, int C, int heads, int ws, int shift,
-                           cudaStream_t stream);
+int launch_swin_attn_fused(float* x, float eps, const void* wqkv_h, const float* bqkv_h, const void* bias_op,
+                           const void* w_proj, const float* b_proj, void* ctx, int dtype, int B, int H, int W, int C, int heads,
+                           int ws, int shift, cudaStream_t stream);
 
 int launch_swin_attn_core(const void* qkv, long long ldq, const void* bias_log2, void* ctx, int dtype, int B, int H, int W, int C,
                           int heads, int ws, int shift, int token_order, int q_prescaled, cudaStream_t stream);
diff --git a/include/csvit.h b/include/csvit.h
--- a/include/csvit.h
+++ b/include/csvit.h
@@ -62,8 +62,8 @@
 CSVIT_API int csvit_window_attention(const void* qkv, const float* bias, void* out, int dtype, int B, int H, int W, int C,
                                      int heads, int ws, int shift, void* stream);
 
-CSVIT_API int csvit_swin_attn_fused(const float* x, float eps, const void* wqkv_h, const float* bqkv_h,
-                                    const void* bias_op, void* ctx, int dtype, int B, int H, int W, int C,
+CSVIT_API int csvit_swin_attn_fused(float* x, float eps, const void* wqkv_h, const float* bqkv_h, const void* bias_op,
+                                    const void* w_proj, const float* b_proj, void* ctx, int dtype, int B, int H, int W, int C,
                                     int heads, int ws, int shift, void* stream);
 
 CSVIT_API int csvit_swin_attn_core(const void* qkv, long long ldq, const void* bias_log2, void* ctx, int dtype, int B, int H,
```

Result: slower. 18060, median of 6 (-1.6%).
